# hyperplane-lab/ACL-GAN

Measured on AMD Instinct MI355X. Metric: training images/sec at 256x256 (gen+dis step), higher is better.
Workload: dtype fp32

## Files before the change

acl-gan_amd/csrc/common.h:

```cpp
#pragma once
#include <hip/hip_runtime.h>
#include <stdint.h>
#include <stddef.h>
#include <string>
#include <atomic>
#include "../../include/aclgan_hip.h"
#include "switches.h"

namespace aclgan {

void set_error(const char* fmt, ...);
int hip_fail(hipError_t e, const char* what);

extern std::atomic<long long> g_launches;
extern std::atomic<long long> g_enc_reuse_hits;

#define ACL_CHECK_LAUNCH(what)                                           \
    do {                                                                 \
        ++::aclgan::g_launches;                                          \
        hipError_t e__ = hipGetLastError();                              \
        if (e__ != hipSuccess) return ::aclgan::hip_fail(e__, what);     \
    } while (0)

#define ACL_REQUIRE(cond, ...)                                           \
    do {                                                                 \
        if (!(cond)) { ::aclgan::set_error(__VA_ARGS__); return ACLGAN_EINVAL; } \
    } while (0)

int reduce_slices_ordered(const float* part, int64_t n, int nslices, float* out, hipStream_t st);
size_t colsum_ordered_bytes(int64_t M, int C);
int colsum_ordered(const float* dy, float* db, int64_t M, int C, void* part, hipStream_t st);

static inline int cdiv(int a, int b) { return (a + b - 1) / b; }
static inline int64_t cdiv64(int64_t a, int64_t b) { return (a + b - 1) / b; }

struct ConvGeom {
    int B, Hi, Wi, Ci, Co, k, s, p, up, act;
    int Hu, Wu;
    int Hp, Wp;
    int Ho, Wo;
    int M;
    int K;
};
int make_geom(const aclgan_conv_desc* d, ConvGeom* g);

int conv_fold(const ConvGeom& g, const float* dxp, float* dx, int accumulate, hipStream_t st);
double conv_exec_flops(const ConvGeom& g, int which, bool f16);
bool conv_wgrad_fast_supported(const ConvGeom& g);
int conv_fwd(const ConvGeom& g, const float* x, const float* w, const float* bias, float* y, hipStream_t st, void* scratch = nullptr, float* stats = nullptr,
             float* keepV = nullptr);
size_t conv_fwd_keep_bytes(const ConvGeom& g);
int conv_fwd_stats_chunk(const ConvGeom& g);
size_t conv_fwd_scratch_bytes(const ConvGeom& g);
size_t conv_up5_scratch_bytes(const ConvGeom& g);
int conv_up5_fwd(const ConvGeom& g, const float* x, const float* w, const float* bias, float* y, void* scratch, hipStream_t st, float* keepV = nullptr);
int conv_fwd_naive(const ConvGeom& g, const float* x, const float* w, const float* bias, float* y, hipStream_t st);
size_t conv_dgrad_scratch_bytes(const ConvGeom& g);
int conv_dgrad(const ConvGeom& g, const float* dy, const float* w, float* dx, void* scratch, int accumulate, hipStream_t st);
int conv_wgrad(const ConvGeom& g, const float* x, const float* dy, float* dw, float* db, hipStream_t st, void* scratch = nullptr, const float* haveV = nullptr);
size_t conv_wgrad_scratch_bytes(const ConvGeom& g);
int conv_up5_dgrad(const ConvGeom& g, const float* dy, const float* w, float* dx, int accumulate, void* scratch, hipStream_t st);
int conv_up5_wgrad(const ConvGeom& g, const float* x, const float* dy, float* dw, float* db, void* scratch, hipStream_t st, const float* haveV = nullptr);

int conv_fwd_fast(const ConvGeom& g, const float* x, const float* w, const float* bias, float* y, hipStream_t st, void* scratch = nullptr, float* stats = nullptr,
                  float* keepV = nullptr);
size_t conv_fwd_fast_scratch_bytes(const ConvGeom& g);
int conv_dgrad_fast(const ConvGeom& g, const float* dy, const float* w, float* dxp, float* dx, int accumulate, bool* direct, hipStream_t st);
int conv_wgrad_fast(const ConvGeom& g, const float* x, const float* dy, float* dw, float* db, hipStream_t st, void* scratch = nullptr, const float* haveV = nullptr);
size_t conv_wgrad_fast_scratch_bytes(const ConvGeom& g);

struct WinoUCache { void* user; float* (*lookup)(void* user, const float* w, int variant, size_t bytes, bool* fresh); };
void set_wino_ucache(const WinoUCache* c);
const WinoUCache* wino_ucache();
size_t conv_wino_u_bytes(const ConvGeom& g);
int conv_wino_u_variant(const ConvGeom& g, int dgrad, bool keepV);
int conv_up5_wino_u_variant(const ConvGeom& g, int dgrad, bool keepV);
int conv_wino_prefill(const ConvGeom& g, int uv, const float* w0, int64_t w_stride, float* U0, int64_t u_stride, int count, hipStream_t st);
int wino_fused_filter_batch(const float* w0, int64_t w_stride, float* Uf0, int64_t u_stride, int count, int Co, int Ci, int flip, hipStream_t st);

bool conv_wino_ok(const ConvGeom& g);
size_t conv_wino_scratch_bytes(const ConvGeom& g);
int conv_fwd_wino(const ConvGeom& g, const float* x, const float* w, const float* bias, float* y, void* scratch, hipStream_t st, float* stats = nullptr,
                  float* keepV = nullptr);
size_t conv_wino_keep_bytes(const ConvGeom& g);
size_t conv_up5_wino_keep_bytes(const ConvGeom& g);
int conv_dgrad_wino_interior(const ConvGeom& g, const float* dy, const float* w, float* dx, int accumulate, void* scratch, hipStream_t st);
size_t conv_wgrad_wino_scratch_bytes(const ConvGeom& g);
bool conv_up5_wino_ok(const ConvGeom& g);
size_t conv_up5_wino_fwd_scratch_bytes(const ConvGeom& g);
size_t conv_up5_wino_dgrad_scratch_bytes(const ConvGeom& g);
size_t conv_up5_wino_wgrad_scratch_bytes(const ConvGeom& g);
int conv_up5_wino_fwd_phases(const ConvGeom& g, const float* x, const float* wp, const float* bias, float* y, void* scratch, hipStream_t st, float* keepV = nullptr,
                             const float* wkey = nullptr);
int conv_up5_wino_dgrad_phases(const ConvGeom& g, const float* dy, const float* wp, float* dx, int accumulate, void* scratch, hipStream_t st,
                               const float* wkey = nullptr);
bool wino_u_cached(const float* wkey, int variant);
int conv_up5_wino_wgrad_phases(const ConvGeom& g, const float* x, const float* dy, float* dwp, float* db, void* scratch, hipStream_t st, const float* haveV = nullptr);
size_t conv_up5_dgrad_scratch_bytes(const ConvGeom& g);
int conv_wgrad_wino(const ConvGeom& g, const float* x, const float* dy, float* dw, float* db, void* scratch, hipStream_t st, const float* haveV = nullptr);

bool conv16_eligible(const ConvGeom& g, int which);
size_t conv_fwd16_scratch_bytes(const ConvGeom& g);
size_t conv_dgrad16_scratch_bytes(const ConvGeom& g);
size_t conv_wgrad16_scratch_bytes(const ConvGeom& g);
int conv_fwd16(const ConvGeom& g, int dtype, const float* x, const float* w, const void* w16, const float* bias, float* y, void* scratch, hipStream_t st,
               const void* x16 = nullptr, int y_storage = 0);
int conv_dgrad16(const ConvGeom& g, int dtype, const float* dy, const float* w, const void* w16t, float* dx, int accumulate, void* scratch, hipStream_t st);
int conv_wgrad16(const ConvGeom& g, int dtype, const float* x, const float* dy, float* dw, float* db, void* scratch, hipStream_t st, int x_storage = 0,
                 int dy_storage = 0);

bool conv16s_ok(const ConvGeom& g, int which);
int conv_fwd16s_stats_chunk(const ConvGeom& g);
int wino_fused_force(int on);
bool wino_fused_ok(int B, int H, int W, int Cin_, int Cout_, int act = ACLGAN_ACT_NONE, int gph = 1, int kph = 1);
int wino_fused_filter(const float* w, float* Uf, int Co, int Ci, int flip, hipStream_t st, int nph = 1);
int wino_fused_launch(int B, int H, int W, int Cin_, int Cout_, const float* in, const float* Uf, const float* bias, float* out, int act, int accumulate,
                      int reflect, float2* stats, hipStream_t st);
int wino_fused_up5_fwd(int B, int Hi, int Wi, int Cin_, int Cout_, const float* x, const float* Uf, const float* bias, float* y, int Hf, int Wf, int act,
                       hipStream_t st);
bool wino_wgrad_fused_ok(const ConvGeom& g);
size_t wino_wgrad_fused_scratch_bytes(const ConvGeom& g);
int wino_wgrad_fused(const ConvGeom& g, const float* x, const float* dy, float* dw, float* db, void* scratch, hipStream_t st);
int wino_fused_up5_dgrad(int B, int Hi, int Wi, int Cin_, int Cout_, const float* dy, const float* Uf, float* dx, int Hf, int Wf, int accumulate, hipStream_t st);
bool wino_fused_s2k4_ok(int B, int Hi, int Wi, int Ci, int Co, int act, int dgrad);
size_t wino_fused_s2k4_u_bytes(int Ci, int Co);
int wino_fused_filter_s2k4(const float* w, float* Uf, int Co, int Ci, int dgrad, hipStream_t st);
int wino_fused_s2k4_fwd(int B, int Hi, int Wi, int Ci, int Co, const float* x, const float* Uf, const float* bias, float* y, int act, float2* stats, hipStream_t st);
int wino_fused_s2k4_dgrad(int B, int Hi, int Wi, int Ci, int Co, const float* dy, const float* Uf, float* dx, int accumulate, hipStream_t st);
bool conv_s2k4_wino_ok(const ConvGeom& g, int which);
size_t conv_s2k4_wino_scratch_bytes(const ConvGeom& g);
int conv_fwd_s2k4_wino(const ConvGeom& g, const float* x, const float* w, const float* bias, float* y, void* scratch, hipStream_t st, float* stats = nullptr);
int conv_dgrad_s2k4_wino_interior(const ConvGeom& g, const float* dy, const float* w, float* dx, int accumulate, void* scratch, hipStream_t st);
bool gemm_x3_shape_ok(int T, int K, int N);
int gemm_slices_x3(const void* A3, size_t a_plane, const void* B3, size_t b_plane, float* C, int T, int K, int N, int nslices, int a_mod, hipStream_t st);
int split3_planes(const float* x, void* out, int64_t n, int64_t plane_elems, hipStream_t st);
int conv_fwd16s(const ConvGeom& g, int dtype, const void* x16, const void* w16, const float* bias, void* y, int yst, hipStream_t st, float* stats = nullptr);
size_t conv_dgrad16s_scratch_bytes(const ConvGeom& g);
bool conv_wgrad16s_ok(const ConvGeom& g);
size_t conv_wgrad16s_scratch_bytes(const ConvGeom& g);
int conv_wgrad16s(const ConvGeom& g, int dtype, const void* x16, const void* dy16, float* dw, float* db, void* scratch, hipStream_t st);
int conv_dgrad16s(const ConvGeom& g, int dtype, const void* dy16, const void* w16t, void* dx, int dxst, int accumulate, void* scratch, hipStream_t st);
int cast_flat16(const float* src, void* dst, int64_t n, int dtype, hipStream_t st);
int transpose_flat16(const float* base, void* base_t, const int64_t* offs, const int* co, const int* taps, const int* ci, int n, int dtype, hipStream_t st);

int conv_fwd_small(const ConvGeom& g, const float* x, const float* w, const float* bias, float* y, hipStream_t st);
int conv_wgrad_small(const ConvGeom& g, const float* x, const float* dy, float* dw, float* db, hipStream_t st, void* scratch = nullptr);
size_t conv_wgrad_small_scratch_bytes(const ConvGeom& g);
int conv_dgrad_small(const ConvGeom& g, const float* dy, const float* w, float* dxp, hipStream_t st);
bool conv_s2k4_thin_dgrad_ok(const ConvGeom& g);

size_t norm_scratch_bytes(int B, int HW, int C);
struct NormST { int x = 0, y = 0, res = 0, dy = 0, dx = 0, dres = 0; };
int norm_fwd(int kind, int act, int B, int HW, int C, const void* x, const float* w, const float* b, int w_stride,
             const void* residual, void* y, float* mean, float* rstd, void* scratch, hipStream_t st, const float* stats = nullptr,
             int stats_chunk = 0, const NormST* sto = nullptr, float* ss_out = nullptr);
int norm_bwd(int kind, int act, int B, int HW, int C, const void* x, const void* y, const void* dy,
             const float* w, int w_stride, const float* mean, const float* rstd, void* dx, float* dw, float* db,
             void* dres, int dres_accumulate, void* scratch, hipStream_t st, const NormST* sto = nullptr, float* sbc_out = nullptr,
             const float* ss = nullptr);
int norm_bwd_ln_params(const float* sbc, int B, int C, float* dgamma, float* dbeta, hipStream_t st);

int act_bwd_inplace(int act, const void* y, void* dy, int64_t n, hipStream_t st, int yst = 0, int gst = 0);
int cast_storage(const void* src, int src_st, void* dst, int dst_st, int64_t n, hipStream_t st);
int positive_mask(const void* y, int yst, unsigned char* dst, int64_t n, hipStream_t st);
int positive_mask_diff(const float* a, int ca, const float* b, int cb, unsigned char* dst, int64_t npix, hipStream_t st);
int avgpool3s2_fwd(int B, int H, int W, int C, const float* x, float* y, hipStream_t st);
int avgpool3s2_bwd(int B, int H, int W, int C, const float* dy, float* dx, int accumulate, hipStream_t st);
size_t diffaugment_scratch_bytes(int N, int H, int W, int C);
int diffaugment_fwd(int N, int H, int W, int C, int policy, const float* x, const float* params, float* y, void* scratch, hipStream_t st);
int diffaugment_bwd(int N, int H, int W, int C, int policy, const float* dy, const float* params, float* dx, int accumulate, void* scratch, hipStream_t st);
int adam_flat(float* p, const float* g, float* m, float* v, int64_t n, const aclgan_adam* o, int step, hipStream_t st);
int adam_flat_ema(float* p, const float* g, float* m, float* v, float* ema, int64_t n, const aclgan_adam* o, int step, float decay, int mode, hipStream_t st);
int nchw_to_nhwc(const float* src, float* dst, int B, int C, int H, int W, hipStream_t st);
int nhwc_to_nchw(const float* src, float* dst, int B, int C, int H, int W, hipStream_t st);
int fill_zero(float* p, int64_t n, hipStream_t st);

int linear_fwd(int B, int I, int O, const float* x, const float* w, const float* bias, int act, float* y, hipStream_t st);
bool mlp3_fwd_ok(int S, int M);
int mlp3_fwd(int B, int S, int M, int O, const float* s, const float* W0, const float* b0, const float* W1, const float* b1, const float* W2,
             const float* b2, float* m0, float* m1, float* ap, hipStream_t st);
int linear_bwd(int B, int I, int O, const float* x, const float* y, float* dy, const float* w, int act,
               float* dx, float* dw, float* db, hipStream_t st);
int linear_bwd_params(int B, int I, int O, const float* x, const float* dy, float* dw, float* db, hipStream_t st);
int gap_fwd(int B, int HW, int C, const void* x, float* y, hipStream_t st, int xst = 0);
int gap_bwd(int B, int HW, int C, const float* dy, void* dx, int accumulate, hipStream_t st, int xst = 0);

int focus_blend_fwd(int B, int HW, const float* dec4, const float* bg, float* out, const float* pair_first, float* pair, hipStream_t st);
int focus_blend_bwd(int B, int HW, const float* dec4, const float* bg, const float* d_out, const float* d_pair,
                    float* d_dec4, float* d_bg, int bg_accumulate, hipStream_t st);
int plain_pair_fwd(int B, int HW, const float* dec3, float* out, const float* pair_first, float* pair, hipStream_t st);
int plain_pair_bwd(int B, int HW, const float* d_out, const float* d_pair, float* d_dec3, hipStream_t st);
int focus_translation_nchw(const float* fg, int64_t fg_bstride, const float* bg, int64_t bg_bstride, const float* focus, int64_t focus_bstride,
                           float* out, int B, int HW, hipStream_t st);
int lsgan_loss(const float* o, int n, float target, float weight, float* loss_slot, float* d_o, float gscale, hipStream_t st, const float* lscale = nullptr);
struct LsganTerm { const float* o; float* d_o; float* slot; int n; float target, weight, gscale; };
const int LSGAN_MAX_TERMS = 12;
int lsgan_loss_batch(const LsganTerm* terms, int nterms, hipStream_t st, const float* lscale = nullptr);
const int L1_PART_FLOATS = 1024;
int l1_loss(const float* a, int a_stride, const float* b, int64_t npix, float* loss_slot, float* d_a, float gscale, int d_accumulate, hipStream_t st,
            const float* lscale = nullptr, float* part = nullptr);
int focus_sums_blocks(int64_t npix);
int focus_sums(const float* dec4, int64_t npix, float eps, float upper, float* part, hipStream_t st);
int focus_loss_finish(const float* dec4, int64_t npix, const float* part, float delta, float upper, float lower, float eps,
                      float scale, float* size_slot, float* digit_slot, float* d_dec4, hipStream_t st, const float* lscale = nullptr,
                      const float* totals = nullptr, int64_t npix_total = 0);
int focus_totals(const float* part, int64_t npix, int nmask, float* totals, hipStream_t st);
int adam_flat_scaled(float* p, const float* g, float* m, float* v, int64_t n, const aclgan_adam* o, int step, float* state, int group, hipStream_t st);
int adam_flat_scaled_ema(float* p, const float* g, float* m, float* v, float* ema, int64_t n, const aclgan_adam* o, int step, float decay, int mode,
                         float* state, int group, hipStream_t st);


const int SN_MAX_LAYERS = 16;
struct SnLayerPtrs { const float* w; float* u; float* v; float* wn; float* uf; float* vf; float* G; int co, k; };
size_t sn_scratch_bytes(int n, const int* co, const int* k);
int sn_power_iteration(int n, const SnLayerPtrs* L, float* sigma, void* scratch, hipStream_t st);
struct SnFoldPtrs { const float* w; const float* G; const float* u; const float* v; float* grad; int co, k; };
size_t sn_fold_scratch_bytes(int n, const int* co, const int* k);
int sn_fold(int n, const SnFoldPtrs* L, const float* sigma, void* scratch, hipStream_t st);

}
```

acl-gan_amd/csrc/conv_fast.hip:

```cpp
#include "conv_fast_common.h"
#include <cstring>

namespace aclgan {
namespace {


constexpr int BK = 16;
constexpr int WG_MAX_CHUNK = 1024 + 16;
constexpr int LDK = BK + 4;

template <int T, bool KC>
__device__ __forceinline__ void read_frags(const float* __restrict__ tile, int ld, int base, int lane, float (&f)[T][8]) {
    const int l31 = lane & 31, kh = lane >> 5;
    if (KC) {
#pragma unroll
        for (int t = 0; t < T; ++t) {
            const f32x4* p = reinterpret_cast<const f32x4*>(tile + (base + t * 32 + l31) * LDK + kh * 8);
            const f32x4 a = p[0], b = p[1];
            f[t][0] = a.x; f[t][1] = a.y; f[t][2] = a.z; f[t][3] = a.w;
            f[t][4] = b.x; f[t][5] = b.y; f[t][6] = b.z; f[t][7] = b.w;
        }
    } else {
#pragma unroll
        for (int ks = 0; ks < 8; ++ks)
#pragma unroll
            for (int t = 0; t < T; ++t) f[t][ks] = tile[(kh * 8 + ks) * ld + base + t * 32 + l31];
    }
}

template <int TM, int TN>
__device__ __forceinline__ void mfma_step(const float (&fa)[TM][8], const float (&fb)[TN][8], int ks, f32x16 (&acc)[TM][TN]) {
#pragma unroll
    for (int i = 0; i < TM; ++i)
#pragma unroll
        for (int j = 0; j < TN; ++j) acc[i][j] = __builtin_amdgcn_mfma_f32_32x32x2f32(fa[i][ks], fb[j][ks], acc[i][j], 0, 0, 0);
}

#define ACL_GEMM_MAINLOOP(TM_, TN_, AKC_, BKC_, KBEG_, NK_, AS_, BS_, ASTR_, BSTR_, LDA_, LDB_, AM_, BN_) \
    do {                                                                                                 \
        const int nk__ = (NK_), kb__ = (KBEG_);                                                          \
        fetch(kb__);                                                                                     \
        stage(0, true);                                                                                  \
        fetch(kb__ + min(1, nk__ - 1));                                                                  \
        __syncthreads();                                                                                 \
        for (int kt = 0; kt < nk__; ++kt) {                                                              \
            const int cur = kt & 1;                                                                      \
            float fa[TM_][8], fb[TN_][8];                                                                \
            read_frags<TM_, AKC_>((AS_) + cur * (ASTR_), (LDA_), (AM_), lane, fa);                       \
            read_frags<TN_, BKC_>((BS_) + cur * (BSTR_), (LDB_), (BN_), lane, fb);                       \
            if (!(AKC_) && !(BKC_)) __builtin_amdgcn_sched_barrier(0);    \
            mfma_step<TM_, TN_>(fa, fb, 0, acc);                                                         \
            stage(cur ^ 1, kt + 1 < nk__);                                                               \
            fetch(kb__ + min(kt + 2, nk__ - 1));                                                         \
            __builtin_amdgcn_sched_barrier(0x6);    \
            mfma_step<TM_, TN_>(fa, fb, 1, acc);                                                         \
            mfma_step<TM_, TN_>(fa, fb, 2, acc);                                                         \
            mfma_step<TM_, TN_>(fa, fb, 3, acc);                                                         \
            mfma_step<TM_, TN_>(fa, fb, 4, acc);                                                         \
            mfma_step<TM_, TN_>(fa, fb, 5, acc);                                                         \
            mfma_step<TM_, TN_>(fa, fb, 6, acc);                                                         \
            mfma_step<TM_, TN_>(fa, fb, 7, acc);                                                         \
            __syncthreads();                                                                             \
        }                                                                                                \
    } while (0)



template <int WM, int WN, int TM, int TN, int OCC = 1>
__global__ void __launch_bounds__(WM * WN * 64, OCC) conv_fwd_fast_kernel(FwdFP pk) {
    constexpr int BM = WM * TM * 32, BN = WN * TN * 32, NT = WM * WN * 64;
    constexpr int RP = NT / 4;
    FwdFP p = pk;
    if (pk.fsl) {
        const long long f = blockIdx.y;
        p.x += (pk.fsx_mod ? f % pk.fsx_mod : f) * pk.fs_x; p.w += f * pk.fs_w; p.y += f * pk.fs_y;
    }
    constexpr int A_IT = BM / RP, B_IT = (BN + RP - 1) / RP;
    __shared__ __attribute__((aligned(16))) float smem[2 * (BM + BN) * LDK];
    __shared__ int ro[BM];
    float* As = smem;
    float* Bs = smem + 2 * BM * LDK;

    const int tid = threadIdx.x, lane = tid & 63, wave = tid >> 6;
    const int wm = wave / WN, wn = wave % WN;
    const int tile = xcd_map(blockIdx.x, p.nwg);
    const int m0 = (tile / p.tiles_n) * BM, n0 = (tile % p.tiles_n) * BN;
    const int q = tid & 3, r0 = tid >> 2;
    const int phase = p.phases ? (int)blockIdx.z : 0;
    const float* wbase = p.w + (size_t)phase * p.Co * p.K;

    for (int r = tid; r < BM; r += NT) {
        int b, oy, ox, o = -1;
        if (fwd_row(p, m0 + r, b, oy, ox)) {
            if (p.phases) o = (b * p.Hf + 2 * (oy + 1) + (phase >> 1)) * p.Wf + 2 * (ox + 1) + (phase & 1);
            else o = (b * p.Ho + oy) * p.Wo + ox;
        }
        ro[r] = o;
    }
    int ay[A_IT], ax[A_IT], ab[A_IT];
#pragma unroll
    for (int i = 0; i < A_IT; ++i) {
        int b = 0, oy = 0, ox = 0;
        if (!fwd_row(p, m0 + r0 + i * RP, b, oy, ox)) { b = 0; oy = 0; ox = 0; }
        ay[i] = oy * p.s - p.p; ax[i] = ox * p.s - p.p; ab[i] = b * p.Hi * p.Wi;
    }
    int wo[B_IT];
#pragma unroll
    for (int i = 0; i < B_IT; ++i) wo[i] = min(n0 + r0 + i * RP, p.Co - 1) * p.K + q * 4;

    const int cpt = p.Ci >> 4;
    int aoff[A_IT];
    f32x4 ra[A_IT], rb[B_IT];
    int f_tap = -1;

    auto fetch = [&](int kt) __attribute__((always_inline)) {
        const int tap = kt / cpt, cc = kt - tap * cpt;
        if (tap != f_tap) {
            f_tap = tap;
            const int ky = tap / p.k, kx = tap - ky * p.k;
#pragma unroll
            for (int i = 0; i < A_IT; ++i) {
                const int iy = refl(ay[i] + ky, p.Hu) >> p.up;
                const int ix = refl(ax[i] + kx, p.Wu) >> p.up;
                aoff[i] = (ab[i] + iy * p.Wi + ix) * p.Ci + q * 4;
            }
        }
#pragma unroll
        for (int i = 0; i < A_IT; ++i) ra[i] = *reinterpret_cast<const f32x4*>(p.x + (size_t)aoff[i] + cc * 16);
#pragma unroll
        for (int i = 0; i < B_IT; ++i)
            if (BN % RP == 0 || r0 + i * RP < BN) rb[i] = *reinterpret_cast<const f32x4*>(wbase + (size_t)wo[i] + kt * 16);
    };
    auto stage = [&](int buf, bool real) __attribute__((always_inline)) {
        float* a = As + buf * BM * LDK;
        float* b = Bs + buf * BN * LDK;
#pragma unroll
        for (int i = 0; i < A_IT; ++i) *reinterpret_cast<f32x4*>(a + (r0 + i * RP) * LDK + q * 4) = ra[i];
#pragma unroll
        for (int i = 0; i < B_IT; ++i)
            if (BN % RP == 0 || r0 + i * RP < BN) *reinterpret_cast<f32x4*>(b + (r0 + i * RP) * LDK + q * 4) = rb[i];
    };

    f32x16 acc[TM][TN];
#pragma unroll
    for (int i = 0; i < TM; ++i)
#pragma unroll
        for (int j = 0; j < TN; ++j)
#pragma unroll
            for (int r = 0; r < 16; ++r) acc[i][j][r] = 0.f;

    const int nk_all = p.K / BK;
    const int kbeg = p.phases ? 0 : blockIdx.z * p.nkz, nk = p.phases ? nk_all : min(p.nkz, nk_all - kbeg);
    if (nk <= 0) return;
    const bool split = !p.phases && gridDim.z > 1;
    ACL_GEMM_MAINLOOP(TM, TN, true, true, kbeg, nk, As, Bs, BM * LDK, BN * LDK, LDK, LDK, wm * TM * 32, wn * TN * 32);

    const int l31 = lane & 31, lh = lane >> 5;
#pragma unroll
    for (int j = 0; j < TN; ++j) {
        const int n = n0 + wn * TN * 32 + j * 32 + l31;
        if (n >= p.Co) continue;
        const float bv = p.bias ? p.bias[n] : 0.f;
#pragma unroll
        for (int i = 0; i < TM; ++i) {
#pragma unroll
            for (int r = 0; r < 16; ++r) {
                const int rl = wm * TM * 32 + i * 32 + (r & 3) + 8 * (r >> 2) + 4 * lh;
                const int o = ro[rl];
                if (o >= 0) {
                    if (split && p.part) p.part[((size_t)blockIdx.z * p.rows + m0 + rl) * p.Co + n] = acc[i][j][r];
                    else if (split) atomicAdd(p.y + (size_t)o * p.Co + n, acc[i][j][r] + ((p.ring > 0 && blockIdx.z == 0) ? bv : 0.f));
                    else p.y[(size_t)o * p.Co + n] = act_apply(acc[i][j][r] + bv, p.act);
                }
            }
        }
    }
}


template <int WM, int WN, int TM, int TN>
int launch_fwd_fast(const ConvGeom& g, FwdFP p, hipStream_t st) {
    constexpr int BM = WM * TM * 32, BN = WN * TN * 32;
    p.tiles_n = cdiv(g.Co, BN);
    int rows = p.M;
    if (p.ring > 0) rows = p.B * (p.Ho * p.Wo - std::max(0, p.Ho - 2 * p.ring) * std::max(0, p.Wo - 2 * p.ring));
    p.nwg = cdiv(rows, BM) * p.tiles_n;
    if (p.phases) {
        hipLaunchKernelGGL((conv_fwd_fast_kernel<WM, WN, TM, TN>), dim3(p.nwg, 1, 4), dim3(WM * WN * 64), 0, st, p);
        ACL_CHECK_LAUNCH("conv_fwd_fast_kernel(phases)");
        return ACLGAN_OK;
    }
    int splits = 1;
    fwd_split_plan(rows, g.Co, g.K, BK, &splits, &p.nkz);
    p.rows = rows;
    if (splits > 1 && p.part != nullptr) {
        hipLaunchKernelGGL((conv_fwd_fast_kernel<WM, WN, TM, TN>), dim3(p.nwg, 1, splits), dim3(WM * WN * 64), 0, st, p);
        ACL_CHECK_LAUNCH("conv_fwd_fast_kernel(split)");
        hipLaunchKernelGGL(fwd_split_finish_kernel, dim3((int)std::min<int64_t>(cdiv64((int64_t)rows * std::max(1, g.Co / 4), 256), 4096)), dim3(256), 0, st, p, splits);
        ACL_CHECK_LAUNCH("fwd_split_finish_kernel");
        return ACLGAN_OK;
    }
    p.part = nullptr;
    const int nk = g.K / BK;
    if (p.ring > 0 && (p.act != ACLGAN_ACT_NONE || g.Co % 4 != 0)) splits = 1, p.nkz = nk;
    if (sw(SW_DETERMINISTIC)) splits = 1, p.nkz = nk;
    if (splits > 1 && p.ring > 0) {
        hipLaunchKernelGGL(ring_zero_kernel, dim3(cdiv(rows * (g.Co / 4), 256)), dim3(256), 0, st, p, rows);
        ACL_CHECK_LAUNCH("ring_zero_kernel");
    } else if (splits > 1) {
        hipError_t e = hipMemsetAsync(p.y, 0, (size_t)g.M * g.Co * sizeof(float), st);
        if (e != hipSuccess) return hip_fail(e, "memset y");
    }
    hipLaunchKernelGGL((conv_fwd_fast_kernel<WM, WN, TM, TN>), dim3(p.nwg, 1, splits), dim3(WM * WN * 64), 0, st, p);
    ACL_CHECK_LAUNCH("conv_fwd_fast_kernel");
    if (splits > 1 && p.ring == 0) {
        const int64_t n = (int64_t)g.M * g.Co;
        hipLaunchKernelGGL(bias_act_kernel, dim3((int)std::min<int64_t>(cdiv64(n, 256), 4096)), dim3(256), 0, st, p.y, p.bias, g.Co, p.act, n);
        ACL_CHECK_LAUNCH("bias_act_kernel");
    }
    return ACLGAN_OK;
}


template <int WM, int WN, int TM, int TN>
__global__ void __launch_bounds__(WM * WN * 64) conv_dgrad_fast_kernel(DgFP p) {
    constexpr int BM = WM * TM * 32, BN = WN * TN * 32, NT = WM * WN * 64;
    constexpr int RP = NT / 4;
    constexpr int A_IT = BM / RP;
    constexpr int LDB = BN + 4, NVB = BN / 4;
    constexpr int B_IT = (BK * NVB + NT - 1) / NT;
    __shared__ __attribute__((aligned(16))) float smem[2 * (BM * LDK + BK * LDB)];
    __shared__ int ri_o[BM];
    __shared__ unsigned long long tap_mask;
    __shared__ int tap_list[64];
    float* As = smem;
    float* Bs = smem + 2 * BM * LDK;

    const int tid = threadIdx.x, lane = tid & 63, wave = tid >> 6;
    const int wm = wave / WN, wn = wave % WN;
    const int tile = xcd_map(blockIdx.x, p.nwg);
    const int m0 = (tile / p.tiles_n) * BM;
    const int n0 = (tile % p.tiles_n) * BN;
    const int cls = blockIdx.z / p.ksplit, slice = blockIdx.z - cls * p.ksplit;
    const int cy = cls / p.s, cx = cls % p.s;
    const int Tx = (p.k - cx + p.s - 1) / p.s, Ty = (p.k - cy + p.s - 1) / p.s;
    const int q = tid & 3, r0 = tid >> 2;

    int ylo, yhi, xlo, xhi;
    dg_box(p, cy, cx, ylo, yhi, xlo, xhi);
    const bool compact = p.mode == 2 && Ty * Tx <= 64;
    if (tid == 0) tap_mask = 0ull;
    __syncthreads();
    for (int r = tid; r < BM; r += NT) {
        int oo = -1, b, y2, x2;
        if (dg_row(p, m0 + r, ylo, yhi, xlo, xhi, b, y2, x2)) {
            const int py = y2 * p.s + cy, px = x2 * p.s + cx;
            if (compact && py < p.Hp && px < p.Wp) {
                unsigned long long mk = 0ull;
                for (int t = 0; t < Ty * Tx; ++t) {
                    const int ty = t / Tx, tx = t - ty * Tx;
                    const int oy = y2 - ty, ox = x2 - tx;
                    bool ok = (unsigned)oy < (unsigned)p.Ho && (unsigned)ox < (unsigned)p.Wo;
                    if (p.band > 0) ok = ok && (oy < 2 || oy >= p.Ho - 2 || ox < 2 || ox >= p.Wo - 2);
                    if (ok) mk |= 1ull << t;
                }
                if (mk) atomicOr(&tap_mask, mk);
            }
            if (py < p.Hp && px < p.Wp) {
                if (p.mode == 0 || p.ringpad) oo = (b * p.Hp + py) * p.Wp + px;
                else oo = (b * p.Hd + (refl(py - p.pad, p.Hi) >> p.upshift)) * p.Wd + (refl(px - p.pad, p.Wi) >> p.upshift);
            }
        }
        ri_o[r] = oo;
    }
    int ntap = Ty * Tx;
    if (compact) {
        __syncthreads();
        if (tid == 0) {
            int n = 0;
            for (int t = 0; t < Ty * Tx; ++t)
                if ((tap_mask >> t) & 1ull) tap_list[n++] = t;
            tap_list[63] = n;
        }
        __syncthreads();
        ntap = tap_list[63];
        if (ntap == 0) return;
    }
    int ay[A_IT], ax[A_IT], ab[A_IT];
#pragma unroll
    for (int i = 0; i < A_IT; ++i) {
        int b = 0, y2 = 0, x2 = 0;
        if (!dg_row(p, m0 + r0 + i * RP, ylo, yhi, xlo, xhi, b, y2, x2)) { b = 0; y2 = 0; x2 = 0; }
        ay[i] = y2; ax[i] = x2; ab[i] = b;
    }
    int bo[B_IT];
#pragma unroll
    for (int i = 0; i < B_IT; ++i) {
        const int idx = tid + i * NT;
        const int krow = idx / NVB, nc = idx - krow * NVB;
        const int n = n0 + nc * 4;
        bo[i] = krow * p.k * p.k * p.Ci + (n < p.Ci ? n : 0);
    }
    const int cpt = p.Co >> 4;
    int aoff[A_IT];
    f32x4 ra[A_IT], rb[B_IT];
    float za[A_IT];
    int f_tap = -1, tapoff = 0;

    auto fetch = [&](int kt) __attribute__((always_inline)) {
        const int tq = kt / cpt, cc = kt - tq * cpt;
        if (tq != f_tap) {
            f_tap = tq;
            const int t = compact ? tap_list[tq] : tq;
            const int ty = t / Tx, tx = t - ty * Tx;
            tapoff = ((cy + p.s * ty) * p.k + (cx + p.s * tx)) * p.Ci;
#pragma unroll
            for (int i = 0; i < A_IT; ++i) {
                const int oy = ay[i] - ty, ox = ax[i] - tx;
                const bool ok = (unsigned)oy < (unsigned)p.Ho && (unsigned)ox < (unsigned)p.Wo;
                bool okk = ok;
                if (p.band > 0) okk = ok && (oy < 2 || oy >= p.Ho - 2 || ox < 2 || ox >= p.Wo - 2);
                const int dpix = p.dyv ? (ab[i] * p.Hf + 2 * (oy + 1) + p.py) * p.Wf + 2 * (ox + 1) + p.px
                                       : (ab[i] * p.Ho + oy) * p.Wo + ox;
                aoff[i] = okk ? dpix * p.Co + q * 4 : -1;
            }
        }
#pragma unroll
        for (int i = 0; i < A_IT; ++i) {
            ra[i] = *reinterpret_cast<const f32x4*>(p.dy + (size_t)(aoff[i] < 0 ? 0 : aoff[i]) + cc * 16);
            za[i] = aoff[i] < 0 ? 0.f : 1.f;
        }
#pragma unroll
        for (int i = 0; i < B_IT; ++i)
            if ((BK * NVB) % NT == 0 || tid + i * NT < BK * NVB)
                rb[i] = *reinterpret_cast<const f32x4*>(p.w + (size_t)bo[i] + tapoff + (size_t)cc * 16 * p.k * p.k * p.Ci);
    };
    auto stage = [&](int buf, bool real) __attribute__((always_inline)) {
        float* a = As + buf * BM * LDK;
        float* b = Bs + buf * BK * LDB;
#pragma unroll
        for (int i = 0; i < A_IT; ++i) *reinterpret_cast<f32x4*>(a + (r0 + i * RP) * LDK + q * 4) = ra[i] * za[i];
#pragma unroll
        for (int i = 0; i < B_IT; ++i) {
            const int idx = tid + i * NT;
            if ((BK * NVB) % NT == 0 || idx < BK * NVB) {
                const int krow = idx / NVB, nc = idx - krow * NVB;
                *reinterpret_cast<f32x4*>(b + krow * LDB + nc * 4) = rb[i];
            }
        }
    };

    f32x16 acc[TM][TN];
#pragma unroll
    for (int i = 0; i < TM; ++i)
#pragma unroll
        for (int j = 0; j < TN; ++j)
#pragma unroll
            for (int r = 0; r < 16; ++r) acc[i][j][r] = 0.f;

    const int nk_all = ntap * cpt;
    const int nkz = (nk_all + p.ksplit - 1) / p.ksplit;
    const int kbeg = slice * nkz, nk = min(nkz, nk_all - kbeg);
    if (nk <= 0) return;
    ACL_GEMM_MAINLOOP(TM, TN, true, false, kbeg, nk, As, Bs, BM * LDK, BK * LDB, LDK, LDB, wm * TM * 32, wn * TN * 32);

    const int l31 = lane & 31, lh = lane >> 5;
#pragma unroll
    for (int j = 0; j < TN; ++j) {
        const int n = n0 + wn * TN * 32 + j * 32 + l31;
        if (n >= p.Ci) continue;
#pragma unroll
        for (int i = 0; i < TM; ++i) {
#pragma unroll
            for (int r = 0; r < 16; ++r) {
                const int of = ri_o[wm * TM * 32 + i * 32 + (r & 3) + 8 * (r >> 2) + 4 * lh];
                if (of >= 0) {
                    float* o = p.dxp + (size_t)of * p.Ci + n;
                    if (p.ksplit > 1 || (p.mode == 2 && !p.ringpad)) atomicAdd(o, acc[i][j][r]);
                    else if (p.accumulate) *o += acc[i][j][r];
                    else *o = acc[i][j][r];
                }
            }
        }
    }
}

template <int WM, int WN, int TM, int TN>
int launch_dgrad_fast(const ConvGeom& g, DgFP p, hipStream_t st) {
    constexpr int BM = WM * TM * 32, BN = WN * TN * 32;
    int mmax = 0;
    for (int cy = 0; cy < g.s; ++cy)
        for (int cx = 0; cx < g.s; ++cx) {
            const int ylo = g.p > cy ? (g.p - cy + g.s - 1) / g.s : 0, xlo = g.p > cx ? (g.p - cx + g.s - 1) / g.s : 0;
            const int yhi = std::min(p.Hc - 1, (g.p + g.Hi - 1 - cy) / g.s), xhi = std::min(p.Wc - 1, (g.p + g.Wi - 1 - cx) / g.s);
            int inner = (yhi - ylo + 1) * (xhi - xlo + 1);
            if (p.band > 0) inner = std::max(0, p.Hc - 2 * p.band) * std::max(0, p.Wc - 2 * p.band);
            const int rows = p.mode == 0 ? p.Hc * p.Wc : (p.mode == 1 ? inner : p.Hc * p.Wc - inner);
            mmax = std::max(mmax, g.B * rows);
        }
    if (mmax <= 0) return ACLGAN_OK;
    p.Mc = mmax;
    p.tiles_n = cdiv(g.Ci, BN);
    p.nwg = cdiv(p.Mc, BM) * p.tiles_n;
    const int nk_min = ((g.k + g.s - 1) / g.s) * ((g.k + g.s - 1) / g.s) * (g.Co / 16);
    const int nblk = p.nwg * g.s * g.s;
    p.ksplit = 1;
    const int nk_plan = (p.mode == 2 && p.band == 0) ? std::max(g.Co / 16, nk_min / ((g.k + g.s - 1) / g.s)) : nk_min;
    if (nblk < 128 && nk_plan >= 32 && !sw(SW_DETERMINISTIC) && !p.ringpad)
        p.ksplit = max(1, min(nk_plan / 8, 512 / nblk));
    if (p.ksplit > 1 && p.mode == 0) {
        hipError_t e = hipMemsetAsync(p.dxp, 0, conv_dgrad_scratch_bytes(g), st);
        if (e != hipSuccess) return hip_fail(e, "memset dxp");
    }
    if (p.ksplit > 1 && p.mode == 1 && !p.accumulate) {
        hipError_t e = hipMemsetAsync(p.dxp, 0, (size_t)g.B * g.Hi * g.Wi * g.Ci * sizeof(float), st);
        if (e != hipSuccess) return hip_fail(e, "memset dx");
    }
    hipLaunchKernelGGL((conv_dgrad_fast_kernel<WM, WN, TM, TN>), dim3(p.nwg, 1, g.s * g.s * p.ksplit), dim3(WM * WN * 64), 0, st, p);
    ACL_CHECK_LAUNCH("conv_dgrad_fast_kernel");
    return ACLGAN_OK;
}

template <int WM, int WN, int TM, int TN>
int launch_dgrad_halo(const ConvGeom& g, DgFP p, hipStream_t st) {
    if (p.band == 0 && !p.ringpad && g.k == 3 && g.s == 1 && g.Ci % 128 == 0 && WM == 2 && WN == 2 && TM == 2 && TN == 2)
        return launch_dgrad_fast<2, 2, 1, 2>(g, p, st);
    return launch_dgrad_fast<WM, WN, TM, TN>(g, p, st);
}

template <int WM, int WN, int TM, int TN>
int dgrad_fast_all(const ConvGeom& g, DgFP p, float* dxp, float* dx, int accumulate, bool* direct, hipStream_t st) {
    if (g.up == 0 && dx != nullptr && (!sw(SW_DETERMINISTIC) || g.p == 0 || (dxp && conv_wino_ok(g)))) {
        *direct = true;
        p.dxp = dx; p.accumulate = accumulate;
        p.mode = 1;
        int rc = (dxp && conv_wino_ok(g)) ? conv_dgrad_wino_interior(g, p.dy, p.w, dx, accumulate, dxp, st)
             : (dxp && conv_s2k4_wino_ok(g, 1)) ? conv_dgrad_s2k4_wino_interior(g, p.dy, p.w, dx, accumulate, dxp, st)
                                      : launch_dgrad_fast<WM, WN, TM, TN>(g, p, st);
        if (rc) return rc;
        if (g.p > 0 && sw(SW_DETERMINISTIC)) {
            hipError_t e = hipMemsetAsync(dxp, 0, (size_t)g.B * g.Hp * g.Wp * g.Ci * sizeof(float), st);
            if (e != hipSuccess) return hip_fail(e, "memset padded grid");
            p.mode = 2; p.ringpad = 1; p.dxp = dxp; p.accumulate = 0;
            rc = launch_dgrad_fast<WM, WN, TM, TN>(g, p, st);
            if (rc) return rc;
            return conv_fold(g, dxp, dx, 1, st);
        }
        if (g.p > 0) { p.mode = 2; rc = launch_dgrad_halo<WM, WN, TM, TN>(g, p, st); }
        return rc;
    }
    *direct = false;
    p.dxp = dxp; p.mode = 0; p.accumulate = 0;
    return launch_dgrad_fast<WM, WN, TM, TN>(g, p, st);
}


template <int WM, int WN, int TM, int TN, bool ST>
__global__ void __launch_bounds__(WM * WN * 64) conv_wgrad_fast_kernel(WgFP p) {
    constexpr int BM = WM * TM * 32, BN = WN * TN * 32, NT = WM * WN * 64;
    constexpr int LDA = BM + 4, LDB = BN + 4, MVA = BM / 4, NVB = BN / 4;
    constexpr int A_IT = (BK * MVA + NT - 1) / NT, B_IT = (BK * NVB + NT - 1) / NT;
    __shared__ __attribute__((aligned(16))) float smem[2 * BK * (LDA + LDB)];
    float* As = smem;
    float* Bs = smem + 2 * BK * LDA;

    const int tid = threadIdx.x, lane = tid & 63, wave = tid >> 6;
    const int wm = wave / WN, wn = wave % WN;
    const int tile = xcd_map(blockIdx.x, p.nwg);
    const int m0 = (tile / p.tiles_n) * BM, n0 = (tile % p.tiles_n) * BN;
    const int pbeg = blockIdx.z * p.chunk;
    const int pend = min(p.P, pbeg + p.chunk);
    if (pbeg >= pend) return;
    const int phase = p.phases ? (int)blockIdx.y : 0;
    float* dwbase = p.dw + (size_t)phase * p.Co * p.Kn + (size_t)blockIdx.z * p.dw_zs;
    const int py = phase >> 1, px = phase & 1;

    __shared__ int4 pinfo[WG_MAX_CHUNK];
    const int st_tap = n0 / p.Ci, st_ky = st_tap / p.k, st_kx = st_tap - st_ky * p.k;
    for (int i = tid; i < pend - pbeg + BK; i += NT) {
        int b, oy, ox;
        wg_coord(p, min(pbeg + i, pend - 1), b, oy, ox);
        const int dyp = p.phases ? (b * p.Hf + 2 * (oy + 1) + py) * p.Wf + 2 * (ox + 1) + px : (b * p.Ho + oy) * p.Wo + ox;
        if (ST) {
            const int iy = refl(oy * p.s - p.p + st_ky, p.Hu) >> p.up, ix = refl(ox * p.s - p.p + st_kx, p.Wu) >> p.up;
            pinfo[i] = make_int4(b * p.Hi * p.Wi + iy * p.Wi + ix, 0, 0, dyp);
        } else {
            pinfo[i] = make_int4(oy * p.s - p.p, ox * p.s - p.p, b * p.Hi * p.Wi, dyp);
        }
    }
    __syncthreads();

    int a_m[A_IT], a_kr[A_IT];
#pragma unroll
    for (int i = 0; i < A_IT; ++i) {
        const int idx = tid + i * NT;
        a_kr[i] = idx / MVA;
        const int m = m0 + (idx - a_kr[i] * MVA) * 4;
        a_m[i] = m < p.Co ? m : 0;
    }
    int b_kr[B_IT], b_ci[B_IT], b_ky[B_IT], b_kx[B_IT];
#pragma unroll
    for (int i = 0; i < B_IT; ++i) {
        const int idx = tid + i * NT;
        b_kr[i] = idx / NVB;
        int n = n0 + (idx - b_kr[i] * NVB) * 4;
        if (n >= p.Kn) n = 0;
        const int tap = n / p.Ci;
        b_ci[i] = n - tap * p.Ci; b_ky[i] = tap / p.k; b_kx[i] = tap - b_ky[i] * p.k;
    }
    f32x4 ra[A_IT], rb[B_IT];
    float za[A_IT];
    const bool do_bias = p.db != nullptr && (tile % p.tiles_n) == 0;
    f32x4 bsum[A_IT];
#pragma unroll
    for (int i = 0; i < A_IT; ++i) bsum[i] = (f32x4){0.f, 0.f, 0.f, 0.f};

    auto fetch = [&](int kt) __attribute__((always_inline)) {
        const int pb = kt * BK;
#pragma unroll
        for (int i = 0; i < A_IT; ++i) {
            if ((BK * MVA) % NT != 0 && tid + i * NT >= BK * MVA) continue;
            const int pi = pb + a_kr[i];
            ra[i] = *reinterpret_cast<const f32x4*>(p.dy + (size_t)pinfo[pi].w * p.Co + a_m[i]);
            za[i] = pbeg + pi < pend ? 1.f : 0.f;
        }
#pragma unroll
        for (int i = 0; i < B_IT; ++i) {
            if ((BK * NVB) % NT != 0 && tid + i * NT >= BK * NVB) continue;
            if (ST) {
                rb[i] = *reinterpret_cast<const f32x4*>(p.x + (size_t)pinfo[pb + b_kr[i]].x * p.Ci + b_ci[i]);
            } else {
                const int4 pi = pinfo[pb + b_kr[i]];
                const int iy = refl(pi.x + b_ky[i], p.Hu) >> p.up;
                const int ix = refl(pi.y + b_kx[i], p.Wu) >> p.up;
                rb[i] = *reinterpret_cast<const f32x4*>(p.x + (size_t)(pi.z + iy * p.Wi + ix) * p.Ci + b_ci[i]);
            }
        }
    };
    auto stage = [&](int buf, bool real) __attribute__((always_inline)) {
        float* a = As + buf * BK * LDA;
        float* b = Bs + buf * BK * LDB;
#pragma unroll
        for (int i = 0; i < A_IT; ++i) {
            const int idx = tid + i * NT;
            if ((BK * MVA) % NT == 0 || idx < BK * MVA) {
                const f32x4 v = ra[i] * za[i];
                *reinterpret_cast<f32x4*>(a + a_kr[i] * LDA + (idx - a_kr[i] * MVA) * 4) = v;
                bsum[i] += v * (real ? 1.f : 0.f);
            }
        }
#pragma unroll
        for (int i = 0; i < B_IT; ++i) {
            const int idx = tid + i * NT;
            if ((BK * NVB) % NT == 0 || idx < BK * NVB) *reinterpret_cast<f32x4*>(b + b_kr[i] * LDB + (idx - b_kr[i] * NVB) * 4) = rb[i];
        }
    };

    f32x16 acc[TM][TN];
#pragma unroll
    for (int i = 0; i < TM; ++i)
#pragma unroll
        for (int j = 0; j < TN; ++j)
#pragma unroll
            for (int r = 0; r < 16; ++r) acc[i][j][r] = 0.f;

    ACL_GEMM_MAINLOOP(TM, TN, false, false, 0, (pend - pbeg + BK - 1) / BK, As, Bs, BK * LDA, BK * LDB, LDA, LDB, wm * TM * 32, wn * TN * 32);

    if (do_bias) {
        float* red = smem;
#pragma unroll
        for (int i = 0; i < A_IT; ++i) {
            const int idx = tid + i * NT;
            if ((BK * MVA) % NT == 0 || idx < BK * MVA) *reinterpret_cast<f32x4*>(red + a_kr[i] * BM + (idx - a_kr[i] * MVA) * 4) = bsum[i];
        }
        __syncthreads();
        if (tid < BM && m0 + tid < p.Co) {
            float t = 0.f;
#pragma unroll
            for (int r = 0; r < BK; ++r) t += red[r * BM + tid];
            atomicAdd(p.db + (size_t)blockIdx.z * p.db_zs + m0 + tid, t);
        }
    }
    const int l31 = lane & 31, lh = lane >> 5;
#pragma unroll
    for (int j = 0; j < TN; ++j) {
        const int n = n0 + wn * TN * 32 + j * 32 + l31;
        if (n >= p.Kn) continue;
#pragma unroll
        for (int i = 0; i < TM; ++i) {
#pragma unroll
            for (int r = 0; r < 16; ++r) {
                const int m = m0 + wm * TM * 32 + i * 32 + (r & 3) + 8 * (r >> 2) + 4 * lh;
                if (m < p.Co) {
                    atomicAdd(dwbase + (size_t)m * p.Kn + n, acc[i][j][r]);
                }
            }
        }
    }
}

constexpr int WGKC_TARGET = 768;

template <int WM, int WN, int TM, int TN>
__global__ void __launch_bounds__(WM * WN * 64) conv_wgrad_kc_kernel(WgFP pk, WgPartX xp) {
    constexpr int BM = WM * TM * 32, BN = WN * TN * 32, NT = WM * WN * 64;
    WgFP p = pk;
    if (pk.fsl) {
        const long long f = blockIdx.y;
        p.x += (pk.fsx_mod ? f % pk.fsx_mod : f) * pk.fs_x; p.dy += f * pk.fs_dy;
    }
    static_assert(BM % 64 == 0 && BN % 64 == 0 && BM + BN <= NT, "one staging unit (4 channels x 4 pixels) per thread, wave-uniform roles");
    constexpr int CH = 1024;
    __shared__ __attribute__((aligned(16))) float smem[2 * (BM + BN) * LDK];
    __shared__ int2 pinfo[CH + BK];
    float* As = smem;
    float* Bs = smem + 2 * BM * LDK;

    const int tid = threadIdx.x, lane = tid & 63, wave = tid >> 6;
    const int wm = wave / WN, wn = wave % WN;
    const int tile = xcd_map(blockIdx.x, p.nwg);
    const int m0 = (tile / p.tiles_n) * BM, n0 = (tile % p.tiles_n) * BN;
    const int pbeg = blockIdx.z * p.chunk;
    const int pend = min(p.P, pbeg + p.chunk);
    const int phase = (p.phases || p.fsl) ? (int)blockIdx.y : 0;
    float* dwbase = p.dw + (size_t)phase * p.Co * p.Kn;
    const int py = phase >> 1, px = phase & 1;
    const int st_tap = n0 / p.Ci, st_ky = st_tap / p.k, st_kx = st_tap - st_ky * p.k;

    const bool isA = tid < BM, isB = !isA && tid < BM + BN;
    const int u = isA ? tid : tid - BM;
    const int ncg = (isA ? BM : BN) >> 2;
    const int cg = u % ncg, pg = u / ncg;
    const float* src = isA ? p.dy : p.x;
    const int cstride = isA ? p.Co : p.Ci;
    const int chan = isA ? m0 + 4 * cg : (n0 - st_tap * p.Ci) + 4 * cg;
    float* mytile = isA ? As : Bs;
    const int tstride = (isA ? BM : BN) * LDK;
    f32x4 rr[4];
    float zm[4];
    const bool do_bias = p.db != nullptr && (tile % p.tiles_n) == 0;
    f32x4 bsum = {0.f, 0.f, 0.f, 0.f};

    f32x16 acc[TM][TN];
#pragma unroll
    for (int i = 0; i < TM; ++i)
#pragma unroll
        for (int j = 0; j < TN; ++j)
#pragma unroll
            for (int r = 0; r < 16; ++r) acc[i][j][r] = 0.f;

    for (int cb = pbeg; cb < pend; cb += CH) {
        const int ce = min(pend, cb + CH);
        for (int i = tid; i < ce - cb + BK; i += NT) {
            int b, oy, ox;
            wg_coord(p, min(cb + i, ce - 1), b, oy, ox);
            const int dyp = p.phases ? (b * p.Hf + 2 * (oy + 1) + py) * p.Wf + 2 * (ox + 1) + px : (b * p.Ho + oy) * p.Wo + ox;
            const int iy = refl(oy * p.s - p.p + st_ky, p.Hu) >> p.up, ix = refl(ox * p.s - p.p + st_kx, p.Wu) >> p.up;
            pinfo[i] = make_int2(b * p.Hi * p.Wi + iy * p.Wi + ix, dyp);
        }
        __syncthreads();

        auto fetch = [&](int kt) __attribute__((always_inline)) {
            const int pb = kt * BK + 4 * pg;
            if (isA || isB) {
#pragma unroll
                for (int j = 0; j < 4; ++j) {
                    const int2 pi = pinfo[pb + j];
                    rr[j] = *reinterpret_cast<const f32x4*>(src + (size_t)(isA ? pi.y : pi.x) * cstride + chan);
                    zm[j] = cb + pb + j < ce ? 1.f : 0.f;
                }
            }
        };
        auto stage = [&](int buf, bool real) __attribute__((always_inline)) {
            if (isA || isB) {
                float* t = mytile + buf * tstride;
                f32x4 v[4];
#pragma unroll
                for (int j = 0; j < 4; ++j) v[j] = rr[j] * zm[j];
                if (isA) {
                    const float on = real ? 1.f : 0.f;
#pragma unroll
                    for (int j = 0; j < 4; ++j) bsum += v[j] * on;
                }
#pragma unroll
                for (int c = 0; c < 4; ++c) {
                    const f32x4 k4 = {v[0][c], v[1][c], v[2][c], v[3][c]};
                    *reinterpret_cast<f32x4*>(t + (c * ncg + cg) * LDK + 4 * pg) = k4;
                }
            }
        };
        ACL_GEMM_MAINLOOP(TM, TN, true, true, 0, (ce - cb + BK - 1) / BK, As, Bs, BM * LDK, BN * LDK, LDK, LDK, wm * TM * 32, wn * TN * 32);
    }

    const bool partial = xp.part != nullptr;
    if (do_bias) {
        float* red = smem;
        if (isA) *reinterpret_cast<f32x4*>(red + pg * BM + 4 * cg) = bsum;
        __syncthreads();
        if (tid < BM) {
            const float t = red[tid] + red[BM + tid] + red[2 * BM + tid] + red[3 * BM + tid];
            if (partial) xp.part_b[((size_t)blockIdx.z * xp.ny + phase) * p.Co + m0 + tid] = t;
            else p.db[m0 + tid] += t;
        }
    }
    const int l31 = lane & 31, lh = lane >> 5;
    constexpr int MQ = BM / 4, NQ = BN / 4;
    if (partial) {
        float* pt = xp.part + (((size_t)blockIdx.z * xp.ny + phase) * p.nwg + tile) * (BM * BN);
#pragma unroll
        for (int j = 0; j < TN; ++j)
#pragma unroll
            for (int i = 0; i < TM; ++i)
#pragma unroll
                for (int r = 0; r < 16; ++r) {
                    const int rw = wm * TM * 32 + i * 32 + (r & 3) + 8 * (r >> 2) + 4 * lh;
                    pt[rw * BN + wn * TN * 32 + j * 32 + l31] = acc[i][j][r];
                }
        return;
    }
#pragma unroll
    for (int j = 0; j < TN; ++j) {
        const int cr = wn * TN * 32 + j * 32 + l31;
        const int n = n0 + 4 * (cr % NQ) + cr / NQ;
#pragma unroll
        for (int i = 0; i < TM; ++i) {
#pragma unroll
            for (int r = 0; r < 16; ++r) {
                const int rw = wm * TM * 32 + i * 32 + (r & 3) + 8 * (r >> 2) + 4 * lh;
                const int m = m0 + 4 * (rw % MQ) + rw / MQ;
                dwbase[(size_t)m * p.Kn + n] += acc[i][j][r];
            }
        }
    }
}

bool wgrad_kc_ok(const ConvGeom& g) {
    return !sw(SW_NOWGKC) && g.Co % 64 == 0 && g.Ci % 64 == 0;
}

template <int WM, int WN, int TM, int TN>
int launch_wgrad_kc(const ConvGeom& g, WgFP p, void* part, hipStream_t st) {
    constexpr int BM = WM * TM * 32, BN = WN * TN * 32;
    const int ny = p.fsl ? p.fsl : (p.phases ? 4 : 1);
    const WgPlan q = wgrad_plan(g.Co, p.Ci, p.Kn, p.P, ny, BK, WGKC_TARGET);
    if (q.BM != BM || q.BN != BN) { set_error("wgrad_kc: tile plan mismatch"); return ACLGAN_EINVAL; }
    p.tiles_n = q.tiles_n; p.nwg = q.nwg; p.chunk = q.chunk;
    WgPartX xp;
    xp.ny = ny; xp.part = nullptr; xp.part_b = nullptr;
    const bool use_part = q.splits > 1 || ny > 1;
    if (use_part) {
        if (!part) { set_error("wgrad_kc: %d slices need the scratch buffer", q.splits); return ACLGAN_EINVAL; }
        xp.part = (float*)part;
        xp.part_b = xp.part + (size_t)q.splits * ny * q.nwg * BM * BN;
    }
    hipLaunchKernelGGL((conv_wgrad_kc_kernel<WM, WN, TM, TN>), dim3(p.nwg, ny, q.splits), dim3(WM * WN * 64), 0, st, p, xp);
    ACL_CHECK_LAUNCH("conv_wgrad_kc_kernel");
    if (use_part) {
        const int64_t n = (int64_t)ny * g.Co * (p.Kn / 4);
        hipLaunchKernelGGL(wgrad_finish_kernel, dim3((int)std::min<int64_t>(cdiv64(n, 256), 4096)), dim3(256), 0, st, p, xp, BM, BN, q.splits);
        ACL_CHECK_LAUNCH("wgrad_finish_kernel");
    }
    return ACLGAN_OK;
}
int launch_wgrad_kc_any(const ConvGeom& g, const WgFP& p, void* part, hipStream_t st) {
    if (g.Co % 128 == 0 && p.Ci % 128 == 0) return launch_wgrad_kc<2, 2, 2, 2>(g, p, part, st);
    if (g.Co % 128 == 0) return launch_wgrad_kc<2, 2, 2, 1>(g, p, part, st);
    if (p.Ci % 128 == 0) return launch_wgrad_kc<2, 2, 1, 2>(g, p, part, st);
    return launch_wgrad_kc<2, 2, 1, 1>(g, p, part, st);
}

template <int WM, int WN, int TM, int TN>
int launch_wgrad_fast(const ConvGeom& g, WgFP p, hipStream_t st, void* det_part = nullptr) {
    constexpr int BM = WM * TM * 32, BN = WN * TN * 32;
    p.tiles_n = cdiv(p.Kn, BN);
    p.nwg = cdiv(g.Co, BM) * p.tiles_n;
    const int target = 1536;
    const int ny = p.phases ? 4 : 1;
    int splits = max(1, target / (p.nwg * ny));
    splits = max(1, min(splits, cdiv(p.P, 256)));
    splits = max(splits, cdiv(p.P, 1024));
    p.chunk = cdiv(cdiv(p.P, splits), 16) * 16;
    splits = cdiv(p.P, p.chunk);
    float* dw_out = p.dw; float* db_out = p.db;
    const int64_t ndw = (int64_t)ny * g.Co * p.Kn;
    if (det_part != nullptr && splits > 1) {
        hipError_t e = hipMemsetAsync(det_part, 0, (size_t)splits * (ndw + g.Co) * sizeof(float), st);
        if (e != hipSuccess) return hip_fail(e, "memset wgrad slices");
        p.dw = (float*)det_part; p.dw_zs = ndw;
        if (p.db) { p.db = (float*)det_part + (size_t)splits * ndw; p.db_zs = g.Co; }
    }
    if (p.Ci % BN == 0) hipLaunchKernelGGL((conv_wgrad_fast_kernel<WM, WN, TM, TN, true>), dim3(p.nwg, ny, splits), dim3(WM * WN * 64), 0, st, p);
    else hipLaunchKernelGGL((conv_wgrad_fast_kernel<WM, WN, TM, TN, false>), dim3(p.nwg, ny, splits), dim3(WM * WN * 64), 0, st, p);
    ACL_CHECK_LAUNCH("conv_wgrad_fast_kernel");
    if (p.dw_zs) {
        int rc = reduce_slices_ordered(p.dw, ndw, splits, dw_out, st);
        if (rc) return rc;
        if (db_out) { rc = reduce_slices_ordered(p.db, g.Co, splits, db_out, st); if (rc) return rc; }
    }
    return ACLGAN_OK;
}
size_t wgrad_fast_det_bytes(const ConvGeom& g, int Kn, int P, int ny) {
    const int nwg = cdiv(g.Co, 128) * cdiv(Kn, 128);
    int splits = std::max(1, 1536 / (nwg * ny));
    splits = std::max(1, std::min(splits, cdiv(P, 256)));
    splits = std::max(splits, cdiv(P, 1024)) + 1;
    return (size_t)splits * ((size_t)ny * g.Co * Kn + g.Co) * sizeof(float) + 256;
}


template <int WM, int WN, int TM, int TN>
int up5_fwd_t(const ConvGeom& g, const float* x, const float* w, const float* bias, float* y, float* wp, hipStream_t st, float* keepV) {
    const int64_t nm = (int64_t)4 * g.Co * 9 * (g.Ci / 4);
    if (!(conv_up5_wino_ok(g) && wino_u_cached(w, conv_up5_wino_u_variant(g, 0, keepV != nullptr)))) {
        hipLaunchKernelGGL(up5_merge_kernel, dim3((int)std::min<int64_t>(cdiv64(nm, 256), 2048)), dim3(256), 0, st, w, wp, g.Co, g.Ci);
        ACL_CHECK_LAUNCH("up5_merge_kernel");
    }
    FwdFP p;
    p.fsl = 0; p.fsx_mod = 0; p.fs_x = p.fs_w = p.fs_y = 0; p.w16 = nullptr; p.x16 = nullptr;
    p.x = x; p.w = wp; p.bias = bias; p.y = y;
    p.Hi = g.Hi; p.Wi = g.Wi; p.Ci = g.Ci; p.Ho = g.Hi - 2; p.Wo = g.Wi - 2; p.Co = g.Co; p.k = 3; p.s = 1; p.p = 0;
    p.up = 0; p.Hu = g.Hi; p.Wu = g.Wi; p.M = g.B * p.Ho * p.Wo; p.K = 9 * g.Ci; p.act = g.act; p.tiles_n = 0; p.nwg = 0; p.nkz = 0;
    p.B = g.B; p.ring = 0; p.phases = 1; p.Hf = g.Ho; p.Wf = g.Wo; p.part = nullptr; p.rows = 0;
    ConvGeom gp = g;
    gp.M = p.M; gp.K = p.K;
    char* wino_scr = (char*)wp + up5_merged_bytes(g) + ((fwd_partial_bytes(g, 2, BK) + 255) & ~(size_t)255);
    if (keepV && !conv_up5_wino_ok(g)) { set_error("conv_fwd: this layer does not keep a Winograd input transform"); return ACLGAN_EINVAL; }
    int rc = conv_up5_wino_ok(g) ? conv_up5_wino_fwd_phases(g, x, wp, bias, y, wino_scr, st, keepV, w) : launch_fwd_fast<WM, WN, TM, TN>(gp, p, st);
    if (rc) return rc;
    p.w = w;
    p.Hi = g.Hi; p.Wi = g.Wi; p.Ho = g.Ho; p.Wo = g.Wo; p.k = 5; p.s = 1; p.p = 2; p.up = 1; p.Hu = g.Hu; p.Wu = g.Wu;
    p.M = g.M; p.K = g.K; p.ring = 2; p.phases = 0;
    p.part = (float*)((char*)wp + up5_merged_bytes(g));
    return launch_fwd_fast<WM, WN, TM, TN>(g, p, st);
}

template <int WM, int WN, int TM, int TN>
int up5_wgrad_t(const ConvGeom& g, const float* x, const float* dy, float* dw, float* db, float* dwp, hipStream_t st, const float* haveV) {
    const size_t nb = (size_t)4 * g.Co * 9 * g.Ci * sizeof(float);
    hipError_t e = hipMemsetAsync(dwp, 0, nb, st);
    if (e != hipSuccess) return hip_fail(e, "memset dwp");
    const bool kc = wgrad_kc_ok(g);
    void* part = (char*)dwp + up5_dwp_bytes(g);
    WgFP p;
    p.fsl = 0; p.fsx_mod = 0; p.fs_x = p.fs_dy = 0;
    p.x = x; p.dy = dy; p.dw = dwp; p.db = db;
    p.Hi = g.Hi; p.Wi = g.Wi; p.Ci = g.Ci; p.Ho = g.Hi - 2; p.Wo = g.Wi - 2; p.Co = g.Co; p.k = 3; p.s = 1; p.p = 0;
    p.up = 0; p.Hu = g.Hi; p.Wu = g.Wi; p.P = g.B * p.Ho * p.Wo; p.Kn = 9 * g.Ci; p.chunk = 0; p.tiles_n = 0; p.nwg = 0;
    p.B = g.B; p.ring = 0; p.phases = 1; p.Hf = g.Ho; p.Wf = g.Wo;
    int rc;
    if (kc && conv_up5_wino_wgrad_scratch_bytes(g)) {
        void* wino_scr = (char*)dwp + ((wgrad_part_scratch(g, BK, WGKC_TARGET) + 255) & ~(size_t)255);
        rc = conv_up5_wino_wgrad_phases(g, x, dy, dwp, db, wino_scr, st, haveV);
    } else rc = kc ? launch_wgrad_kc_any(g, p, part, st) : launch_wgrad_fast<WM, WN, TM, TN>(g, p, st);
    if (rc) return rc;
    const int64_t ns = (int64_t)g.Co * 25 * (g.Ci / 4);
    hipLaunchKernelGGL(up5_scatter_kernel, dim3((int)std::min<int64_t>(cdiv64(ns, 256), 2048)), dim3(256), 0, st, dwp, dw, g.Co, g.Ci);
    ACL_CHECK_LAUNCH("up5_scatter_kernel");
    p.dw = dw;
    p.Hi = g.Hi; p.Wi = g.Wi; p.Ho = g.Ho; p.Wo = g.Wo; p.k = 5; p.s = 1; p.p = 2; p.up = 1; p.Hu = g.Hu; p.Wu = g.Wu;
    p.ring = 2; p.phases = 0; p.Kn = g.K;
    p.P = g.B * (g.Ho * g.Wo - (g.Ho - 4) * (g.Wo - 4));
    return kc ? launch_wgrad_kc_any(g, p, part, st) : launch_wgrad_fast<WM, WN, TM, TN>(g, p, st);
}

template <int WM, int WN, int TM, int TN>
int up5_dgrad_t(const ConvGeom& g, const float* dy, const float* w, float* dx, int accumulate, float* wp, hipStream_t st) {
    const int64_t nm = (int64_t)4 * g.Co * 9 * (g.Ci / 4);
    if (!(conv_up5_wino_ok(g) && wino_u_cached(w, conv_up5_wino_u_variant(g, 1, false)))) {
        hipLaunchKernelGGL(up5_merge_kernel, dim3((int)std::min<int64_t>(cdiv64(nm, 256), 2048)), dim3(256), 0, st, w, wp, g.Co, g.Ci);
        ACL_CHECK_LAUNCH("up5_merge_kernel");
    }
    ConvGeom gv = g;
    gv.k = 3; gv.s = 1; gv.p = 0; gv.up = 0; gv.Hu = g.Hi; gv.Wu = g.Wi; gv.Hp = g.Hi; gv.Wp = g.Wi;
    gv.Ho = g.Hi - 2; gv.Wo = g.Wi - 2; gv.M = g.B * gv.Ho * gv.Wo; gv.K = 9 * g.Ci;
    DgFP p;
    p.dy = dy; p.dxp = dx;
    p.Ho = gv.Ho; p.Wo = gv.Wo; p.Co = g.Co; p.Ci = g.Ci; p.k = 3; p.s = 1; p.Hp = g.Hi; p.Wp = g.Wi;
    p.Hc = g.Hi; p.Wc = g.Wi; p.Mc = 0; p.tiles_n = 0; p.nwg = 0; p.ksplit = 1;
    p.mode = 1; p.pad = 0; p.B = g.B; p.Hi = g.Hi; p.Wi = g.Wi;
    p.dyv = 1; p.Hf = g.Ho; p.Wf = g.Wo; p.band = 0; p.upshift = 0; p.Hd = g.Hi; p.Wd = g.Wi;
    if (conv_up5_wino_ok(g)) {
        const int rc = conv_up5_wino_dgrad_phases(g, dy, wp, dx, accumulate, (char*)wp + up5_merged_bytes(g), st, w);
        if (rc) return rc;
    } else for (int ph = 0; ph < 4; ++ph) {
        p.w = wp + (size_t)ph * g.Co * 9 * g.Ci;
        p.py = ph >> 1; p.px = ph & 1;
        p.accumulate = (ph > 0 || accumulate) ? 1 : 0;
        const int rc = launch_dgrad_fast<WM, WN, TM, TN>(gv, p, st);
        if (rc) return rc;
    }
    p.w = w;
    p.Ho = g.Ho; p.Wo = g.Wo; p.k = 5; p.s = 1; p.Hp = g.Hp; p.Wp = g.Wp; p.Hc = g.Hp; p.Wc = g.Wp;
    p.mode = 2; p.accumulate = 1; p.pad = 2; p.Hi = g.Hu; p.Wi = g.Wu;
    p.dyv = 0; p.band = 6; p.upshift = 1; p.Hd = g.Hi; p.Wd = g.Wi;
    if (sw(SW_DETERMINISTIC)) {
        float* dxp = (float*)((char*)wp + up5_merged_bytes(g));
        hipError_t e = hipMemsetAsync(dxp, 0, (size_t)g.B * g.Hp * g.Wp * g.Ci * sizeof(float), st);
        if (e != hipSuccess) return hip_fail(e, "memset padded grid");
        p.ringpad = 1; p.dxp = dxp; p.accumulate = 0;
        const int rc = launch_dgrad_fast<WM, WN, TM, TN>(g, p, st);
        if (rc) return rc;
        return conv_fold(g, dxp, dx, 1, st);
    }
    return launch_dgrad_fast<WM, WN, TM, TN>(g, p, st);
}


}

size_t conv_up5_scratch_bytes(const ConvGeom& g) {
    return up5_eligible(g) ? (size_t)4 * g.Co * 9 * g.Ci * sizeof(float) : 0;
}
size_t conv_up5_dgrad_scratch_bytes(const ConvGeom& g) {
    if (sw(SW_NOFAST) || !up5_eligible(g)) return 0;
    const size_t padded = sw(SW_DETERMINISTIC) ? (size_t)g.B * g.Hp * g.Wp * g.Ci * sizeof(float) : 0;
    return up5_merged_bytes(g) + std::max(conv_up5_wino_dgrad_scratch_bytes(g), padded);
}
size_t conv_wgrad_fast_scratch_bytes(const ConvGeom& g) {
    if (sw(SW_NOFAST)) return 0;
    if (wgrad_kc_ok(g) && conv_wino_ok(g)) return conv_wgrad_wino_scratch_bytes(g);
    if (wgrad_kc_ok(g)) return ((wgrad_part_scratch(g, BK, WGKC_TARGET) + 255) & ~(size_t)255) + (up5_eligible(g) ? conv_up5_wino_wgrad_scratch_bytes(g) : 0);
    if (sw(SW_DETERMINISTIC)) return wgrad_fast_det_bytes(g, g.K, g.M, 1);
    return conv_up5_scratch_bytes(g);
}
size_t conv_fwd_fast_scratch_bytes(const ConvGeom& g) {
    if (sw(SW_NOFAST)) return 0;
    if (conv_wino_ok(g)) return conv_wino_scratch_bytes(g);
    if (up5_eligible(g)) return up5_merged_bytes(g) + ((fwd_partial_bytes(g, 2, BK) + 255) & ~(size_t)255) + conv_up5_wino_fwd_scratch_bytes(g);
    return std::max(fwd_partial_bytes(g, 0, BK), conv_s2k4_wino_scratch_bytes(g));
}

int conv_up5_fwd(const ConvGeom& g, const float* x, const float* w, const float* bias, float* y, void* scratch, hipStream_t st, float* keepV) {
    if (sw(SW_NOFAST) || !up5_eligible(g) || !scratch) return ACLGAN_EUNSUPPORTED;
    if (g.Co > 64) return up5_fwd_t<2, 2, 2, 2>(g, x, w, bias, y, (float*)scratch, st, keepV);
    if (g.Co > 32) return up5_fwd_t<4, 1, 2, 2>(g, x, w, bias, y, (float*)scratch, st, keepV);
    return up5_fwd_t<4, 1, 2, 1>(g, x, w, bias, y, (float*)scratch, st, keepV);
}

int conv_up5_dgrad(const ConvGeom& g, const float* dy, const float* w, float* dx, int accumulate, void* scratch, hipStream_t st) {
    if (sw(SW_NOFAST) || !up5_eligible(g) || !scratch) return ACLGAN_EUNSUPPORTED;
    if (sw(SW_NOUP5DGRAD)) return ACLGAN_EUNSUPPORTED;
    if (g.Ci > 64) return up5_dgrad_t<2, 2, 2, 2>(g, dy, w, dx, accumulate, (float*)scratch, st);
    if (g.Ci > 32) return up5_dgrad_t<4, 1, 2, 2>(g, dy, w, dx, accumulate, (float*)scratch, st);
    return up5_dgrad_t<4, 1, 2, 1>(g, dy, w, dx, accumulate, (float*)scratch, st);
}

int conv_up5_wgrad(const ConvGeom& g, const float* x, const float* dy, float* dw, float* db, void* scratch, hipStream_t st, const float* haveV) {
    if (sw(SW_NOFAST) || !up5_eligible(g) || !scratch || !dw) return ACLGAN_EUNSUPPORTED;
    if (sw(SW_DETERMINISTIC) && !wgrad_kc_ok(g)) return ACLGAN_EUNSUPPORTED;
    if (g.Co > 64) return up5_wgrad_t<2, 2, 2, 2>(g, x, dy, dw, db, (float*)scratch, st, haveV);
    if (g.Co > 32) return up5_wgrad_t<2, 2, 1, 2>(g, x, dy, dw, db, (float*)scratch, st, haveV);
    return up5_wgrad_t<1, 4, 1, 2>(g, x, dy, dw, db, (float*)scratch, st, haveV);
}

int gemm_slices_f32(const float* A, const float* Bm, float* Cm, int T, int K, int N, int nslices, int a_mod, hipStream_t st) {
    if (K % 16 != 0 || T <= 0 || N <= 0) { set_error("gemm_slices_f32: bad shape"); return ACLGAN_EINVAL; }
    FwdFP p;
    p.part = nullptr; p.rows = 0; p.w16 = nullptr; p.x16 = nullptr;
    p.x = A; p.w = Bm; p.bias = nullptr; p.y = Cm;
    p.Hi = T; p.Wi = 1; p.Ci = K; p.Ho = T; p.Wo = 1; p.Co = N; p.k = 1; p.s = 1; p.p = 0;
    p.up = 0; p.Hu = T; p.Wu = 1; p.M = T; p.K = K; p.act = ACLGAN_ACT_NONE; p.tiles_n = 0; p.nwg = 0; p.nkz = K / BK;
    p.B = 1; p.ring = 0; p.phases = 0; p.Hf = 0; p.Wf = 0;
    p.fsl = nslices; p.fsx_mod = a_mod; p.fs_x = (long long)T * K; p.fs_w = (long long)N * K; p.fs_y = (long long)T * N;
    if (N > 64) {
        p.tiles_n = cdiv(N, 128); p.nwg = cdiv(T, 64) * p.tiles_n;
        hipLaunchKernelGGL((conv_fwd_fast_kernel<2, 2, 1, 2, 4>), dim3(p.nwg, nslices, 1), dim3(256), 0, st, p);
    } else if (N > 32) {
        p.tiles_n = cdiv(N, 64); p.nwg = cdiv(T, 256) * p.tiles_n;
        hipLaunchKernelGGL((conv_fwd_fast_kernel<4, 1, 2, 2>), dim3(p.nwg, nslices, 1), dim3(256), 0, st, p);
    } else {
        p.tiles_n = cdiv(N, 32); p.nwg = cdiv(T, 256) * p.tiles_n;
        hipLaunchKernelGGL((conv_fwd_fast_kernel<4, 1, 2, 1>), dim3(p.nwg, nslices, 1), dim3(256), 0, st, p);
    }
    ACL_CHECK_LAUNCH("conv_fwd_fast_kernel(gemm slices)");
    return ACLGAN_OK;
}

int conv_fwd_stats_chunk(const ConvGeom& g) {
    if (sw(SW_NOSTATFUSE) || sw(SW_NOFAST) || g.Ci % 16 != 0 || g.act != ACLGAN_ACT_NONE) return 0;
    if (conv_wino_ok(g)) return 16;
    return (g.Ho % 4 == 0 && g.Wo % 4 == 0 && conv_s2k4_wino_ok(g, 0)) ? 16 : 0;
}
size_t conv_fwd_keep_bytes(const ConvGeom& g) {
    if (sw(SW_NOKEEPV) || sw(SW_NOFAST) || !wgrad_kc_ok(g)) return 0;
    if (up5_eligible(g)) return conv_up5_wino_wgrad_scratch_bytes(g) ? conv_up5_wino_keep_bytes(g) : 0;
    if (g.Ci % 16 != 0 || !conv_wino_ok(g) || !conv_wgrad_wino_scratch_bytes(g)) return 0;
    return conv_wino_keep_bytes(g);
}
int conv_fwd_fast(const ConvGeom& g, const float* x, const float* w, const float* bias, float* y, hipStream_t st, void* scratch, float* stats, float* keepV) {
    if (sw(SW_NOFAST) || g.Ci % 16 != 0) return ACLGAN_EUNSUPPORTED;
    if (scratch && conv_wino_ok(g)) return conv_fwd_wino(g, x, w, bias, y, scratch, st, stats, keepV);
    if (scratch && !keepV && conv_s2k4_wino_ok(g, 0) && (!stats || (g.Ho % 4 == 0 && g.Wo % 4 == 0)))
        return conv_fwd_s2k4_wino(g, x, w, bias, y, scratch, st, stats);
    if (stats || keepV) return ACLGAN_EUNSUPPORTED;
    FwdFP p;
    p.fsl = 0; p.fsx_mod = 0; p.fs_x = p.fs_w = p.fs_y = 0; p.w16 = nullptr; p.x16 = nullptr;
    p.part = (float*)scratch; p.rows = 0;
    p.x = x; p.w = w; p.bias = bias; p.y = y;
    p.Hi = g.Hi; p.Wi = g.Wi; p.Ci = g.Ci; p.Ho = g.Ho; p.Wo = g.Wo; p.Co = g.Co; p.k = g.k; p.s = g.s; p.p = g.p;
    p.up = g.up; p.Hu = g.Hu; p.Wu = g.Wu; p.M = g.M; p.K = g.K; p.act = g.act; p.tiles_n = 0; p.nwg = 0; p.nkz = 0;
    p.B = g.B; p.ring = 0; p.phases = 0; p.Hf = 0; p.Wf = 0;
    if (g.Co > 64) return launch_fwd_fast<2, 2, 2, 2>(g, p, st);
    if (g.Co > 32) return launch_fwd_fast<4, 1, 2, 2>(g, p, st);
    return launch_fwd_fast<4, 1, 2, 1>(g, p, st);
}

int conv_dgrad_fast(const ConvGeom& g, const float* dy, const float* w, float* dxp, float* dx, int accumulate, bool* direct, hipStream_t st) {
    *direct = false;
    if (sw(SW_NOFAST) || g.Co % 16 != 0 || g.Ci % 4 != 0) return ACLGAN_EUNSUPPORTED;
    if (sw(SW_NODIRECT)) dx = nullptr;
    if (sw(SW_DETERMINISTIC) && !dxp) { set_error("conv_dgrad: deterministic mode needs the scratch buffer"); return ACLGAN_EINVAL; }
    DgFP p;
    p.dy = dy; p.w = w; p.dxp = dxp;
    p.Ho = g.Ho; p.Wo = g.Wo; p.Co = g.Co; p.Ci = g.Ci; p.k = g.k; p.s = g.s; p.Hp = g.Hp; p.Wp = g.Wp;
    p.Hc = cdiv(g.Hp, g.s); p.Wc = cdiv(g.Wp, g.s); p.Mc = 0; p.tiles_n = 0; p.nwg = 0; p.ksplit = 1;
    p.mode = 0; p.accumulate = 0; p.pad = g.p; p.B = g.B; p.Hi = g.Hu; p.Wi = g.Wu;
    p.dyv = 0; p.py = 0; p.px = 0; p.Hf = 0; p.Wf = 0; p.band = 0; p.upshift = 0; p.Hd = g.Hu; p.Wd = g.Wu;
    if (g.Ci > 64) return dgrad_fast_all<2, 2, 2, 2>(g, p, dxp, dx, accumulate, direct, st);
    if (g.Ci > 32) return dgrad_fast_all<4, 1, 2, 2>(g, p, dxp, dx, accumulate, direct, st);
    return dgrad_fast_all<4, 1, 2, 1>(g, p, dxp, dx, accumulate, direct, st);
}

size_t gemm_at_b_slices_scratch(int T, int M, int N, int nslices) {
    return wgrad_partial_bytes(wgrad_plan(M, N, N, T, nslices, BK, WGKC_TARGET), M, nslices) + 256;
}
int gemm_at_b_slices_f32(const float* A, const float* Bm, float* Cm, int T, int M, int N, int nslices, int b_mod, void* part, hipStream_t st) {
    if (M % 64 != 0 || N % 64 != 0 || T <= 0) { set_error("gemm_at_b_slices_f32: bad shape"); return ACLGAN_EINVAL; }
    WgFP p;
    p.x = Bm; p.dy = A; p.dw = Cm; p.db = nullptr;
    p.Hi = T; p.Wi = 1; p.Ci = N; p.Ho = T; p.Wo = 1; p.Co = M; p.k = 1; p.s = 1; p.p = 0;
    p.up = 0; p.Hu = T; p.Wu = 1; p.P = T; p.Kn = N; p.chunk = 0; p.tiles_n = 0; p.nwg = 0;
    p.B = 1; p.ring = 0; p.phases = 0; p.Hf = 0; p.Wf = 0;
    p.fsl = nslices; p.fsx_mod = b_mod; p.fs_x = (long long)T * N; p.fs_dy = (long long)T * M;
    p.dw_overwrite = 1;
    ConvGeom g;
    memset(&g, 0, sizeof g);
    g.Co = M; g.Ci = N;
    return launch_wgrad_kc_any(g, p, part, st);
}

bool conv_wgrad_fast_supported(const ConvGeom& g) { return !sw(SW_NOFAST) && g.Co % 4 == 0 && g.Ci % 4 == 0; }
int conv_wgrad_fast(const ConvGeom& g, const float* x, const float* dy, float* dw, float* db, hipStream_t st, void* scratch, const float* haveV) {
    if (sw(SW_NOFAST) || g.Co % 4 != 0 || g.Ci % 4 != 0) return ACLGAN_EUNSUPPORTED;
    WgFP p;
    p.fsl = 0; p.fsx_mod = 0; p.fs_x = p.fs_dy = 0;
    p.x = x; p.dy = dy; p.dw = dw; p.db = db;
    p.Hi = g.Hi; p.Wi = g.Wi; p.Ci = g.Ci; p.Ho = g.Ho; p.Wo = g.Wo; p.Co = g.Co; p.k = g.k; p.s = g.s; p.p = g.p;
    p.up = g.up; p.Hu = g.Hu; p.Wu = g.Wu; p.P = g.M; p.Kn = g.K; p.chunk = 0; p.tiles_n = 0; p.nwg = 0;
    p.B = g.B; p.ring = 0; p.phases = 0; p.Hf = 0; p.Wf = 0;
    if (scratch && conv_wino_ok(g) && wgrad_kc_ok(g)) return conv_wgrad_wino(g, x, dy, dw, db, scratch, st, haveV);
    if (wgrad_kc_ok(g) && (scratch || wgrad_part_scratch(g, BK, WGKC_TARGET) == 0)) return launch_wgrad_kc_any(g, p, scratch, st);
    void* det = nullptr;
    if (sw(SW_DETERMINISTIC)) {
        if (!scratch) { set_error("conv_wgrad: deterministic mode needs the scratch buffer (aclgan_conv2d_wgrad_ws)"); return ACLGAN_EINVAL; }
        det = scratch;
    }
    if (g.Co > 64) return launch_wgrad_fast<2, 2, 2, 2>(g, p, st, det);
    if (g.Co > 32) return launch_wgrad_fast<2, 2, 1, 2>(g, p, st, det);
    return launch_wgrad_fast<1, 4, 1, 2>(g, p, st, det);
}

namespace {
double fused_flops(int B, int OH, int OW, int Cin_, int Cout_, int gph, int kph) {
    const int TY = cdiv(OH, 4), TX = cdiv(OW, 4);
    const double wgs = (double)B * cdiv(TY, 4) * cdiv(TX, 8) * (Cout_ / 64) * gph;
    return wgs * 2.0 * 36.0 * 32.0 * 64.0 * (double)Cin_ * kph;
}
double pipe_flops(int B, int OH, int OW, int Cin_, int Cout_, int slices) { return 2.0 * 36.0 * slices * (double)B * cdiv(OH, 4) * cdiv(OW, 4) * Cin_ * Cout_; }
}
double conv_exec_flops(const ConvGeom& g, int which, bool f16) {
    const double direct = 2.0 * (double)g.M * g.Co * g.K;
    const double ringpix = (double)g.Ho * g.Wo - (double)std::max(0, g.Ho - 4) * std::max(0, g.Wo - 4);
    if (up5_eligible(g) && !sw(SW_NOFAST)) {
        const double ring_fwd = 2.0 * g.B * ringpix * g.Co * g.K;
        const double band = (double)g.Hp * g.Wp - (double)std::max(0, g.Hp - 12) * std::max(0, g.Wp - 12);
        const double ring_dg = 2.0 * g.B * band * g.Ci * g.Co * 9.0;
        if (!f16 && conv_up5_wino_ok(g)) {
            if (which == 0) return (wino_fused_ok(g.B, g.Hi - 2, g.Wi - 2, g.Ci, g.Co, g.act, 4, 1) ? fused_flops(g.B, g.Hi - 2, g.Wi - 2, g.Ci, g.Co, 4, 1)
                                                                                                     : pipe_flops(g.B, g.Hi - 2, g.Wi - 2, g.Ci, g.Co, 4)) + ring_fwd;
            if (which == 1) return (wino_fused_ok(g.B, g.Hi, g.Wi, g.Co, g.Ci, ACLGAN_ACT_NONE, 1, 4) ? fused_flops(g.B, g.Hi, g.Wi, g.Co, g.Ci, 1, 4)
                                                                                                       : pipe_flops(g.B, g.Hi, g.Wi, g.Co, g.Ci, 4)) + ring_dg;
            return (conv_up5_wino_wgrad_scratch_bytes(g) ? pipe_flops(g.B, g.Hi - 2, g.Wi - 2, g.Ci, g.Co, 4) : 4.0 * 2.0 * g.B * (g.Hi - 2.0) * (g.Wi - 2.0) * g.Co * 9.0 * g.Ci) + ring_fwd;
        }
        const double phases = 4.0 * 2.0 * g.B * (g.Hi - 2.0) * (g.Wi - 2.0) * g.Co * 9.0 * g.Ci;
        return phases + (which == 1 ? ring_dg : ring_fwd);
    }
    if (!f16 && !sw(SW_NOFAST) && g.Ci % 16 == 0 && conv_wino_ok(g)) {
        const double halo = 2.0 * g.B * ((double)g.Hp * g.Wp - (double)g.Hi * g.Wi) * g.Ci * g.Co * 3.0;
        if (which == 0) return wino_fused_ok(g.B, g.Hi, g.Wi, g.Ci, g.Co, g.act) && !conv_fwd_keep_bytes(g) ? fused_flops(g.B, g.Hi, g.Wi, g.Ci, g.Co, 1, 1)
                                                                                                              : pipe_flops(g.B, g.Hi, g.Wi, g.Ci, g.Co, 1);
        if (which == 1) return (wino_fused_ok(g.B, g.Hi, g.Wi, g.Co, g.Ci, ACLGAN_ACT_NONE) ? fused_flops(g.B, g.Hi, g.Wi, g.Co, g.Ci, 1, 1) : pipe_flops(g.B, g.Hi, g.Wi, g.Co, g.Ci, 1)) + halo;
        if (wgrad_kc_ok(g) && conv_wgrad_wino_scratch_bytes(g)) return pipe_flops(g.B, g.Hi, g.Wi, g.Ci, g.Co, 1);
        return direct;
    }
    const bool s2k4_dg_direct = !sw(SW_NODIRECT);
    if (!f16 && !sw(SW_NOFAST) && which < 2 && conv_s2k4_wino_ok(g, which) && (which == 0 || s2k4_dg_direct)) {
        if (which == 0) return fused_flops(g.B, g.Ho, g.Wo, g.Ci, g.Co, 1, 4);
        const double halo = 2.0 * g.B * ((double)g.Hp * g.Wp - (double)g.Hi * g.Wi) * g.Ci * g.Co * 2.0;
        return fused_flops(g.B, g.Ho, g.Wo, g.Co, g.Ci, 4, 1) + halo;
    }
    if (which == 1 && !f16 && conv_s2k4_thin_dgrad_ok(g)) return 0.0;
    if (which == 1 && g.Ci < 32) return direct * 32.0 / g.Ci;
    if (which == 2 && g.k == 7 && (g.Ci < 16 || g.Co < 16)) return direct * 1.09 * (g.Ci == 3 ? 4.0 / 3.0 : 1.0);
    return direct;
}

}
```

acl-gan_amd/csrc/conv_wino.hip:

```cpp
#include "common.h"
#include "st16.h"
#include <atomic>
#include <cstdlib>
#include <algorithm>

namespace aclgan {

int gemm_slices_f32(const float* A, const float* Bm, float* Cm, int T, int K, int N, int nslices, int a_mod, hipStream_t st);
size_t gemm_at_b_slices_scratch(int T, int M, int N, int nslices);
int gemm_at_b_slices_f32(const float* A, const float* Bm, float* Cm, int T, int M, int N, int nslices, int b_mod, void* part, hipStream_t st);

static thread_local const WinoUCache* g_ucache = nullptr;
void set_wino_ucache(const WinoUCache* c) { g_ucache = c; }
const WinoUCache* wino_ucache() { return g_ucache; }
bool wino_u_cached(const float* wkey, int variant) {
    if (!g_ucache || !wkey) return false;
    bool fresh = true;
    float* u = g_ucache->lookup(g_ucache->user, wkey, variant, 0, &fresh);
    return u != nullptr && !fresh;
}

namespace {

float* cached_u(float* scratch_u, const float* key, int variant, size_t bytes, bool* fresh) {
    *fresh = true;
    if (!g_ucache || !key) return scratch_u;
    float* u = g_ucache->lookup(g_ucache->user, key, variant, bytes, fresh);
    if (!u) { *fresh = true; return scratch_u; }
    return u;
}
enum { U_PIPE = 0, U_FRAG = 1, U_X3 = 2 };
inline int uvar(int variant, int layout) { return variant | (layout << 4); }

__device__ __forceinline__ int reflw(int v, int n) {
    v = v < 0 ? -v : v;
    return v >= n ? 2 * (n - 1) - v : v;
}
__device__ __forceinline__ float actw(float v, int act) {
    if (act == ACLGAN_ACT_RELU) return v > 0.f ? v : 0.f;
    if (act == ACLGAN_ACT_LRELU) return v > 0.f ? v : 0.2f * v;
    if (act == ACLGAN_ACT_TANH) return tanhf(v);
    return v;
}

template <int NV> struct VecOf { typedef float T __attribute__((ext_vector_type(NV))); };
template <> struct VecOf<1> { typedef float T; };
template <int NV> __device__ __forceinline__ typename VecOf<NV>::T actv(typename VecOf<NV>::T v, int act) {
    if (act == ACLGAN_ACT_NONE) return v;
#pragma unroll
    for (int e = 0; e < NV; ++e) v[e] = actw(v[e], act);
    return v;
}
template <> __device__ __forceinline__ float actv<1>(float v, int act) { return actw(v, act); }

template <typename F>
__device__ __forceinline__ void bt6(const F (&d)[6], F (&t)[6]) {
    t[0] = 4.f * d[0] - 5.f * d[2] + d[4];
    t[1] = -4.f * d[1] - 4.f * d[2] + d[3] + d[4];
    t[2] = 4.f * d[1] - 4.f * d[2] - d[3] + d[4];
    t[3] = -2.f * d[1] - d[2] + 2.f * d[3] + d[4];
    t[4] = 2.f * d[1] - d[2] - 2.f * d[3] + d[4];
    t[5] = 4.f * d[1] - 5.f * d[3] + d[5];
}
template <typename F>
__device__ __forceinline__ void g6(const F (&g)[3], F (&u)[6]) {
    u[0] = 0.25f * g[0];
    u[1] = -(g[0] + g[1] + g[2]) * (1.f / 6.f);
    u[2] = -(g[0] - g[1] + g[2]) * (1.f / 6.f);
    u[3] = g[0] * (1.f / 24.f) + g[1] * (1.f / 12.f) + g[2] * (1.f / 6.f);
    u[4] = g[0] * (1.f / 24.f) - g[1] * (1.f / 12.f) + g[2] * (1.f / 6.f);
    u[5] = g[2];
}
template <typename F>
__device__ __forceinline__ void at4(const F (&m)[6], F (&y)[4]) {
    y[0] = m[0] + m[1] + m[2] + m[3] + m[4];
    y[1] = m[1] - m[2] + 2.f * (m[3] - m[4]);
    y[2] = m[1] + m[2] + 4.f * (m[3] + m[4]);
    y[3] = m[1] - m[2] + 8.f * (m[3] - m[4]) + m[5];
}

__global__ void __launch_bounds__(256) wino_filter_kernel(const float* __restrict__ w, float* __restrict__ U, int Co, int Ci, int flip, int64_t planes,
                                                          int64_t wstr, int64_t ustr, int64_t ustr16) {
    const int R = flip ? Ci : Co, K = flip ? Co : Ci;
    const int64_t n = (int64_t)R * K;
    w += (size_t)blockIdx.y * wstr;
    unsigned short* U16 = reinterpret_cast<unsigned short*>(U) + (size_t)blockIdx.y * ustr16;
    U += (size_t)blockIdx.y * ustr;
    for (int64_t i = (int64_t)blockIdx.x * 256 + threadIdx.x; i < n; i += (int64_t)gridDim.x * 256) {
        const int kk = (int)(i % K), row = (int)(i / K);
        const int co = flip ? kk : row, ci = flip ? row : kk;
        float t[6][3];
#pragma unroll
        for (int kx = 0; kx < 3; ++kx) {
            float c[3];
#pragma unroll
            for (int ky = 0; ky < 3; ++ky) {
                const int sy = flip ? 2 - ky : ky, sx = flip ? 2 - kx : kx;
                c[ky] = w[((size_t)(co * 3 + sy) * 3 + sx) * Ci + ci];
            }
            float o[6];
            g6(c, o);
#pragma unroll
            for (int a = 0; a < 6; ++a) t[a][kx] = o[a];
        }
#pragma unroll
        for (int a = 0; a < 6; ++a) {
            float o[6];
            g6(t[a], o);
#pragma unroll
            for (int j = 0; j < 6; ++j) {
                const size_t at = ((size_t)(a * 6 + j) * R + row) * K + kk;
                if (planes) {
                    unsigned short h, m, l;
                    split3(o[j], h, m, l);
                    U16[at] = h; U16[at + planes] = m; U16[at + 2 * planes] = l;
                } else {
                    U[at] = o[j];
                }
            }
        }
    }
}

struct WView { int H, W, sy, sx, oy0, ox0, HS, WS; };
struct WViews { WView v[4]; int nph; };
__host__ __device__ __forceinline__ size_t vaddr(const WView& v, int b, int iy, int ix, int C) {
    return ((size_t)(b * v.HS + v.oy0 + v.sy * iy) * v.WS + v.ox0 + v.sx * ix) * C;
}
WView ident_view(int H, int W) { WView v = {H, W, 1, 1, 0, 0, H, W}; return v; }
WView phase_view(int Hv, int Wv, int py, int px, int Hf, int Wf) { WView v = {Hv, Wv, 2, 2, 2 + py, 2 + px, Hf, Wf}; return v; }

template <int NV>
__global__ void __launch_bounds__(256) wino_input_kernel(const float* __restrict__ x, float* __restrict__ V, int B, WViews vs, int C, int TY, int TX, int off,
                                                         int reflect, int64_t planes) {
    typedef typename VecOf<NV>::T F;
    const WView v = vs.v[blockIdx.y];
    const int Cv = C / NV;
    const int64_t T = (int64_t)B * TY * TX, n = T * Cv;
    float* Vp = V + (size_t)blockIdx.y * 36 * T * C;
    unsigned short* Vq = reinterpret_cast<unsigned short*>(V) + (size_t)blockIdx.y * 36 * T * C;
    for (int64_t i = (int64_t)blockIdx.x * 256 + threadIdx.x; i < n; i += (int64_t)gridDim.x * 256) {
        const int c = (int)(i % Cv) * NV;
        const int64_t t = i / Cv;
        const int tx = (int)(t % TX), ty = (int)((t / TX) % TY), b = (int)(t / ((int64_t)TX * TY));
        F tmp[6][6];
#pragma unroll
        for (int j = 0; j < 6; ++j) {
            F d[6];
            const int ixr = 4 * tx + off + j;
            const bool xin = (unsigned)ixr < (unsigned)v.W;
            const int ix = reflect ? reflw(ixr, v.W) : (xin ? ixr : 0);
#pragma unroll
            for (int r = 0; r < 6; ++r) {
                const int iyr = 4 * ty + off + r;
                const bool yin = (unsigned)iyr < (unsigned)v.H;
                const int iy = reflect ? reflw(iyr, v.H) : (yin ? iyr : 0);
                const F val = *reinterpret_cast<const F*>(x + vaddr(v, b, iy, ix, C) + c);
                d[r] = (reflect || (xin && yin)) ? val : (F)(0.f);
            }
            F o[6];
            bt6(d, o);
#pragma unroll
            for (int r = 0; r < 6; ++r) tmp[r][j] = o[r];
        }
#pragma unroll
        for (int r = 0; r < 6; ++r) {
            F o[6];
            bt6(tmp[r], o);
#pragma unroll
            for (int j = 0; j < 6; ++j) {
                const size_t at = ((size_t)(r * 6 + j) * T + t) * C + c;
                if (planes) {
                    if constexpr (NV == 1) {
                        unsigned short h, m, l;
                        split3(o[j], h, m, l);
                        Vq[at] = h; Vq[at + planes] = m; Vq[at + 2 * planes] = l;
                    } else {
                        typedef unsigned int U __attribute__((ext_vector_type(NV / 2)));
                        U ph, pm, pl;
#pragma unroll
                        for (int e = 0; e < NV; e += 2) {
                            unsigned short h0, m0, l0, h1, m1, l1;
                            split3(o[j][e], h0, m0, l0); split3(o[j][e + 1], h1, m1, l1);
                            const unsigned int wh = h0 | ((unsigned int)h1 << 16), wm = m0 | ((unsigned int)m1 << 16), wl = l0 | ((unsigned int)l1 << 16);
                            if constexpr (NV == 2) { ph = wh; pm = wm; pl = wl; }
                            else { ph[e / 2] = wh; pm[e / 2] = wm; pl[e / 2] = wl; }
                        }
                        *reinterpret_cast<U*>(Vq + at) = ph; *reinterpret_cast<U*>(Vq + at + planes) = pm; *reinterpret_cast<U*>(Vq + at + 2 * planes) = pl;
                    }
                } else {
                    *reinterpret_cast<F*>(Vp + at) = o[j];
                }
            }
        }
    }
}

template <int NV, int SUM>
__global__ void __launch_bounds__(256) wino_output_kernel(const float* __restrict__ M, const float* __restrict__ bias, float* __restrict__ y, int B, WViews vs,
                                                          int C, int TY, int TX, int act, int accumulate, float2* __restrict__ stats) {
    constexpr int sum = SUM;
    typedef typename VecOf<NV>::T F;
    const int Cv = C / NV;
    const int64_t T = (int64_t)B * TY * TX, n = T * Cv;
    for (int64_t i = (int64_t)blockIdx.x * 256 + threadIdx.x; i < n; i += (int64_t)gridDim.x * 256) {
        const int c = (int)(i % Cv) * NV;
        const int64_t t = i / Cv;
        const int tx = (int)(t % TX), ty = (int)((t / TX) % TY), b = (int)(t / ((int64_t)TX * TY));
        const F bv = bias ? *reinterpret_cast<const F*>(bias + c) : (F)(0.f);
        F tot[SUM ? 4 : 1][4];
#pragma unroll
        for (int r = 0; r < (SUM ? 4 : 1); ++r)
#pragma unroll
            for (int j = 0; j < 4; ++j) tot[r][j] = (F)(0.f);
        F st_sh = (F)(0.f), st_s = (F)(0.f), st_q = (F)(0.f);
        const unsigned int toff = (unsigned int)t * (unsigned int)C + (unsigned int)c;
        for (int ph = 0; ph < vs.nph; ++ph) {
            const float* Mp = M + (size_t)ph * 36 * T * C;
            F tmp[4][6];
#pragma unroll
            for (int j = 0; j < 6; ++j) {
                F m[6];
#pragma unroll
                for (int r = 0; r < 6; ++r) m[r] = *reinterpret_cast<const F*>(Mp + (size_t)(r * 6 + j) * T * C + toff);
                F o[4];
                at4(m, o);
#pragma unroll
                for (int r = 0; r < 4; ++r) tmp[r][j] = o[r];
            }
#pragma unroll
            for (int r = 0; r < 4; ++r) {
                F o[4];
                at4(tmp[r], o);
#pragma unroll
                for (int j = 0; j < 4; ++j) {
                    if (sum) tot[SUM ? r : 0][j] += o[j];
                    else {
                        const WView v = vs.v[ph];
                        const int oy = 4 * ty + r, ox = 4 * tx + j;
                        if (oy < v.H && ox < v.W) {
                            F* dst = reinterpret_cast<F*>(y + vaddr(v, b, oy, ox, C) + c);
                            const F val = actv<NV>(o[j] + bv, act);
                            *dst = accumulate ? *dst + val : val;
                            if (stats) {
                                if (r == 0 && j == 0) st_sh = val;
                                const F dv = val - st_sh;
                                st_s += dv; st_q += dv * dv;
                            }
                        }
                    }
                }
            }
        }
        if (stats) {
            const F mean = st_sh + st_s * (1.f / 16.f), m2 = st_q - st_s * st_s * (1.f / 16.f);
            float2* o = stats + (size_t)t * C + c;
            if constexpr (NV == 1) o[0] = make_float2(mean, m2);
            else {
#pragma unroll
                for (int e = 0; e < NV; ++e) o[e] = make_float2(mean[e], m2[e]);
            }
        }
        if (sum) {
            const WView v = vs.v[0];
#pragma unroll
            for (int r = 0; r < 4; ++r)
#pragma unroll
                for (int j = 0; j < 4; ++j) {
                    const int oy = 4 * ty + r, ox = 4 * tx + j;
                    if (oy < v.H && ox < v.W) {
                        F* dst = reinterpret_cast<F*>(y + vaddr(v, b, oy, ox, C) + c);
                        const F val = actv<NV>(tot[SUM ? r : 0][j] + bv, act);
                        *dst = accumulate ? *dst + val : val;
                    }
                }
        }
    }
}

template <typename F>
__device__ __forceinline__ void a6(const F (&y)[4], F (&m)[6]) {
    m[0] = y[0];
    m[1] = y[0] + y[1] + y[2] + y[3];
    m[2] = y[0] - y[1] + y[2] - y[3];
    m[3] = y[0] + 2.f * y[1] + 4.f * y[2] + 8.f * y[3];
    m[4] = y[0] - 2.f * y[1] + 4.f * y[2] - 8.f * y[3];
    m[5] = y[3];
}
__device__ __forceinline__ void gt3(const float (&u)[6], float (&g)[3]) {
    g[0] = 0.25f * u[0] - (u[1] + u[2]) * (1.f / 6.f) + (u[3] + u[4]) * (1.f / 24.f);
    g[1] = (u[2] - u[1]) * (1.f / 6.f) + (u[3] - u[4]) * (1.f / 12.f);
    g[2] = -(u[1] + u[2]) * (1.f / 6.f) + (u[3] + u[4]) * (1.f / 6.f) + u[5];
}

template <int NV>
__global__ void __launch_bounds__(256) wino_outgrad_kernel(const float* __restrict__ dy, float* __restrict__ dM, float* __restrict__ bpart, int B, WViews vs,
                                                           int C, int TY, int TX) {
    typedef typename VecOf<NV>::T F;
    const WView v = vs.v[blockIdx.y];
    const int Cv = C / NV;
    const int64_t T = (int64_t)B * TY * TX;
    float* dMp = dM + (size_t)blockIdx.y * 36 * T * C;
    const int64_t gid = (int64_t)blockIdx.x * 256 + threadIdx.x, nth = (int64_t)gridDim.x * 256;
    const int c = (int)(gid % Cv) * NV;
    F bs = (F)(0.f);
    for (int64_t t = gid / Cv; t < T; t += nth / Cv) {
        const int tx = (int)(t % TX), ty = (int)((t / TX) % TY), b = (int)(t / ((int64_t)TX * TY));
        F tmp[6][4];
#pragma unroll
        for (int j = 0; j < 4; ++j) {
            F q[4];
            const int ox = 4 * tx + j;
#pragma unroll
            for (int r = 0; r < 4; ++r) {
                const int oy = 4 * ty + r;
                const bool in = oy < v.H && ox < v.W;
                q[r] = in ? *reinterpret_cast<const F*>(dy + vaddr(v, b, in ? oy : 0, in ? ox : 0, C) + c) : (F)(0.f);
                bs += q[r];
            }
            F o[6];
            a6(q, o);
#pragma unroll
            for (int r = 0; r < 6; ++r) tmp[r][j] = o[r];
        }
#pragma unroll
        for (int r = 0; r < 6; ++r) {
            F o[6];
            a6(tmp[r], o);
#pragma unroll
            for (int j = 0; j < 6; ++j) *reinterpret_cast<F*>(dMp + ((size_t)(r * 6 + j) * T + t) * C + c) = o[j];
        }
    }
    if (bpart) *reinterpret_cast<F*>(bpart + ((size_t)blockIdx.y * (nth / Cv) + gid / Cv) * C + c) = bs;
}
__global__ void __launch_bounds__(256) wino_bias_finish_kernel(const float* __restrict__ bpart, int rows, int C, float* __restrict__ db,
                                                               float* __restrict__ level2) {
    __shared__ float red[16][17];
    const int cl = threadIdx.x & 15, rg = threadIdx.x >> 4;
    const int c = blockIdx.x * 16 + cl;
    const int per_slice = (rows + gridDim.y - 1) / gridDim.y;
    const int r0 = blockIdx.y * per_slice, r1 = min(rows, r0 + per_slice);
    const int per = (max(r1 - r0, 0) + 15) >> 4;
    float s0 = 0.f, s1 = 0.f, s2 = 0.f, s3 = 0.f;
    if (c < C) {
        const int jb = r0 + rg * per, je = min(r1, jb + per);
        int j = jb;
        for (; j + 3 < je; j += 4) {
            s0 += bpart[(size_t)j * C + c]; s1 += bpart[(size_t)(j + 1) * C + c];
            s2 += bpart[(size_t)(j + 2) * C + c]; s3 += bpart[(size_t)(j + 3) * C + c];
        }
        for (; j < je; ++j) s0 += bpart[(size_t)j * C + c];
    }
    red[rg][cl] = (s0 + s1) + (s2 + s3);
    __syncthreads();
    if (threadIdx.x < 16 && c < C) {
        float t = 0.f;
#pragma unroll
        for (int g = 0; g < 16; ++g) t += red[g][threadIdx.x];
        if (level2) level2[(size_t)blockIdx.y * C + c] = t;
        else db[c] += t;
    }
}
__global__ void __launch_bounds__(256) wino_filtergrad_kernel(const float* __restrict__ dU, float* __restrict__ dw, int Co, int Ci) {
    const int64_t n = (int64_t)Co * Ci;
    dU += (size_t)blockIdx.y * 36 * n;
    dw += (size_t)blockIdx.y * 9 * n;
    for (int64_t i = (int64_t)blockIdx.x * 256 + threadIdx.x; i < n; i += (int64_t)gridDim.x * 256) {
        const int ci = (int)(i % Ci), co = (int)(i / Ci);
        float t[3][6];
#pragma unroll
        for (int j = 0; j < 6; ++j) {
            float u[6];
#pragma unroll
            for (int r = 0; r < 6; ++r) u[r] = dU[((size_t)(r * 6 + j) * Co + co) * Ci + ci];
            float o[3];
            gt3(u, o);
#pragma unroll
            for (int r = 0; r < 3; ++r) t[r][j] = o[r];
        }
#pragma unroll
        for (int r = 0; r < 3; ++r) {
            float o[3];
            gt3(t[r], o);
#pragma unroll
            for (int j = 0; j < 3; ++j) dw[((size_t)(co * 3 + r) * 3 + j) * Ci + ci] += o[j];
        }
    }
}

size_t align256(size_t b) { return (b + 255) & ~(size_t)255; }
int grid_for(int64_t n, int cap) { return (int)std::min<int64_t>(cdiv64(n, 256), cap); }
const int WINO_BIAS_BLOCKS = 1024;
const size_t WINO_BPART_BYTES = (size_t)WINO_BIAS_BLOCKS * 256 * 4 * sizeof(float);
const size_t WINO_L2_BYTES = (size_t)64 * 1024 * sizeof(float);

int launch_wino_input(const float* x, float* V, int B, const WViews& vs, int nph, int C, int TY, int TX, int off, int reflect, hipStream_t st, int64_t planes = 0) {
    const int nv = planes ? sw(SW_WINO_VEC3) : sw(SW_WINO_VEC);
    const dim3 grid(grid_for((int64_t)B * TY * TX * (C / nv), 16384), nph);
    if (nv == 4) hipLaunchKernelGGL(wino_input_kernel<4>, grid, dim3(256), 0, st, x, V, B, vs, C, TY, TX, off, reflect, planes);
    else if (nv == 2) hipLaunchKernelGGL(wino_input_kernel<2>, grid, dim3(256), 0, st, x, V, B, vs, C, TY, TX, off, reflect, planes);
    else hipLaunchKernelGGL(wino_input_kernel<1>, grid, dim3(256), 0, st, x, V, B, vs, C, TY, TX, off, reflect, planes);
    ACL_CHECK_LAUNCH("wino_input_kernel");
    return ACLGAN_OK;
}
int launch_wino_output(const float* M, const float* bias, float* y, int B, const WViews& vs, int C, int TY, int TX, int act, int accumulate, int sum,
                       hipStream_t st, float2* stats = nullptr) {
    const int nv = sw(SW_WINO_VEC);
    ACL_REQUIRE((int64_t)B * TY * TX * C < (1ll << 30), "wino_output: plane beyond 2^30 elements");
    const dim3 grid(grid_for((int64_t)B * TY * TX * (C / nv), 16384));
#define ACL_WO(NV_)                                                                                                                                     \
    do {                                                                                                                                                \
        if (sum) hipLaunchKernelGGL((wino_output_kernel<NV_, 1>), grid, dim3(256), 0, st, M, bias, y, B, vs, C, TY, TX, act, accumulate, stats);           \
        else hipLaunchKernelGGL((wino_output_kernel<NV_, 0>), grid, dim3(256), 0, st, M, bias, y, B, vs, C, TY, TX, act, accumulate, stats);             \
    } while (0)
    if (nv == 4) ACL_WO(4);
    else if (nv == 2) ACL_WO(2);
    else ACL_WO(1);
#undef ACL_WO
    ACL_CHECK_LAUNCH("wino_output_kernel");
    return ACLGAN_OK;
}
int launch_wino_outgrad(const float* dy, float* dM, float* bpart, int B, const WViews& vs, int nph, int C, int TY, int TX, hipStream_t st, int* rows) {
    const int nv = sw(SW_WINO_VEC), Cv = C / nv;
    const int mult = std::max(1, Cv / 256);
    int blocks = (int)std::max<int64_t>(1, std::min<int64_t>(WINO_BIAS_BLOCKS, cdiv64((int64_t)B * TY * TX * Cv, 256)));
    blocks = cdiv(blocks, mult) * mult;
    *rows = blocks * 256 / Cv;
    const dim3 grid(blocks, nph);
    if (nv == 4) hipLaunchKernelGGL(wino_outgrad_kernel<4>, grid, dim3(256), 0, st, dy, dM, bpart, B, vs, C, TY, TX);
    else if (nv == 2) hipLaunchKernelGGL(wino_outgrad_kernel<2>, grid, dim3(256), 0, st, dy, dM, bpart, B, vs, C, TY, TX);
    else hipLaunchKernelGGL(wino_outgrad_kernel<1>, grid, dim3(256), 0, st, dy, dM, bpart, B, vs, C, TY, TX);
    ACL_CHECK_LAUNCH("wino_outgrad_kernel");
    return ACLGAN_OK;
}
const int WINO_BIAS_SLICES = 64;
int launch_wino_bias_finish(const float* bpart, int rows, int C, float* db, float* level2, hipStream_t st) {
    if (rows >= 1024) {
        hipLaunchKernelGGL(wino_bias_finish_kernel, dim3(cdiv(C, 16), WINO_BIAS_SLICES), dim3(256), 0, st, bpart, rows, C, (float*)nullptr, level2);
        ACL_CHECK_LAUNCH("wino_bias_finish_kernel(level 1)");
        hipLaunchKernelGGL(wino_bias_finish_kernel, dim3(cdiv(C, 16), 1), dim3(256), 0, st, level2, WINO_BIAS_SLICES, C, db, (float*)nullptr);
    } else {
        hipLaunchKernelGGL(wino_bias_finish_kernel, dim3(cdiv(C, 16), 1), dim3(256), 0, st, bpart, rows, C, db, (float*)nullptr);
    }
    ACL_CHECK_LAUNCH("wino_bias_finish_kernel");
    return ACLGAN_OK;
}
bool wino_bias_ok(int C) { const int Cv = C / sw(SW_WINO_VEC); return C % sw(SW_WINO_VEC) == 0 && (256 % Cv == 0 || Cv % 256 == 0); }

WViews one_view(const WView& v) { WViews w; w.v[0] = v; w.v[1] = v; w.v[2] = v; w.v[3] = v; w.nph = 1; return w; }

float* take(char*& cur, size_t bytes) { float* p = (float*)cur; cur += align256(bytes); return p; }

}

bool conv_wino_ok(const ConvGeom& g) {
    return !sw(SW_NOWINO) && g.k == 3 && g.s == 1 && g.p == 1 && g.up == 0 && g.Ho % 4 == 0 && g.Wo % 4 == 0 && g.Ci % 16 == 0 && g.Co % 16 == 0 &&
           (int64_t)g.Ci * g.Co >= 64 * 64;
}
size_t conv_wino_u_bytes(const ConvGeom& g) {
    if (conv_wino_ok(g)) return align256((size_t)36 * g.Co * g.Ci * 6);
    if (conv_up5_wino_ok(g)) return align256((size_t)144 * g.Co * g.Ci * 6);
    if (conv_s2k4_wino_ok(g, 0) || conv_s2k4_wino_ok(g, 1)) return align256(wino_fused_s2k4_u_bytes(g.Ci, g.Co));
    return 0;
}
size_t conv_wino_scratch_bytes(const ConvGeom& g) {
    if (!conv_wino_ok(g)) return 0;
    const int64_t T = (int64_t)g.B * (g.Ho / 4) * (g.Wo / 4);
    const int cmax = std::max(g.Ci, g.Co);
    return align256((size_t)36 * g.Co * g.Ci * 6) + align256((size_t)36 * T * cmax * 6) + align256((size_t)36 * T * cmax * sizeof(float)) + 256;
}
namespace {
int wino_run(int B, int H, int W, int Cin_, int Cout_, const float* in, const float* w, int w_co, int w_ci, int flip, const float* bias, float* out,
             int act, int accumulate, int reflect, void* scratch, hipStream_t st, float2* stats = nullptr, float* keepV = nullptr) {
    const int TY = H / 4, TX = W / 4;
    const int64_t T = (int64_t)B * TY * TX;
    char* cur = (char*)scratch;
    if (!keepV && wino_fused_ok(B, H, W, Cin_, Cout_, act)) {
        bool fresh_f = true;
        float* Uf = cached_u((float*)scratch, w, uvar(flip ? 1 : 0, U_FRAG), (size_t)36 * Cout_ * Cin_ * 4, &fresh_f);
        if (fresh_f) { const int rcf = wino_fused_filter(w, Uf, w_co, w_ci, flip, st); if (rcf) return rcf; }
        return wino_fused_launch(B, H, W, Cin_, Cout_, in, Uf, bias, out, act, accumulate, reflect, stats, st);
    }
    const bool x3 = !keepV && sw(SW_WINO_X3) && gemm_x3_shape_ok((int)T, Cin_, Cout_);
    const size_t eb = x3 ? 6 : 4;
    float* U = take(cur, (size_t)36 * Cout_ * Cin_ * 6);
    float* V = take(cur, (size_t)36 * T * Cin_ * eb);
    float* M = take(cur, (size_t)36 * T * Cout_ * 4);
    if (keepV) V = keepV;
    const WViews vw = one_view(ident_view(H, W));
    const int64_t uplanes = x3 ? (int64_t)36 * Cout_ * Cin_ : 0, vplanes = x3 ? (int64_t)36 * T * Cin_ : 0;
    bool fresh = true;
    U = cached_u(U, w, uvar(flip ? 1 : 0, x3 ? U_X3 : U_PIPE), (size_t)36 * Cout_ * Cin_ * eb, &fresh);
    if (fresh) {
        hipLaunchKernelGGL(wino_filter_kernel, dim3(grid_for((int64_t)w_co * w_ci, 4096), 1), dim3(256), 0, st, w, U, w_co, w_ci, flip, uplanes,
                           (int64_t)0, (int64_t)0, (int64_t)0);
        ACL_CHECK_LAUNCH("wino_filter_kernel");
    }
    int rc = launch_wino_input(in, V, B, vw, 1, Cin_, TY, TX, -1, reflect, st, vplanes);
    if (rc) return rc;
    rc = x3 ? gemm_slices_x3(V, (size_t)vplanes * 2, U, (size_t)uplanes * 2, M, (int)T, Cin_, Cout_, 36, 0, st) : gemm_slices_f32(V, U, M, (int)T, Cin_, Cout_, 36, 0, st);
    if (rc) return rc;
    return launch_wino_output(M, bias, out, B, vw, Cout_, TY, TX, act, accumulate, 0, st, stats);
}
}
int conv_wino_u_variant(const ConvGeom& g, int dgrad, bool keepV) {
    if (!conv_wino_ok(g)) return -1;
    const int Cin_ = dgrad ? g.Co : g.Ci, Cout_ = dgrad ? g.Ci : g.Co, act = dgrad ? ACLGAN_ACT_NONE : g.act;
    const int64_t T = (int64_t)g.B * (g.Hi / 4) * (g.Wi / 4);
    if (dgrad) keepV = false;
    if (!keepV && wino_fused_ok(g.B, g.Hi, g.Wi, Cin_, Cout_, act)) return uvar(dgrad, U_FRAG);
    const bool x3 = !keepV && sw(SW_WINO_X3) && gemm_x3_shape_ok((int)T, Cin_, Cout_);
    return uvar(dgrad, x3 ? U_X3 : U_PIPE);
}
int conv_wino_prefill(const ConvGeom& g, int uv, const float* w0, int64_t w_stride, float* U0, int64_t u_stride, int count, hipStream_t st) {
    if (!conv_wino_ok(g) || uv < 0 || count < 1) return ACLGAN_EUNSUPPORTED;
    const int flip = uv & 1, layout = uv >> 4;
    if (layout == U_FRAG) return wino_fused_filter_batch(w0, w_stride, U0, u_stride, count, g.Co, g.Ci, flip, st);
    const int64_t planes = layout == U_X3 ? (int64_t)36 * g.Co * g.Ci : 0;
    hipLaunchKernelGGL(wino_filter_kernel, dim3(grid_for((int64_t)g.Co * g.Ci, 4096), count), dim3(256), 0, st, w0, U0, g.Co, g.Ci, flip, planes,
                       w_stride, u_stride, u_stride * 2);
    ACL_CHECK_LAUNCH("wino_filter_kernel(batch)");
    return ACLGAN_OK;
}
size_t conv_wino_keep_bytes(const ConvGeom& g) {
    if (!conv_wino_ok(g) || g.Co % 64 != 0 || g.Ci % 64 != 0) return 0;
    if (sw(SW_WINO_X3) && gemm_x3_shape_ok(1, g.Ci, g.Co)) return 0;
    if (wino_fused_ok(g.B, g.Hi, g.Wi, g.Ci, g.Co, g.act)) return 0;
    if (wino_wgrad_fused_ok(g)) return 0;
    return align256((size_t)36 * g.B * (g.Ho / 4) * (g.Wo / 4) * g.Ci * sizeof(float));
}
int conv_fwd_wino(const ConvGeom& g, const float* x, const float* w, const float* bias, float* y, void* scratch, hipStream_t st, float* stats, float* keepV) {
    if (!conv_wino_ok(g) || !scratch) return ACLGAN_EUNSUPPORTED;
    return wino_run(g.B, g.Hi, g.Wi, g.Ci, g.Co, x, w, g.Co, g.Ci, 0, bias, y, g.act, 0, 1, scratch, st, (float2*)stats, keepV);
}
int conv_dgrad_wino_interior(const ConvGeom& g, const float* dy, const float* w, float* dx, int accumulate, void* scratch, hipStream_t st) {
    if (!conv_wino_ok(g) || !scratch) return ACLGAN_EUNSUPPORTED;
    return wino_run(g.B, g.Hi, g.Wi, g.Co, g.Ci, dy, w, g.Co, g.Ci, 1, nullptr, dx, ACLGAN_ACT_NONE, accumulate, 0, scratch, st);
}

size_t conv_wgrad_wino_scratch_bytes(const ConvGeom& g) {
    if (!conv_wino_ok(g) || g.Co % 64 != 0 || g.Ci % 64 != 0) return 0;
    const int64_t T = (int64_t)g.B * (g.Ho / 4) * (g.Wo / 4);
    const size_t pipe = align256((size_t)36 * T * g.Ci * 4) + align256((size_t)36 * T * g.Co * 4) + align256((size_t)36 * g.Co * g.Ci * 4) +
                        align256(WINO_BPART_BYTES + WINO_L2_BYTES) + gemm_at_b_slices_scratch((int)T, g.Co, g.Ci, 36) + 256;
    return std::max(pipe, wino_wgrad_fused_scratch_bytes(g));
}
int conv_wgrad_wino(const ConvGeom& g, const float* x, const float* dy, float* dw, float* db, void* scratch, hipStream_t st, const float* haveV) {
    if (!conv_wino_ok(g) || g.Co % 64 != 0 || g.Ci % 64 != 0 || !scratch || !dw) return ACLGAN_EUNSUPPORTED;
    if (wino_wgrad_fused_ok(g)) return wino_wgrad_fused(g, x, dy, dw, db, scratch, st);
    if (!wino_bias_ok(g.Co)) return ACLGAN_EUNSUPPORTED;
    const int TY = g.Ho / 4, TX = g.Wo / 4;
    const int64_t T = (int64_t)g.B * TY * TX;
    char* cur = (char*)scratch;
    float* V = take(cur, (size_t)36 * T * g.Ci * 4);
    float* dM = take(cur, (size_t)36 * T * g.Co * 4);
    float* dU = take(cur, (size_t)36 * g.Co * g.Ci * 4);
    float* bpart = take(cur, WINO_BPART_BYTES + WINO_L2_BYTES);
    void* part = cur;
    const WViews vw = one_view(ident_view(g.Hi, g.Wi));
    int rc0 = ACLGAN_OK;
    if (haveV) V = const_cast<float*>(haveV);
    else rc0 = launch_wino_input(x, V, g.B, vw, 1, g.Ci, TY, TX, -1, 1, st);
    if (rc0) return rc0;
    int brows = 0;
    rc0 = launch_wino_outgrad(dy, dM, db ? bpart : (float*)nullptr, g.B, vw, 1, g.Co, TY, TX, st, &brows);
    if (rc0) return rc0;
    if (db) {
        const int rcb = launch_wino_bias_finish(bpart, brows, g.Co, db, bpart + WINO_BPART_BYTES / sizeof(float), st);
        if (rcb) return rcb;
    }
    const int rc = gemm_at_b_slices_f32(dM, V, dU, (int)T, g.Co, g.Ci, 36, 0, part, st);
    if (rc) return rc;
    hipLaunchKernelGGL(wino_filtergrad_kernel, dim3(grid_for((int64_t)g.Co * g.Ci, 4096), 1), dim3(256), 0, st, dU, dw, g.Co, g.Ci);
    ACL_CHECK_LAUNCH("wino_filtergrad_kernel");
    return ACLGAN_OK;
}

bool conv_up5_wino_ok(const ConvGeom& g) {
    return !sw(SW_NOWINO) && !sw(SW_NOWINOUP5) && g.up == 1 && g.k == 5 && g.p == 2 && g.s == 1 && g.Hi >= 6 && g.Wi >= 6 && g.Ci % 16 == 0 &&
           g.Co % 16 == 0 && (int64_t)g.Ci * g.Co >= 64 * 64;
}
namespace {
struct Up5Geo { int Hv, Wv, TY, TX, TYd, TXd; int64_t T, Td; WViews ph; };
Up5Geo up5_geo(const ConvGeom& g) {
    Up5Geo q;
    q.Hv = g.Hi - 2; q.Wv = g.Wi - 2;
    q.TY = cdiv(q.Hv, 4); q.TX = cdiv(q.Wv, 4); q.T = (int64_t)g.B * q.TY * q.TX;
    q.TYd = cdiv(g.Hi, 4); q.TXd = cdiv(g.Wi, 4); q.Td = (int64_t)g.B * q.TYd * q.TXd;
    for (int p = 0; p < 4; ++p) q.ph.v[p] = phase_view(q.Hv, q.Wv, p >> 1, p & 1, g.Ho, g.Wo);
    q.ph.nph = 4;
    return q;
}
}
int conv_up5_wino_u_variant(const ConvGeom& g, int dgrad, bool keepV) {
    if (!conv_up5_wino_ok(g)) return -1;
    const Up5Geo q = up5_geo(g);
    if (!dgrad) {
        if (!keepV && wino_fused_ok(g.B, g.Hi - 2, g.Wi - 2, g.Ci, g.Co, g.act, 4, 1)) return uvar(2, U_FRAG);
        return uvar(2, (!keepV && sw(SW_WINO_X3) && gemm_x3_shape_ok((int)q.T, g.Ci, g.Co)) ? U_X3 : U_PIPE);
    }
    if (wino_fused_ok(g.B, g.Hi, g.Wi, g.Co, g.Ci, ACLGAN_ACT_NONE, 1, 4)) return uvar(3, U_FRAG);
    return uvar(3, (sw(SW_WINO_X3) && gemm_x3_shape_ok((int)q.Td, g.Co, g.Ci)) ? U_X3 : U_PIPE);
}
size_t conv_up5_wino_fwd_scratch_bytes(const ConvGeom& g) {
    if (!conv_up5_wino_ok(g)) return 0;
    const Up5Geo q = up5_geo(g);
    return align256((size_t)144 * g.Co * g.Ci * 6) + align256((size_t)36 * q.T * g.Ci * 6) + align256((size_t)144 * q.T * g.Co * 4) + 256;
}
size_t conv_up5_wino_keep_bytes(const ConvGeom& g) {
    if (!conv_up5_wino_ok(g) || g.Co % 64 != 0 || g.Ci % 64 != 0) return 0;
    if (sw(SW_WINO_X3) && gemm_x3_shape_ok(1, g.Ci, g.Co)) return 0;
    if (wino_fused_ok(g.B, g.Hi - 2, g.Wi - 2, g.Ci, g.Co, g.act, 4, 1)) return 0;
    return align256((size_t)36 * up5_geo(g).T * g.Ci * sizeof(float));
}
int conv_up5_wino_fwd_phases(const ConvGeom& g, const float* x, const float* wp, const float* bias, float* y, void* scratch, hipStream_t st, float* keepV,
                             const float* wkey) {
    if (!conv_up5_wino_ok(g) || !scratch) return ACLGAN_EUNSUPPORTED;
    const Up5Geo q = up5_geo(g);
    char* cur = (char*)scratch;
    if (!keepV && wino_fused_ok(g.B, g.Hi - 2, g.Wi - 2, g.Ci, g.Co, g.act, 4, 1)) {
        bool fresh_f = true;
        float* Uf = cached_u((float*)scratch, wkey, uvar(2, U_FRAG), (size_t)144 * g.Co * g.Ci * 4, &fresh_f);
        if (fresh_f) { const int rcf = wino_fused_filter(wp, Uf, g.Co, g.Ci, 0, st, 4); if (rcf) return rcf; }
        return wino_fused_up5_fwd(g.B, g.Hi, g.Wi, g.Ci, g.Co, x, Uf, bias, y, g.Ho, g.Wo, g.act, st);
    }
    const bool x3 = !keepV && sw(SW_WINO_X3) && gemm_x3_shape_ok((int)q.T, g.Ci, g.Co);
    const size_t eb = x3 ? 6 : 4;
    float* U = take(cur, (size_t)144 * g.Co * g.Ci * 6);
    float* V = take(cur, (size_t)36 * q.T * g.Ci * 6);
    float* M = take(cur, (size_t)144 * q.T * g.Co * 4);
    if (keepV) V = keepV;
    const int64_t uplanes = x3 ? (int64_t)144 * g.Co * g.Ci : 0, vplanes = x3 ? (int64_t)36 * q.T * g.Ci : 0;
    bool fresh = true;
    U = cached_u(U, wkey, uvar(2, x3 ? U_X3 : U_PIPE), (size_t)144 * g.Co * g.Ci * eb, &fresh);
    if (fresh) {
        hipLaunchKernelGGL(wino_filter_kernel, dim3(grid_for((int64_t)g.Co * g.Ci, 4096), 4), dim3(256), 0, st, wp, U, g.Co, g.Ci, 0, uplanes,
                           (int64_t)g.Co * 9 * g.Ci, (int64_t)36 * g.Co * g.Ci, (int64_t)36 * g.Co * g.Ci);
        ACL_CHECK_LAUNCH("wino_filter_kernel(up5)");
    }
    int rc = launch_wino_input(x, V, g.B, one_view(ident_view(g.Hi, g.Wi)), 1, g.Ci, q.TY, q.TX, 0, 0, st, vplanes);
    if (rc) return rc;
    rc = x3 ? gemm_slices_x3(V, (size_t)vplanes * 2, U, (size_t)uplanes * 2, M, (int)q.T, g.Ci, g.Co, 144, 36, st) : gemm_slices_f32(V, U, M, (int)q.T, g.Ci, g.Co, 144, 36, st);
    if (rc) return rc;
    return launch_wino_output(M, bias, y, g.B, q.ph, g.Co, q.TY, q.TX, g.act, 0, 0, st);
}
size_t conv_up5_wino_dgrad_scratch_bytes(const ConvGeom& g) {
    if (!conv_up5_wino_ok(g)) return 0;
    const Up5Geo q = up5_geo(g);
    return align256((size_t)144 * g.Co * g.Ci * 6) + align256((size_t)144 * q.Td * g.Co * 6) + align256((size_t)144 * q.Td * g.Ci * 4) + 256;
}
int conv_up5_wino_dgrad_phases(const ConvGeom& g, const float* dy, const float* wp, float* dx, int accumulate, void* scratch, hipStream_t st, const float* wkey) {
    if (!conv_up5_wino_ok(g) || !scratch) return ACLGAN_EUNSUPPORTED;
    const Up5Geo q = up5_geo(g);
    char* cur = (char*)scratch;
    if (wino_fused_ok(g.B, g.Hi, g.Wi, g.Co, g.Ci, ACLGAN_ACT_NONE, 1, 4)) {
        bool fresh_f = true;
        float* Uf = cached_u((float*)scratch, wkey, uvar(3, U_FRAG), (size_t)144 * g.Co * g.Ci * 4, &fresh_f);
        if (fresh_f) { const int rcf = wino_fused_filter(wp, Uf, g.Co, g.Ci, 1, st, 4); if (rcf) return rcf; }
        return wino_fused_up5_dgrad(g.B, g.Hi, g.Wi, g.Ci, g.Co, dy, Uf, dx, g.Ho, g.Wo, accumulate, st);
    }
    const bool x3 = sw(SW_WINO_X3) && gemm_x3_shape_ok((int)q.Td, g.Co, g.Ci);
    const size_t eb = x3 ? 6 : 4;
    float* U = take(cur, (size_t)144 * g.Co * g.Ci * 6);
    float* V = take(cur, (size_t)144 * q.Td * g.Co * 6);
    float* M = take(cur, (size_t)144 * q.Td * g.Ci * 4);
    const int64_t uplanes = x3 ? (int64_t)144 * g.Co * g.Ci : 0, vplanes = x3 ? (int64_t)144 * q.Td * g.Co : 0;
    bool fresh = true;
    U = cached_u(U, wkey, uvar(3, x3 ? U_X3 : U_PIPE), (size_t)144 * g.Co * g.Ci * eb, &fresh);
    if (fresh) {
        hipLaunchKernelGGL(wino_filter_kernel, dim3(grid_for((int64_t)g.Co * g.Ci, 4096), 4), dim3(256), 0, st, wp, U, g.Co, g.Ci, 1, uplanes,
                           (int64_t)g.Co * 9 * g.Ci, (int64_t)36 * g.Co * g.Ci, (int64_t)36 * g.Co * g.Ci);
        ACL_CHECK_LAUNCH("wino_filter_kernel(up5 dgrad)");
    }
    int rc = launch_wino_input(dy, V, g.B, q.ph, 4, g.Co, q.TYd, q.TXd, -2, 0, st, vplanes);
    if (rc) return rc;
    rc = x3 ? gemm_slices_x3(V, (size_t)vplanes * 2, U, (size_t)uplanes * 2, M, (int)q.Td, g.Co, g.Ci, 144, 0, st) : gemm_slices_f32(V, U, M, (int)q.Td, g.Co, g.Ci, 144, 0, st);
    if (rc) return rc;
    WViews dst = one_view(ident_view(g.Hi, g.Wi));
    dst.nph = 4;
    return launch_wino_output(M, nullptr, dx, g.B, dst, g.Ci, q.TYd, q.TXd, ACLGAN_ACT_NONE, accumulate, 1, st);
}
size_t conv_up5_wino_wgrad_scratch_bytes(const ConvGeom& g) {
    if (!conv_up5_wino_ok(g) || g.Co % 64 != 0 || g.Ci % 64 != 0) return 0;
    const Up5Geo q = up5_geo(g);
    return align256((size_t)36 * q.T * g.Ci * 4) + align256((size_t)144 * q.T * g.Co * 4) + align256((size_t)144 * g.Co * g.Ci * 4) +
           align256(4 * WINO_BPART_BYTES + WINO_L2_BYTES) + gemm_at_b_slices_scratch((int)q.T, g.Co, g.Ci, 144) + 256;
}
int conv_up5_wino_wgrad_phases(const ConvGeom& g, const float* x, const float* dy, float* dwp, float* db, void* scratch, hipStream_t st, const float* haveV) {
    if (!conv_up5_wino_ok(g) || g.Co % 64 != 0 || g.Ci % 64 != 0 || !scratch || !wino_bias_ok(g.Co)) return ACLGAN_EUNSUPPORTED;
    const Up5Geo q = up5_geo(g);
    char* cur = (char*)scratch;
    float* V = take(cur, (size_t)36 * q.T * g.Ci * 4);
    float* dM = take(cur, (size_t)144 * q.T * g.Co * 4);
    float* dU = take(cur, (size_t)144 * g.Co * g.Ci * 4);
    float* bpart = take(cur, 4 * WINO_BPART_BYTES + WINO_L2_BYTES);
    void* part = cur;
    int rc0 = ACLGAN_OK;
    if (haveV) V = const_cast<float*>(haveV);
    else rc0 = launch_wino_input(x, V, g.B, one_view(ident_view(g.Hi, g.Wi)), 1, g.Ci, q.TY, q.TX, 0, 0, st);
    if (rc0) return rc0;
    int brows = 0;
    rc0 = launch_wino_outgrad(dy, dM, db ? bpart : (float*)nullptr, g.B, q.ph, 4, g.Co, q.TY, q.TX, st, &brows);
    if (rc0) return rc0;
    if (db) {
        const int rcb = launch_wino_bias_finish(bpart, 4 * brows, g.Co, db, bpart + 4 * WINO_BPART_BYTES / sizeof(float), st);
        if (rcb) return rcb;
    }
    const int rc = gemm_at_b_slices_f32(dM, V, dU, (int)q.T, g.Co, g.Ci, 144, 36, part, st);
    if (rc) return rc;
    hipLaunchKernelGGL(wino_filtergrad_kernel, dim3(grid_for((int64_t)g.Co * g.Ci, 4096), 4), dim3(256), 0, st, dU, dwp, g.Co, g.Ci);
    ACL_CHECK_LAUNCH("wino_filtergrad_kernel(up5)");
    return ACLGAN_OK;
}

bool conv_s2k4_wino_ok(const ConvGeom& g, int which) {
    if (!sw(SW_WINO_S2K4) || sw(SW_NOWINO) || g.k != 4 || g.s != 2 || g.p != 1 || g.up != 0) return false;
    if (which == 1 && sw(SW_DETERMINISTIC)) return false;
    return wino_fused_s2k4_ok(g.B, g.Hi, g.Wi, g.Ci, g.Co, which ? ACLGAN_ACT_NONE : g.act, which);
}
size_t conv_s2k4_wino_scratch_bytes(const ConvGeom& g) {
    return (conv_s2k4_wino_ok(g, 0) || conv_s2k4_wino_ok(g, 1)) ? align256(wino_fused_s2k4_u_bytes(g.Ci, g.Co)) + 256 : 0;
}
int conv_fwd_s2k4_wino(const ConvGeom& g, const float* x, const float* w, const float* bias, float* y, void* scratch, hipStream_t st, float* stats) {
    if (!conv_s2k4_wino_ok(g, 0) || !scratch) return ACLGAN_EUNSUPPORTED;
    bool fresh = true;
    float* Uf = cached_u((float*)scratch, w, uvar(0, U_FRAG), wino_fused_s2k4_u_bytes(g.Ci, g.Co), &fresh);
    if (fresh) { const int rcf = wino_fused_filter_s2k4(w, Uf, g.Co, g.Ci, 0, st); if (rcf) return rcf; }
    return wino_fused_s2k4_fwd(g.B, g.Hi, g.Wi, g.Ci, g.Co, x, Uf, bias, y, g.act, (float2*)stats, st);
}
int conv_dgrad_s2k4_wino_interior(const ConvGeom& g, const float* dy, const float* w, float* dx, int accumulate, void* scratch, hipStream_t st) {
    if (!conv_s2k4_wino_ok(g, 1) || !scratch) return ACLGAN_EUNSUPPORTED;
    bool fresh = true;
    float* Uf = cached_u((float*)scratch, w, uvar(1, U_FRAG), wino_fused_s2k4_u_bytes(g.Ci, g.Co), &fresh);
    if (fresh) { const int rcf = wino_fused_filter_s2k4(w, Uf, g.Co, g.Ci, 1, st); if (rcf) return rcf; }
    return wino_fused_s2k4_dgrad(g.B, g.Hi, g.Wi, g.Ci, g.Co, dy, Uf, dx, accumulate, st);
}

}
```

acl-gan_amd/csrc/conv_wino_fused.hip:

```cpp
#include "common.h"
#include <cstdlib>
#include <algorithm>
#include <cmath>
#include <type_traits>

namespace aclgan {

const WinoUCache* wino_ucache();

namespace {

typedef float f32x2 __attribute__((ext_vector_type(2)));
typedef float f32x4 __attribute__((ext_vector_type(4)));
typedef float f32x16 __attribute__((ext_vector_type(16)));
typedef unsigned int u32x4 __attribute__((ext_vector_type(4)));

constexpr int TBX = 8, TBY = 4;
constexpr int PR = 4 * TBY + 2, PC = 4 * TBX + 2, NPIX = PR * PC;
constexpr int RS = 42;
constexpr int QS = PR * RS;
constexpr int NBC = 64;
constexpr unsigned int OOBV = 0x7ffffff0u;
constexpr int M_BYTES = 36 * 32 * 32 * 4;

struct WfP {
    const float* x; const float* Uf; const float* bias; float* y; float2* stats;
    int B, Cin, Cout;
    int IH, IW, ivs, ivy0, ivx0, IHS, IWS, off, reflect;
    int nkph;
    int kph_xoff[4];
    int uphase;
    int OH, OW, ovs, OHS, OWS, ovy0[4], ovx0[4];
    int TY, TX, NBY, NBX, act, accumulate, ncb, ntb, xcdmap;
    long long xbytes, ubytes;
};


__device__ __forceinline__ int reflf(int v, int n) {
    v = v < 0 ? -v : v;
    return v >= n ? 2 * (n - 1) - v : v;
}
__device__ __forceinline__ float actf(float v, int act) {
    if (act == ACLGAN_ACT_RELU) return v > 0.f ? v : 0.f;
    if (act == ACLGAN_ACT_LRELU) return v > 0.f ? v : 0.2f * v;
    if (act == ACLGAN_ACT_TANH) return tanhf(v);
    return v;
}

__device__ __forceinline__ void at4f(const float (&m)[6], float (&y)[4]) {
    y[0] = m[0] + m[1] + m[2] + m[3] + m[4];
    y[1] = m[1] - m[2] + 2.f * (m[3] - m[4]);
    y[2] = m[1] + m[2] + 4.f * (m[3] + m[4]);
    y[3] = m[1] - m[2] + 8.f * (m[3] - m[4]) + m[5];
}
__device__ __forceinline__ void g6f(const float (&g)[3], float (&u)[6]) {
    u[0] = 0.25f * g[0];
    u[1] = -(g[0] + g[1] + g[2]) * (1.f / 6.f);
    u[2] = -(g[0] - g[1] + g[2]) * (1.f / 6.f);
    u[3] = g[0] * (1.f / 24.f) + g[1] * (1.f / 12.f) + g[2] * (1.f / 6.f);
    u[4] = g[0] * (1.f / 24.f) - g[1] * (1.f / 12.f) + g[2] * (1.f / 6.f);
    u[5] = g[2];
}

__device__ __forceinline__ int s2k4_tap(int mode, int par, int t) {
    if (mode == 1) return par == 0 ? (t == 0 ? -1 : (t == 1 ? 1 : 3)) : (t == 0 ? 0 : (t == 1 ? 2 : -1));
    return par == 0 ? (t == 0 ? 3 : (t == 1 ? 1 : -1)) : (t == 0 ? -1 : (t == 1 ? 2 : 0));
}
__global__ void __launch_bounds__(256) wino_filter_frag_kernel(const float* __restrict__ w, float* __restrict__ Uf, int Co, int Ci, int flip,
                                                               int64_t wstr, int64_t ustr, int mode) {
    const int R = flip ? Ci : Co, K = flip ? Co : Ci, KQ = K >> 2;
    const int64_t n = (int64_t)R * K;
    w += (size_t)blockIdx.y * wstr;
    Uf += (size_t)blockIdx.y * ustr;
    const int py = (int)(blockIdx.y >> 1) & 1, px = (int)blockIdx.y & 1;
    for (int64_t idx = (int64_t)blockIdx.x * 256 + threadIdx.x; idx < n; idx += (int64_t)gridDim.x * 256) {
        const int row = (int)(idx % R), kk = (int)(idx / R);
        const int co = flip ? kk : row, ci = flip ? row : kk;
        float t[6][3];
#pragma unroll
        for (int kx = 0; kx < 3; ++kx) {
            float c[3];
#pragma unroll
            for (int ky = 0; ky < 3; ++ky) {
                if (mode == 0) {
                    const int sy = flip ? 2 - ky : ky, sx = flip ? 2 - kx : kx;
                    c[ky] = w[((size_t)(co * 3 + sy) * 3 + sx) * Ci + ci];
                } else {
                    const int sy = s2k4_tap(mode, py, ky), sx = s2k4_tap(mode, px, kx);
                    c[ky] = (sy >= 0 && sx >= 0) ? w[((size_t)(co * 4 + sy) * 4 + sx) * Ci + ci] : 0.f;
                }
            }
            float o[6];
            g6f(c, o);
#pragma unroll
            for (int a = 0; a < 6; ++a) t[a][kx] = o[a];
        }
        const int cb = row >> 6, j = (row >> 5) & 1, l31 = row & 31;
        const int kq = kk >> 2, h = (kk >> 1) & 1, e = kk & 1;
        float* base = Uf + ((size_t)cb * KQ + kq) * (4 * 9 * 2 * 128) + (size_t)(h * 32 + l31) * 4 + j * 2 + e;
#pragma unroll
        for (int a = 0; a < 6; ++a) {
            float o[6];
            g6f(t[a], o);
#pragma unroll
            for (int jf = 0; jf < 6; ++jf) {
                const int g = (a / 3) * 2 + jf / 3, fi = (a % 3) * 3 + jf % 3;
                base[(size_t)(g * 9 + fi) * 256] = o[jf];
            }
        }
    }
}

__device__ __forceinline__ f32x2 opaque2(float v) {
    f32x2 r = {v, v};
    asm volatile("" : "+v"(r));
    return r;
}
__device__ __forceinline__ f32x2 fma2(f32x2 a, f32x2 b, f32x2 c) { return __builtin_elementwise_fma(a, b, c); }
__device__ __forceinline__ f32x4 fma4(f32x4 a, f32x4 b, f32x4 c) { return __builtin_elementwise_fma(a, b, c); }
__device__ __forceinline__ f32x4 opaque4(float v) {
    f32x4 r = {v, v, v, v};
    asm volatile("" : "+v"(r));
    return r;
}
struct BtK { f32x2 k4, k5n, k4n, k2, k2n; };
template <int W>
__device__ __forceinline__ void bt3(const BtK& k, const f32x2 (&x)[5], f32x2& o0, f32x2& o1, f32x2& o2) {
    if (W == 0) {
        const f32x2 pp = fma2(k.k4n, x[2], x[4]), qq = fma2(k.k4, x[1], -x[3]);
        o0 = fma2(k.k4, x[0], fma2(k.k5n, x[2], x[4]));
        o1 = pp - qq;
        o2 = pp + qq;
    } else {
        const f32x2 pp = x[3] - x[1], sd = x[2] - x[0];
        o0 = fma2(k.k2, sd, pp);
        o1 = fma2(k.k2n, sd, pp);
        o2 = fma2(k.k4, x[0], fma2(k.k5n, x[2], x[4]));
    }
}

constexpr int KC = 8;
constexpr int NP = 5;
constexpr int XBUF = (KC / 2) * QS;
constexpr int UD = 17;

template <int WI, int WJ, int ABL>
__device__ __forceinline__ void wf_wave(const WfP& p, char* smem, const int lane, const int cb, const unsigned int (&go)[NP], const int (&lub)[NP],
                                        f32x16 (&acc)[9][2]) {
    const int nchp = p.Cin / KC, nch = nchp * p.nkph, KQp = p.Cin >> 2;
    const int wave = WI * 2 + WJ;
    const int l31 = lane & 31, h = lane >> 5;
    const int lanebase = (h * QS + 4 * (l31 >> 3) * RS + (l31 & 7)) * 8;
    const __amdgpu_buffer_rsrc_t rx = __builtin_amdgcn_make_buffer_rsrc(const_cast<float*>(p.x), 0, (int)p.xbytes, 0x00020000);
    const __amdgpu_buffer_rsrc_t ru = __builtin_amdgcn_make_buffer_rsrc(const_cast<float*>(p.Uf), 0, (int)p.ubytes, 0x00020000);
    const int uvo = lane * 16;
    const int ustep = 4 * 9 * 2 * 64 * 8;
    const int ubase = (cb * KQp * 4 + wave) * (9 * 2 * 64 * 8) + (int)blockIdx.y * p.uphase;
    auto xoff = [&](int chunk) __attribute__((always_inline)) {
        int c = min(chunk, nch - 1), xo = 0;
        if (c >= nchp) { c -= nchp; xo = p.kph_xoff[1]; if (c >= nchp) { c -= nchp; xo = p.kph_xoff[2]; if (c >= nchp) { c -= nchp; xo = p.kph_xoff[3]; } } }
        return __builtin_amdgcn_readfirstlane(c * (KC * 4) + xo);
    };
    auto uoff = [&](int kq) __attribute__((always_inline)) {
        int q = min(kq, 2 * nch - 1), so = ubase;
        if (q >= KQp) { q -= KQp; so += p.uphase; if (q >= KQp) { q -= KQp; so += p.uphase; if (q >= KQp) { q -= KQp; so += p.uphase; } } }
        return __builtin_amdgcn_readfirstlane(so + q * ustep);
    };
    const BtK bk = {opaque2(4.f), opaque2(-5.f), opaque2(-4.f), opaque2(2.f), opaque2(-2.f)};

    f32x4 xr[NP];
    auto xissue = [&](int xso, int i) __attribute__((always_inline)) {
        xr[i] = __builtin_bit_cast(f32x4, __builtin_amdgcn_raw_buffer_load_b128(rx, go[i], xso, 0));
    };
    auto xwrite = [&](int par, int i) __attribute__((always_inline)) {
        char* dst = smem + par * XBUF * 8 + lub[i];
        *reinterpret_cast<f32x2*>(dst) = (f32x2){xr[i].x, xr[i].y};
        *reinterpret_cast<f32x2*>(dst + QS * 8) = (f32x2){xr[i].z, xr[i].w};
    };
    auto xslot = [&](int xso, int par, int wsl) __attribute__((always_inline)) {
        if (wsl >= 12 && wsl - 12 < NP) xwrite(par, wsl - 12);
        if (wsl < NP) xissue(xso, wsl);
    };

    f32x2 u[2][9][2];
    auto uload = [&](int so, int par2, int fi) __attribute__((always_inline)) {
        const f32x4 v = __builtin_bit_cast(f32x4, __builtin_amdgcn_raw_buffer_load_b128(ru, uvo + (fi & 3) * 1024, so + (fi >> 2) * 4096, 0));
        u[par2][fi][0] = (f32x2){v.x, v.y};
        u[par2][fi][1] = (f32x2){v.z, v.w};
    };
    f32x2 d[5][5];
    auto rdcol = [&](int par, int ss, int c) __attribute__((always_inline)) {
        const int cc = WJ + c;
        const char* src = smem + par * XBUF * 8 + lanebase;
#pragma unroll
        for (int r = 0; r < 5; ++r) d[c][r] = *reinterpret_cast<const f32x2*>(src + (2 * ss * QS + (WI + r) * RS + (cc & 3) * 9 + (cc >> 2)) * 8);
    };
    auto transform = [&](f32x2 (&V)[9]) __attribute__((always_inline)) {
        f32x2 t[3][5];
#pragma unroll
        for (int c = 0; c < 5; ++c) bt3<WI>(bk, d[c], t[0][c], t[1][c], t[2][c]);
#pragma unroll
        for (int il = 0; il < 3; ++il) bt3<WJ>(bk, t[il], V[il * 3], V[il * 3 + 1], V[il * 3 + 2]);
    };
    auto mfma1 = [&](int fi, int j, float a, float b) __attribute__((always_inline)) {
        if (fi == 8) asm volatile("v_mfma_f32_32x32x2_f32 %0, %1, %2, %0" : "+v"(acc[fi][j]) : "v"(a), "v"(b));
        else acc[fi][j] = __builtin_amdgcn_mfma_f32_32x32x2f32(a, b, acc[fi][j], 0, 0, 0);
    };

    {
        f32x4 xp[NP];
#pragma unroll
        for (int i = 0; i < NP; ++i) xp[i] = __builtin_bit_cast(f32x4, __builtin_amdgcn_raw_buffer_load_b128(rx, go[i], 0, 0));
#pragma unroll
        for (int fi = 0; fi < 9; ++fi) uload(uoff(0), 0, fi);
#pragma unroll
        for (int fi = 0; fi < 8; ++fi) uload(uoff(1), 1, fi);
#pragma unroll
        for (int i = 0; i < NP; ++i) {
            *reinterpret_cast<f32x2*>(smem + lub[i]) = (f32x2){xp[i].x, xp[i].y};
            *reinterpret_cast<f32x2*>(smem + lub[i] + QS * 8) = (f32x2){xp[i].z, xp[i].w};
        }
        const int xso1 = xoff(1);
#pragma unroll
        for (int i = 0; i < NP; ++i) xissue(xso1, i);
    }
    __syncthreads();
    f32x2 Va[9], Vb[9];
#pragma unroll
    for (int c = 0; c < 5; ++c) rdcol(0, 0, c);
    transform(Va);
    if (ABL & 1) {
#pragma unroll
        for (int i = 0; i < 9; ++i) Vb[i] = Va[i];
    }

    auto substep = [&](int ch, int par, int ss, f32x2 (&Vc)[9], f32x2 (&Vn)[9]) __attribute__((always_inline)) {
        const int kq = ch * 2 + ss;
        const int npar = ss == 0 ? par : par ^ 1, ns = ss == 0 ? 1 : 0;
        const int schunk = ss == 1 ? ch + 2 : ch + 1, spar = ss == 1 ? par : par ^ 1;
        const int wbase = ss == 1 ? 0 : 9;
        const int so_nxt = uoff(kq + 1), so_nx2 = uoff(kq + 2), xso = xoff(schunk);
#pragma unroll
        for (int s = 0; s < 9; ++s) {
            mfma1(s, 0, Vc[s].x, u[ss][s][0].x);
            mfma1(s, 1, Vc[s].x, u[ss][s][1].x);
            mfma1(s, 0, Vc[s].y, u[ss][s][0].y);
            mfma1(s, 1, Vc[s].y, u[ss][s][1].y);
            if (!(ABL & 2)) uload(s == 0 ? so_nxt : so_nx2, s == 0 ? (ss ^ 1) : ss, (s + UD) % 9);
            if (s < 5 && !(ABL & 1)) rdcol(npar, ns, s);
            if (!(ABL & 4)) xslot(xso, spar, wbase + s);
            __builtin_amdgcn_sched_barrier(0);
        }
        if (!(ABL & 1)) transform(Vn);
        __builtin_amdgcn_sched_barrier(0);
        if (ss == 0 && !(ABL & 8)) __syncthreads();
    };
    for (int ch = 0; ch < ((ABL & 16) ? 0 : nch); ch += 2) {
        substep(ch, 0, 0, Va, Vb);
        substep(ch, 0, 1, Vb, Va);
        substep(ch + 1, 1, 0, Va, Vb);
        substep(ch + 1, 1, 1, Vb, Va);
    }
}

template <int ABL = 0>
__global__ void __launch_bounds__(256) __attribute__((amdgpu_waves_per_eu(1, 1))) wino_fused_kernel(WfP p) {
    constexpr int JN = KC / 4;
    constexpr int NSLOT = NPIX * JN;
    constexpr int MAIN_BYTES = 2 * XBUF * 8;
    __shared__ __attribute__((aligned(16))) char smem[MAIN_BYTES > M_BYTES ? MAIN_BYTES : M_BYTES];

    const int tid = threadIdx.x, lane = tid & 63;
    const int wave = __builtin_amdgcn_readfirstlane(tid >> 6);
    int cb, tb;
    {
        const int bid = blockIdx.x;
        if (p.xcdmap) { const int per = 8 / p.ncb, xcd = bid & 7, idx = bid >> 3; cb = xcd / per; tb = idx * per + xcd % per; }
        else { cb = bid % p.ncb; tb = bid / p.ncb; }
    }
    const int bx = tb % p.NBX, by = (tb / p.NBX) % p.NBY, b = tb / (p.NBX * p.NBY);
    const int ty0 = by * TBY, tx0 = bx * TBX;
    const int gph = blockIdx.y;
    const int ovy0 = gph == 0 ? p.ovy0[0] : (gph == 1 ? p.ovy0[1] : (gph == 2 ? p.ovy0[2] : p.ovy0[3]));
    const int ovx0 = gph == 0 ? p.ovx0[0] : (gph == 1 ? p.ovx0[1] : (gph == 2 ? p.ovx0[2] : p.ovx0[3]));

    unsigned int go[NP];
    int lub[NP];
#pragma unroll
    for (int i = 0; i < NP; ++i) {
        const int s = i * 256 + tid;
        go[i] = OOBV;
        lub[i] = 36 * 8;
        if (s < NSLOT) {
            const int pix = s / JN, j = s - pix * JN;
            const int r = pix / PC, c = pix - r * PC;
            int iy = 4 * ty0 + p.off + r, ix = 4 * tx0 + p.off + c;
            if (p.reflect == 1) { iy = reflf(iy, p.IH); ix = reflf(ix, p.IW); }
            else if (p.reflect == 2) { iy = min(max(iy, 0), p.IH - 1); ix = min(max(ix, 0), p.IW - 1); }
            if ((unsigned)iy < (unsigned)p.IH && (unsigned)ix < (unsigned)p.IW)
                go[i] = (unsigned int)((((size_t)b * p.IHS + p.ivy0 + p.ivs * iy) * p.IWS + p.ivx0 + p.ivs * ix) * p.Cin * 4 + j * 16);
            lub[i] = (2 * j * QS + r * RS + (c & 3) * 9 + (c >> 2)) * 8;
        }
    }

    f32x16 acc[9][2];
#pragma unroll
    for (int i = 0; i < 9; ++i)
#pragma unroll
        for (int j = 0; j < 2; ++j)
#pragma unroll
            for (int r = 0; r < 16; ++r) acc[i][j][r] = 0.f;

    if (ABL & 512) p.y[tid] = 0.f;
    if (wave == 0) wf_wave<0, 0, ABL>(p, smem, lane, cb, go, lub, acc);
    else if (wave == 1) wf_wave<0, 1, ABL>(p, smem, lane, cb, go, lub, acc);
    else if (wave == 2) wf_wave<1, 0, ABL>(p, smem, lane, cb, go, lub, acc);
    else wf_wave<1, 1, ABL>(p, smem, lane, cb, go, lub, acc);

    float* Ms = reinterpret_cast<float*>(smem);
    const int wi = wave >> 1, wj = wave & 1;
    const int l31 = lane & 31, h = lane >> 5;
    const int tl = tid >> 4, c4 = tid & 15;
    const int n = cb * NBC + c4 * 4;
    const f32x4 bv = p.bias ? *reinterpret_cast<const f32x4*>(p.bias + n) : (f32x4)(0.f);
    const float slope = p.act == ACLGAN_ACT_RELU ? 0.f : (p.act == ACLGAN_ACT_LRELU ? 0.2f : 1.f);
    const f32x4 k2 = opaque4(2.f), k4 = opaque4(4.f), k8 = opaque4(8.f);
#pragma unroll
    for (int P = 0; P < ((ABL & 512) ? 0 : 2); ++P) {
        __syncthreads();
#pragma unroll
        for (int fi = 0; fi < 9; ++fi) {
            const int f = (3 * wi + fi / 3) * 6 + 3 * wj + fi % 3;
#pragma unroll
            for (int j = 0; j < 2; ++j)
#pragma unroll
                for (int r8 = 0; r8 < 8; ++r8) {
                    const int tr = (r8 & 3) + 8 * (r8 >> 2) + 4 * h;
                    Ms[(f * 16 + tr) * 64 + j * 32 + l31] = acc[fi][j][8 * P + r8];
                }
        }
        __syncthreads();
        if (ABL & 256) continue;
        const int tile = 16 * P + tl;
        const int ty = ty0 + (tile >> 3), tx = tx0 + (tile & 7);
        const bool live = ty < p.TY && tx < p.TX;
        const int rows = live ? min(4, p.OH - 4 * ty) : 0, cols = live ? min(4, p.OW - 4 * tx) : 0;
        float* ybase = p.y + (((size_t)b * p.OHS + ovy0 + p.ovs * 4 * (live ? ty : 0)) * p.OWS + ovx0 + p.ovs * 4 * (live ? tx : 0)) * p.Cout + n;
        const size_t yrs = (size_t)p.ovs * p.OWS * p.Cout, ycs = (size_t)p.ovs * p.Cout;
        auto at4v = [&](const f32x4 (&m)[6], f32x4& y0, f32x4& y1, f32x4& y2, f32x4& y3) __attribute__((always_inline)) {
            const f32x4 s12 = m[1] + m[2], d12 = m[1] - m[2], s34 = m[3] + m[4], d34 = m[3] - m[4];
            y0 = m[0] + s12 + s34;
            y1 = fma4(k2, d34, d12);
            y2 = fma4(k4, s34, s12);
            y3 = fma4(k8, d34, d12) + m[5];
        };
        f32x4 tmp[4][6];
#pragma unroll
        for (int jf = 0; jf < 6; ++jf) {
            f32x4 m[6];
#pragma unroll
            for (int i = 0; i < 6; ++i) m[i] = *reinterpret_cast<const f32x4*>(Ms + ((i * 6 + jf) * 16 + tl) * 64 + c4 * 4);
            at4v(m, tmp[0][jf], tmp[1][jf], tmp[2][jf], tmp[3][jf]);
        }
        auto finish = [&](auto ACT_, auto ACC_, auto STATS_) __attribute__((always_inline)) {
            constexpr bool ACT = decltype(ACT_)::value, ACC = decltype(ACC_)::value, STATS = decltype(STATS_)::value;
            f32x4 sh = (f32x4)(0.f), s1 = (f32x4)(0.f), s2 = (f32x4)(0.f);
#pragma unroll
            for (int a = 0; a < 4; ++a) {
                f32x4 o[4], old[4];
                if (ACC) {
#pragma unroll
                    for (int bb = 0; bb < 4; ++bb) old[bb] = (a < rows && bb < cols) ? *reinterpret_cast<const f32x4*>(ybase + a * yrs + bb * ycs) : (f32x4)(0.f);
                }
                at4v(tmp[a], o[0], o[1], o[2], o[3]);
#pragma unroll
                for (int bb = 0; bb < 4; ++bb) {
                    f32x4 val = o[bb] + bv;
                    if (ACT) {
#pragma unroll
                        for (int e = 0; e < 4; ++e) val[e] = fmaxf(val[e], 0.f) + slope * fminf(val[e], 0.f);
                    }
                    if (ACC) val += old[bb];
                    if (a < rows && bb < cols && !(ABL & 128)) *reinterpret_cast<f32x4*>(ybase + a * yrs + bb * ycs) = val;
                    if (STATS) {
                        if (a == 0 && bb == 0) sh = val;
                        const f32x4 dv = val - sh;
                        s1 += dv; s2 += dv * dv;
                    }
                }
            }
            if (STATS && live) {
                const f32x4 mean = sh + s1 * (1.f / 16.f), m2 = s2 - s1 * s1 * (1.f / 16.f);
                float* so = reinterpret_cast<float*>(p.stats + (((size_t)b * p.TY + ty) * p.TX + tx) * p.Cout + n);
                *reinterpret_cast<f32x4*>(so) = (f32x4){mean[0], m2[0], mean[1], m2[1]};
                *reinterpret_cast<f32x4*>(so + 4) = (f32x4){mean[2], m2[2], mean[3], m2[3]};
            }
        };
        using T_ = std::true_type; using F_ = std::false_type;
        const bool actq = p.act != ACLGAN_ACT_NONE, accq = p.accumulate != 0, stq = p.stats != nullptr;
        if (!actq && !accq && stq) finish(F_{}, F_{}, T_{});
        else if (!actq && !accq && !stq) finish(F_{}, F_{}, F_{});
        else if (!actq && accq && !stq) finish(F_{}, T_{}, F_{});
        else if (accq) { if (stq) finish(T_{}, T_{}, T_{}); else finish(T_{}, T_{}, F_{}); }
        else { if (stq) finish(T_{}, F_{}, T_{}); else finish(T_{}, F_{}, F_{}); }
    }
}

thread_local int tl_wino_force = 0;

}

int wino_fused_force(int on) { const int old = tl_wino_force; tl_wino_force = on; return old; }

bool wino_fused_ok(int B, int H, int W, int Cin_, int Cout_, int act, int gph, int kph) {
    const int m = tl_wino_force > 0 ? 2 : (sw(SW_WINO_FUSED) & 15);
    if (m == 0) return false;
    const bool shape = act != ACLGAN_ACT_TANH && Cin_ % (2 * KC) == 0 && Cout_ % NBC == 0 && (long long)4 * 36 * Cin_ * Cout_ * 4 < 0x7fffffe0ll && H >= 4 && W >= 4 &&
                       (long long)B * (2 * H + 8) * (2 * W + 8) * std::max(Cin_, Cout_) * 4 < 0x7fffffe0ll;
    if (!shape || m == 2) return shape;
    const int TY = cdiv(H, 4), TX = cdiv(W, 4);
    const double nwg = (double)B * cdiv(TY, TBY) * cdiv(TX, TBX) * (Cout_ / NBC) * gph;
    const double t_fused = (10.0 + 83.0 * (double)Cin_ * kph / 256.0) * std::ceil(nwg / 256.0);
    const double t_pipe = 30.0 + 0.0488 * (double)B * TY * TX * gph * kph * ((double)Cin_ * Cout_ / 65536.0);
    return t_fused <= t_pipe;
}
size_t wino_fused_u_bytes(int Cin_, int Cout_) { return (size_t)36 * Cin_ * Cout_ * sizeof(float); }

int wino_fused_filter(const float* w, float* Uf, int Co, int Ci, int flip, hipStream_t st, int nph) {
    const int64_t n = (int64_t)Co * Ci;
    hipLaunchKernelGGL(wino_filter_frag_kernel, dim3((int)std::min<int64_t>(cdiv64(n, 256), 4096), nph), dim3(256), 0, st, w, Uf, Co, Ci, flip,
                       (int64_t)Co * 9 * Ci, (int64_t)36 * n, 0);
    ACL_CHECK_LAUNCH("wino_filter_frag_kernel");
    return ACLGAN_OK;
}
int wino_fused_filter_batch(const float* w0, int64_t w_stride, float* Uf0, int64_t u_stride, int count, int Co, int Ci, int flip, hipStream_t st) {
    const int64_t n = (int64_t)Co * Ci;
    hipLaunchKernelGGL(wino_filter_frag_kernel, dim3((int)std::min<int64_t>(cdiv64(n, 256), 1024), count), dim3(256), 0, st, w0, Uf0, Co, Ci, flip,
                       w_stride, u_stride, 0);
    ACL_CHECK_LAUNCH("wino_filter_frag_kernel(batch)");
    return ACLGAN_OK;
}

namespace {
int wino_fused_go(WfP& p, int ngph, hipStream_t st) {
    p.TY = cdiv(p.OH, 4); p.TX = cdiv(p.OW, 4); p.NBY = cdiv(p.TY, TBY); p.NBX = cdiv(p.TX, TBX);
    p.ncb = p.Cout / NBC; p.ntb = p.B * p.NBY * p.NBX;
    p.xcdmap = (p.ncb <= 8 && 8 % p.ncb == 0 && p.ntb % (8 / p.ncb) == 0) ? 1 : 0;
    p.xbytes = (long long)p.B * p.IHS * p.IWS * p.Cin * 4;
    p.uphase = 36 * p.Cin * p.Cout * 4;
    p.ubytes = (long long)p.uphase * p.nkph * ngph;
    const dim3 grid(p.ncb * p.ntb, ngph);
    const int abl = sw(SW_WINO_FUSED) >> 4;
#ifdef ACLGAN_FUSED_ABLATION
#define ACL_ABL(A_) else if (abl == A_) hipLaunchKernelGGL((wino_fused_kernel<A_>), grid, dim3(256), 0, st, p);
    if (abl == 0) hipLaunchKernelGGL(wino_fused_kernel<0>, grid, dim3(256), 0, st, p);
    ACL_ABL(1) ACL_ABL(2) ACL_ABL(4) ACL_ABL(8) ACL_ABL(14) ACL_ABL(15) ACL_ABL(31) ACL_ABL(128)
#undef ACL_ABL
    else
#endif
    { (void)abl; hipLaunchKernelGGL(wino_fused_kernel<0>, grid, dim3(256), 0, st, p); }
    ACL_CHECK_LAUNCH("wino_fused_kernel");
    return ACLGAN_OK;
}
}

int wino_fused_launch(int B, int H, int W, int Cin_, int Cout_, const float* in, const float* Uf, const float* bias, float* out, int act, int accumulate,
                      int reflect, float2* stats, hipStream_t st) {
    if (!wino_fused_ok(B, H, W, Cin_, Cout_, act) || H % 4 != 0 || W % 4 != 0) return ACLGAN_EUNSUPPORTED;
    WfP p;
    p.x = in; p.Uf = Uf; p.bias = bias; p.y = out; p.stats = stats;
    p.B = B; p.Cin = Cin_; p.Cout = Cout_;
    p.IH = H; p.IW = W; p.ivs = 1; p.ivy0 = 0; p.ivx0 = 0; p.IHS = H; p.IWS = W; p.off = -1; p.reflect = reflect;
    p.nkph = 1;
    for (int i = 0; i < 4; ++i) { p.kph_xoff[i] = 0; p.ovy0[i] = 0; p.ovx0[i] = 0; }
    p.OH = H; p.OW = W; p.ovs = 1; p.OHS = H; p.OWS = W;
    p.act = act; p.accumulate = accumulate;
    return wino_fused_go(p, 1, st);
}

int wino_fused_up5_fwd(int B, int Hi, int Wi, int Cin_, int Cout_, const float* x, const float* Uf, const float* bias, float* y, int Hf, int Wf, int act,
                       hipStream_t st) {
    if (!wino_fused_ok(B, Hi - 2, Wi - 2, Cin_, Cout_, act, 4, 1) || Hi < 6 || Wi < 6) return ACLGAN_EUNSUPPORTED;
    WfP p;
    p.x = x; p.Uf = Uf; p.bias = bias; p.y = y; p.stats = nullptr;
    p.B = B; p.Cin = Cin_; p.Cout = Cout_;
    p.IH = Hi; p.IW = Wi; p.ivs = 1; p.ivy0 = 0; p.ivx0 = 0; p.IHS = Hi; p.IWS = Wi; p.off = 0; p.reflect = 0;
    p.nkph = 1;
    for (int i = 0; i < 4; ++i) { p.kph_xoff[i] = 0; p.ovy0[i] = 2 + (i >> 1); p.ovx0[i] = 2 + (i & 1); }
    p.OH = Hi - 2; p.OW = Wi - 2; p.ovs = 2; p.OHS = Hf; p.OWS = Wf;
    p.act = act; p.accumulate = 0;
    return wino_fused_go(p, 4, st);
}
int wino_fused_up5_dgrad(int B, int Hi, int Wi, int Cin_, int Cout_, const float* dy, const float* Uf, float* dx, int Hf, int Wf, int accumulate, hipStream_t st) {
    if (!wino_fused_ok(B, Hi, Wi, Cout_, Cin_, ACLGAN_ACT_NONE, 1, 4) || Hi < 6 || Wi < 6) return ACLGAN_EUNSUPPORTED;
    WfP p;
    p.x = dy; p.Uf = Uf; p.bias = nullptr; p.y = dx; p.stats = nullptr;
    p.B = B; p.Cin = Cout_; p.Cout = Cin_;
    p.IH = Hi - 2; p.IW = Wi - 2; p.ivs = 2; p.ivy0 = 2; p.ivx0 = 2; p.IHS = Hf; p.IWS = Wf; p.off = -2; p.reflect = 0;
    p.nkph = 4;
    for (int i = 0; i < 4; ++i) { p.kph_xoff[i] = ((i >> 1) * Wf + (i & 1)) * Cout_ * 4; p.ovy0[i] = 0; p.ovx0[i] = 0; }
    p.OH = Hi; p.OW = Wi; p.ovs = 1; p.OHS = Hi; p.OWS = Wi;
    p.act = ACLGAN_ACT_NONE; p.accumulate = accumulate;
    return wino_fused_go(p, 1, st);
}

int wino_fused_filter_s2k4(const float* w, float* Uf, int Co, int Ci, int dgrad, hipStream_t st) {
    const int64_t n = (int64_t)Co * Ci;
    hipLaunchKernelGGL(wino_filter_frag_kernel, dim3((int)std::min<int64_t>(cdiv64(n, 256), 4096), 4), dim3(256), 0, st, w, Uf, Co, Ci, dgrad ? 1 : 0,
                       (int64_t)0, (int64_t)36 * n, dgrad ? 2 : 1);
    ACL_CHECK_LAUNCH("wino_filter_frag_kernel(s2k4)");
    return ACLGAN_OK;
}
bool wino_fused_s2k4_ok(int B, int Hi, int Wi, int Ci, int Co, int act, int dgrad) {
    const int m = tl_wino_force > 0 ? 2 : (sw(SW_WINO_FUSED) & 15);
    if (m == 0) return false;
    const int Cin_ = dgrad ? Co : Ci, Cout_ = dgrad ? Ci : Co;
    const bool shape = act != ACLGAN_ACT_TANH && Hi % 2 == 0 && Wi % 2 == 0 && Hi >= 8 && Wi >= 8 && Cin_ % (2 * KC) == 0 && Cout_ % NBC == 0 &&
                       (long long)4 * 36 * Ci * Co * 4 < 0x7fffffe0ll && (long long)B * Hi * Wi * std::max(Ci, Co) * 4 < 0x7fffffe0ll;
    if (!shape || m == 2) return shape;
    const int OH = Hi / 2, OW = Wi / 2, TY = cdiv(OH, 4), TX = cdiv(OW, 4);
    const int gph = dgrad ? 4 : 1, kph = dgrad ? 1 : 4;
    const double nwg = (double)B * cdiv(TY, TBY) * cdiv(TX, TBX) * (Cout_ / NBC) * gph;
    const double t_fused = (10.0 + 83.0 * (double)Cin_ * kph / 256.0) * std::ceil(nwg / 256.0);
    const double flop = 2.0 * B * OH * OW * 16.0 * Ci * Co;
    const double nblk = (double)cdiv(B * OH * OW, 128) * cdiv(dgrad ? Ci : Co, 128) * (dgrad ? 4 : 1);
    const double t_direct = 8.0 + flop / (nblk >= 256 ? 120e6 : 60e6 + 60e6 * nblk / 256.0);
    return t_fused <= 0.95 * t_direct;
}
size_t wino_fused_s2k4_u_bytes(int Ci, int Co) { return (size_t)144 * Ci * Co * sizeof(float); }

int wino_fused_s2k4_fwd(int B, int Hi, int Wi, int Ci, int Co, const float* x, const float* Uf, const float* bias, float* y, int act, float2* stats,
                        hipStream_t st) {
    if (!wino_fused_s2k4_ok(B, Hi, Wi, Ci, Co, act, 0)) return ACLGAN_EUNSUPPORTED;
    const int OH = Hi / 2, OW = Wi / 2;
    if (stats && (OH % 4 != 0 || OW % 4 != 0)) return ACLGAN_EUNSUPPORTED;
    WfP p;
    p.x = x; p.Uf = Uf; p.bias = bias; p.y = y; p.stats = stats;
    p.B = B; p.Cin = Ci; p.Cout = Co;
    p.IH = OH; p.IW = OW; p.ivs = 2; p.ivy0 = 0; p.ivx0 = 0; p.IHS = Hi; p.IWS = Wi; p.off = -1; p.reflect = 2;
    p.nkph = 4;
    for (int i = 0; i < 4; ++i) { p.kph_xoff[i] = ((i >> 1) * Wi + (i & 1)) * Ci * 4; p.ovy0[i] = 0; p.ovx0[i] = 0; }
    p.OH = OH; p.OW = OW; p.ovs = 1; p.OHS = OH; p.OWS = OW;
    p.act = act; p.accumulate = 0;
    return wino_fused_go(p, 1, st);
}
int wino_fused_s2k4_dgrad(int B, int Hi, int Wi, int Ci, int Co, const float* dy, const float* Uf, float* dx, int accumulate, hipStream_t st) {
    if (!wino_fused_s2k4_ok(B, Hi, Wi, Ci, Co, ACLGAN_ACT_NONE, 1)) return ACLGAN_EUNSUPPORTED;
    const int OH = Hi / 2, OW = Wi / 2;
    WfP p;
    p.x = dy; p.Uf = Uf; p.bias = nullptr; p.y = dx; p.stats = nullptr;
    p.B = B; p.Cin = Co; p.Cout = Ci;
    p.IH = OH; p.IW = OW; p.ivs = 1; p.ivy0 = 0; p.ivx0 = 0; p.IHS = OH; p.IWS = OW; p.off = -1; p.reflect = 0;
    p.nkph = 1;
    for (int i = 0; i < 4; ++i) { p.kph_xoff[i] = 0; p.ovy0[i] = i >> 1; p.ovx0[i] = i & 1; }
    p.OH = OH; p.OW = OW; p.ovs = 2; p.OHS = Hi; p.OWS = Wi;
    p.act = ACLGAN_ACT_NONE; p.accumulate = accumulate;
    return wino_fused_go(p, 4, st);
}

}
```

acl-gan_amd/csrc/switches.h:

```cpp
#pragma once
#include <atomic>

namespace aclgan {

enum SwitchId {
    SW_LANES, SW_U_BATCH, SW_NORM_MASK, SW_MLP_FUSED, SW_FAULT_AT, SW_ENC_REUSE,
    SW_GLDS_TILE, SW_WINO_X3, SW_WINO_FUSED, SW_WINO_WGRAD_FUSED, SW_WINO_S2K4, SW_DGRAD16S_DIRECT, SW_FWD16_PATCH,
    SW_DETERMINISTIC,
    SW_NOFAST, SW_NOUP5, SW_SPLIT_NWG,
    SW_NOWGKC, SW_NOUP5DGRAD,
    SW_NOSTATFUSE, SW_NOKEEPV, SW_NODIRECT,
    SW_NOWGRAD16S, SW_WGRAD16S_MINPIX, SW_NOGLDS16,
    SW_NOSMALL, SW_NOTHIN,
    SW_NOWINO, SW_NOWINOUP5, SW_WINO_VEC, SW_WINO_VEC3,
    SW_ROCTX, SW_NOUCACHE, SW_ACT16, SW_CO16, SW_SIDE_STREAM, SW_KEEPV_BUDGET_GB,
    SW_COUNT
};

const long long SW_BIAS = 1ll << 32;
extern std::atomic<long long> g_switches[SW_COUNT];
int sw_latch(SwitchId id);
inline int sw(SwitchId id) {
    const long long e = g_switches[id].load(std::memory_order_relaxed);
    return e ? (int)(e - SW_BIAS) : sw_latch(id);
}
double sw_real(SwitchId id);
int sw_set(SwitchId id, int v);

long long tuning_epoch();

}
```

acl-gan_amd/csrc/switches.hip:

```cpp
#include <string.h>
#include "common.h"

#include <climits>
#include <cmath>
#include <cstdlib>

namespace aclgan {

namespace {

enum Rule {
    R_INT,
    R_BOOL,
    R_NOT,
    R_CLAMP,
    R_RANGE,
    R_LOW4,
    R_ONEOF,
};
enum { SETTABLE = 1,
       EMPTY_UNSET = 2 };

struct Switch {
    const char* key;
    const char* env;
    int dflt;
    Rule rule;
    int lo, hi;
    int flags;
    double (*parse)(const char*);
};

double parse_real(const char* s) { return atof(s); }
const int VEC_124 = (1 << 1) | (1 << 2) | (1 << 4);

const Switch kSwitches[SW_COUNT] = {
    {"lanes",             "ACLGAN_LANES",             3,  R_CLAMP, 1, 3,       SETTABLE | EMPTY_UNSET, nullptr},
    {"u_batch",           "ACLGAN_U_BATCH",           1,  R_BOOL,  0, 0,       SETTABLE | EMPTY_UNSET, nullptr},
    {"norm_mask",         "ACLGAN_NORM_MASK",         1,  R_BOOL,  0, 0,       SETTABLE | EMPTY_UNSET, nullptr},
    {"mlp_fused",         "ACLGAN_MLP_FUSED",         1,  R_BOOL,  0, 0,       SETTABLE | EMPTY_UNSET, nullptr},
    {"fault_at",          nullptr,                    -1, R_INT,   0, 0,       SETTABLE, nullptr},
    {"enc_reuse",         nullptr,                    1,  R_BOOL,  0, 0,       SETTABLE, nullptr},
    {"glds_tile",         "ACLGAN_GLDS_TILE",         0,  R_CLAMP, 0, INT_MAX, SETTABLE, nullptr},
    {"wino_x3",           "ACLGAN_WINO_X3",           0,  R_BOOL,  0, 0,       SETTABLE, nullptr},
    {"wino_fused",        "ACLGAN_WINO_FUSED",        1,  R_LOW4,  0, 2,       SETTABLE, nullptr},
    {"wino_wgrad_fused",  "ACLGAN_WINO_WGRAD_FUSED",  1,  R_RANGE, 0, 2,       SETTABLE, nullptr},
    {"wino_s2k4",         "ACLGAN_NOWINOS2",          1,  R_NOT,   0, 0,       SETTABLE, nullptr},
    {"dgrad16s_direct",   "ACLGAN_DGRAD16S_DIRECT",   0,  R_BOOL,  0, 0,       SETTABLE, nullptr},
    {"fwd16_patch",       "ACLGAN_FWD16_PATCH",       1,  R_LOW4,  0, 2,       SETTABLE, nullptr},
    {"deterministic",     "ACLGAN_DETERMINISTIC",     0,  R_BOOL,  0, 0,       0, nullptr},
    {"nofast",            "ACLGAN_NOFAST",            0,  R_BOOL,  0, 0,       0, nullptr},
    {"noup5",             "ACLGAN_NOUP5",             0,  R_BOOL,  0, 0,       0, nullptr},
    {"split_nwg",         "ACLGAN_SPLIT_NWG",         256, R_INT,  0, 0,       0, nullptr},
    {"nowgkc",            "ACLGAN_NOWGKC",            0,  R_BOOL,  0, 0,       0, nullptr},
    {"noup5dgrad",        "ACLGAN_NOUP5DGRAD",        0,  R_BOOL,  0, 0,       0, nullptr},
    {"nostatfuse",        "ACLGAN_NOSTATFUSE",        0,  R_BOOL,  0, 0,       0, nullptr},
    {"nokeepv",           "ACLGAN_NOKEEPV",           0,  R_BOOL,  0, 0,       0, nullptr},
    {"nodirect",          "ACLGAN_NODIRECT",          0,  R_BOOL,  0, 0,       0, nullptr},
    {"nowgrad16s",        "ACLGAN_NOWGRAD16S",        0,  R_BOOL,  0, 0,       0, nullptr},
    {"wgrad16s_minpix",   "ACLGAN_WGRAD16S_MINPIX",   64, R_INT,   0, 0,       0, nullptr},
    {"noglds16",          "ACLGAN_NOGLDS16",          0,  R_BOOL,  0, 0,       0, nullptr},
    {"nosmall",           "ACLGAN_NOSMALL",           0,  R_BOOL,  0, 0,       0, nullptr},
    {"nothin",            "ACLGAN_NOTHIN",            0,  R_BOOL,  0, 0,       0, nullptr},
    {"nowino",            "ACLGAN_NOWINO",            0,  R_BOOL,  0, 0,       0, nullptr},
    {"nowinoup5",         "ACLGAN_NOWINOUP5",         0,  R_BOOL,  0, 0,       0, nullptr},
    {"wino_vec",          "ACLGAN_WINO_VEC",          2,  R_ONEOF, VEC_124, 0, 0, nullptr},
    {"wino_vec3",         "ACLGAN_WINO_VEC3",         2,  R_ONEOF, VEC_124, 0, 0, nullptr},
    {"roctx",             "ACLGAN_ROCTX",             0,  R_BOOL,  0, 0,       0, nullptr},
    {"noucache",          "ACLGAN_NOUCACHE",          0,  R_BOOL,  0, 0,       0, nullptr},
    {"act16",             "ACLGAN_ACT16",             1,  R_BOOL,  0, 0,       0, nullptr},
    {"co16",              "ACLGAN_CO16",              1,  R_BOOL,  0, 0,       0, nullptr},
    {"side_stream",       "ACLGAN_SIDE_STREAM",       1,  R_BOOL,  0, 0,       0, nullptr},
    {"keepv_budget_gb",   "ACLGAN_KEEPV_BUDGET_GB",   64, R_INT,   0, 0,       0, parse_real},
};

int normalise(const Switch& s, int v, bool from_env) {
    switch (s.rule) {
    case R_INT: return v;
    case R_BOOL: return v ? 1 : 0;
    case R_NOT: return (v ? 1 : 0) ^ (from_env ? 1 : 0);
    case R_CLAMP: return v < s.lo ? s.lo : v > s.hi ? s.hi : v;
    case R_RANGE: return (v < s.lo || v > s.hi) ? s.dflt : v;
    case R_LOW4: return (v < 0 || (v & 15) < s.lo || (v & 15) > s.hi) ? s.dflt : v;
    case R_ONEOF: return (v >= 0 && v < 31 && ((s.lo >> v) & 1)) ? v : s.dflt;
    }
    return v;
}

std::atomic<double> g_real[SW_COUNT];
std::atomic<long long> g_tuning_epoch{0};

int find(const char* key) {
    for (int i = 0; i < SW_COUNT; ++i)
        if (!strcmp(key, kSwitches[i].key)) return i;
    return -1;
}

}

std::atomic<long long> g_switches[SW_COUNT];

int sw_latch(SwitchId id) {
    const Switch& s = kSwitches[id];
    const char* e = s.env ? getenv(s.env) : nullptr;
    if (e && !*e && (s.flags & EMPTY_UNSET)) e = nullptr;
    int v = s.dflt;
    if (e && s.parse) {
        const double r = s.parse(e);
        g_real[id].store(r, std::memory_order_relaxed);
        v = std::isfinite(r) && std::fabs(r) < 2e9 ? (int)r : 0;
    } else if (e) {
        v = normalise(s, atoi(e), true);
    } else if (s.parse) {
        g_real[id].store(s.dflt, std::memory_order_relaxed);
    }
    long long expected = 0;
    return g_switches[id].compare_exchange_strong(expected, v + SW_BIAS, std::memory_order_release, std::memory_order_acquire) ? v : (int)(expected - SW_BIAS);
}

double sw_real(SwitchId id) {
    if (!g_switches[id].load(std::memory_order_acquire)) sw_latch(id);
    return g_real[id].load(std::memory_order_relaxed);
}

int sw_set(SwitchId id, int v) {
    sw(id);
    return (int)(g_switches[id].exchange(normalise(kSwitches[id], v, false) + SW_BIAS) - SW_BIAS);
}

long long tuning_epoch() { return g_tuning_epoch.load(); }

}

using namespace aclgan;

extern "C" {

int aclgan_set_deterministic(int on) { sw_set(SW_DETERMINISTIC, on); return ACLGAN_OK; }
int aclgan_get_deterministic(void) { return sw(SW_DETERMINISTIC); }

int aclgan_tuning(const char* key, int value, int* previous) {
    ACL_REQUIRE(key, "aclgan_tuning: null key");
    const int i = find(key);
    if (i < 0) { set_error("aclgan_tuning: unknown key '%s'", key); return ACLGAN_EINVAL; }
    if (!(kSwitches[i].flags & SETTABLE)) { set_error("aclgan_tuning: key '%s' is read-only (set %s before the first use instead)", key, kSwitches[i].env); return ACLGAN_EINVAL; }
    const int old = sw_set((SwitchId)i, value);
    ++g_tuning_epoch;
    if (previous) *previous = old;
    return ACLGAN_OK;
}
int aclgan_tuning_get(const char* key, long long* value) {
    ACL_REQUIRE(key && value, "aclgan_tuning_get: null argument");
    if (!strcmp(key, "epoch")) { *value = tuning_epoch(); return ACLGAN_OK; }
    if (!strcmp(key, "enc_reuse_hits")) { *value = g_enc_reuse_hits.load(); return ACLGAN_OK; }
    const int i = find(key);
    if (i < 0) { set_error("aclgan_tuning_get: unknown key '%s'", key); return ACLGAN_EINVAL; }
    *value = sw((SwitchId)i);
    return ACLGAN_OK;
}
int aclgan_set_tuning(const char* key, int value) {
    int old = 0;
    return aclgan_tuning(key, value, &old) == ACLGAN_OK ? old : -1;
}

}
```

Before: 104.2.

## Handle up5 conv borders via clamped Winograd plus dedicated MFMA border-correction kernels

Adds an up5_border mode for the upsample+5x5 conv. The Winograd path now covers the full image using clamp-padding, and small MFMA kernels apply difference-based corrections on the one-pixel output border for forward and weight-gradient. This replaces the earlier ring GEMM pass over the border band. The new switch defaults to 1, which enables only the wgrad border path for 64-aligned channels; the forward border needs level 2. The cost is extra kernel launches and atomic-free but read-modify-write accumulation into y/dw, plus more geometry and workspace logic.

```diff
diff --git a/acl-gan_amd/csrc/common.h b/acl-gan_amd/csrc/common.h
--- a/acl-gan_amd/csrc/common.h
+++ b/acl-gan_amd/csrc/common.h
@@ -87,6 +87,7 @@
 int conv_dgrad_wino_interior(const ConvGeom& g, const float* dy, const float* w, float* dx, int accumulate, void* scratch, hipStream_t st);
 size_t conv_wgrad_wino_scratch_bytes(const ConvGeom& g);
 bool conv_up5_wino_ok(const ConvGeom& g);
+bool conv_up5_border(const ConvGeom& g, int which);
 size_t conv_up5_wino_fwd_scratch_bytes(const ConvGeom& g);
 size_t conv_up5_wino_dgrad_scratch_bytes(const ConvGeom& g);
 size_t conv_up5_wino_wgrad_scratch_bytes(const ConvGeom& g);
@@ -116,7 +117,7 @@
 int wino_fused_filter(const float* w, float* Uf, int Co, int Ci, int flip, hipStream_t st, int nph = 1);
 int wino_fused_launch(int B, int H, int W, int Cin_, int Cout_, const float* in, const float* Uf, const float* bias, float* out, int act, int accumulate,
                       int reflect, float2* stats, hipStream_t st);
-int wino_fused_up5_fwd(int B, int Hi, int Wi, int Cin_, int Cout_, const float* x, const float* Uf, const float* bias, float* y, int Hf, int Wf, int act,
+int wino_fused_up5_fwd(int B, int Hi, int Wi, int Cin_, int Cout_, const float* x, const float* Uf, const float* bias, float* y, int Hf, int Wf, int act, int border,
                        hipStream_t st);
 bool wino_wgrad_fused_ok(const ConvGeom& g);
 size_t wino_wgrad_fused_scratch_bytes(const ConvGeom& g);
diff --git a/acl-gan_amd/csrc/conv_fast.hip b/acl-gan_amd/csrc/conv_fast.hip
--- a/acl-gan_amd/csrc/conv_fast.hip
+++ b/acl-gan_amd/csrc/conv_fast.hip
@@ -808,6 +808,183 @@
 }
 
 
+__device__ __forceinline__ int up5_ct(int j, int W, int w) { return j < 0 ? -1 - j : (j >= W ? w - 1 - (j - W) : j >> 1); }
+__device__ __forceinline__ int up5_re(int i, int H) { return min(max(i, 0), H - 1) >> 1; }
+
+constexpr int UB_NW = 16, UB_U = 4;
+struct Up5BfP { const float* x; const float* w; float* y; int B, h, w_, Ci, Co, H, W, nTW, nTH, tiles; };
+__global__ void __launch_bounds__(UB_NW * 64) up5_border_fwd_kernel(Up5BfP p) {
+    __shared__ float red[UB_NW][32][65];
+    __shared__ long long yoff[32];
+    const int tid = threadIdx.x, lane = tid & 63, wave = __builtin_amdgcn_readfirstlane(tid >> 6), l31 = lane & 31, kh = lane >> 5;
+    int t = blockIdx.x;
+    const int b = t / p.tiles;
+    t -= b * p.tiles;
+    int side, i0;
+    if (t < 2 * p.nTW) { side = t / p.nTW; i0 = (t - side * p.nTW) * 32; }
+    else { t -= 2 * p.nTW; const int s2 = t / p.nTH; side = 2 + s2; i0 = 1 + (t - s2 * p.nTH) * 32; }
+    const int co0 = blockIdx.y * 64;
+    const bool rowt = side < 2;
+    const int idx = i0 + l31;
+    const bool live = rowt ? idx < p.W : idx < p.H - 1;
+    const int r = rowt ? (side ? p.H - 1 : 0) : (live ? idx : 1);
+    const int c = rowt ? (live ? idx : 0) : (side == 2 ? 0 : p.W - 1);
+    if (tid < 32) yoff[tid] = live ? ((long long)(b * p.H + r) * p.W + c) * p.Co : -1ll;
+    const bool has_l = rowt && i0 == 0, has_r = rowt && p.W - 1 >= i0 && p.W - 1 < i0 + 32;
+    const int nact = 5 + (has_l ? 5 : 0) + (has_r ? 5 : 0), nch = p.Ci >> 3, nitems = nact * nch;
+    const bool nok0 = co0 + l31 < p.Co, nok1 = co0 + 32 + l31 < p.Co;
+    const float* wrow0 = p.w + (size_t)min(co0 + l31, p.Co - 1) * 25 * p.Ci + kh * 4;
+    const float* wrow1 = p.w + (size_t)min(co0 + 32 + l31, p.Co - 1) * 25 * p.Ci + kh * 4;
+    f32x16 acc[2];
+#pragma unroll
+    for (int j = 0; j < 2; ++j)
+#pragma unroll
+        for (int e = 0; e < 16; ++e) acc[j][e] = 0.f;
+    for (int it0 = wave * UB_U; it0 < nitems; it0 += UB_NW * UB_U) {
+        f32x4 a[UB_U], a2[UB_U], bw[UB_U], bw1[UB_U];
+        bool onu[UB_U];
+#pragma unroll
+        for (int u = 0; u < UB_U; ++u) {
+            const int item = min(it0 + u, nitems - 1);
+            {
+                const int ta = item / nch, cc = (item - ta * nch) * 8;
+                const int tt = ta < 5 ? ta : ((has_l && ta < 10) ? ta : 10 + ta - (has_l ? 10 : 5));
+                const int gq = tt / 5, k = tt - 5 * gq;
+                int oa, ob, tap;
+                bool on;
+                if (rowt && gq == 0) {
+                    const int j = up5_ct(c + k - 2, p.W, p.w_);
+                    oa = ((b * p.h + (side ? p.h - 2 : 1)) * p.w_ + j) * p.Ci; ob = ((b * p.h + (side ? p.h - 1 : 0)) * p.w_ + j) * p.Ci;
+                    on = live; tap = (side ? 20 : 0) + k;
+                } else {
+                    const bool left = rowt ? gq == 1 : side == 2;
+                    const int i = up5_re(r + k - 2, p.H);
+                    oa = ((b * p.h + i) * p.w_ + (left ? 1 : p.w_ - 2)) * p.Ci; ob = ((b * p.h + i) * p.w_ + (left ? 0 : p.w_ - 1)) * p.Ci;
+                    on = live && (!rowt || c == (left ? 0 : p.W - 1)); tap = 5 * k + (left ? 0 : 4);
+                }
+                a[u] = *reinterpret_cast<const f32x4*>(p.x + oa + kh * 4 + cc); a2[u] = *reinterpret_cast<const f32x4*>(p.x + ob + kh * 4 + cc);
+                bw[u] = *reinterpret_cast<const f32x4*>(wrow0 + (size_t)tap * p.Ci + cc);
+                bw1[u] = *reinterpret_cast<const f32x4*>(wrow1 + (size_t)tap * p.Ci + cc);
+                onu[u] = on && it0 + u < nitems;
+            }
+        }
+#pragma unroll
+        for (int u = 0; u < UB_U; ++u) {
+            const f32x4 z4 = {0.f, 0.f, 0.f, 0.f};
+            a[u] = onu[u] ? a[u] - a2[u] : z4;
+            bw[u] = nok0 ? bw[u] : z4; bw1[u] = nok1 ? bw1[u] : z4;
+        }
+#pragma unroll
+        for (int u = 0; u < UB_U; ++u)
+#pragma unroll
+            for (int e = 0; e < 4; ++e) {
+                acc[0] = __builtin_amdgcn_mfma_f32_32x32x2f32(a[u][e], bw[u][e], acc[0], 0, 0, 0);
+                acc[1] = __builtin_amdgcn_mfma_f32_32x32x2f32(a[u][e], bw1[u][e], acc[1], 0, 0, 0);
+            }
+    }
+#pragma unroll
+    for (int j = 0; j < 2; ++j)
+#pragma unroll
+        for (int e = 0; e < 16; ++e) red[wave][(e & 3) + 8 * (e >> 2) + 4 * kh][j * 32 + l31] = acc[j][e];
+    __syncthreads();
+    const int n = tid & 63;
+#pragma unroll
+    for (int i = 0; i < 2; ++i) {
+        const int m = (tid >> 6) + 16 * i;
+        const long long o = yoff[m];
+        if (o >= 0 && co0 + n < p.Co) {
+            float sum = 0.f;
+#pragma unroll
+            for (int wv = 0; wv < UB_NW; ++wv) sum += red[wv][m][n];
+            p.y[o + co0 + n] += sum;
+        }
+    }
+}
+
+struct Up5BwP { const float* x; const float* dy; float* dw; int B, h, w_, Ci, Co, H, W, tiles_n; };
+__global__ void __launch_bounds__(UB_NW * 64) up5_border_wgrad_kernel(Up5BwP p) {
+    __shared__ float red[UB_NW][32][33];
+    const int tid = threadIdx.x, lane = tid & 63, wave = __builtin_amdgcn_readfirstlane(tid >> 6), l31 = lane & 31, kh = lane >> 5;
+    const int co0 = (blockIdx.x / p.tiles_n) * 32, ci0 = (blockIdx.x % p.tiles_n) * 32;
+    const int tp = blockIdx.y;
+    const int ky = tp < 5 ? 0 : (tp < 10 ? 4 : (tp < 13 ? tp - 9 : tp - 12));
+    const int kx = tp < 5 ? tp : (tp < 10 ? tp - 5 : (tp < 13 ? 0 : 4));
+    f32x16 acc;
+#pragma unroll
+    for (int e = 0; e < 16; ++e) acc[e] = 0.f;
+    for (int pass = 0; pass < 2; ++pass) {
+        if (pass == 0 ? (ky != 0 && ky != 4) : (kx != 0 && kx != 4)) continue;
+        const int L = pass == 0 ? p.W : p.H, nu = (L + 7) >> 3, nunits = p.B * nu;
+        const int sy = pass == 0 ? p.Co : p.W * p.Co, sx = pass == 0 ? p.Ci : p.w_ * p.Ci, shift = pass == 0 ? kx - 2 : ky - 2;
+        const int ry = pass == 0 ? (ky ? p.H - 1 : 0) * p.W * p.Co : (kx ? p.W - 1 : 0) * p.Co;
+        const int ra = pass == 0 ? (ky ? p.h - 2 : 1) * p.w_ * p.Ci : (kx ? p.w_ - 2 : 1) * p.Ci;
+        const int rb = pass == 0 ? (ky ? p.h - 1 : 0) * p.w_ * p.Ci : (kx ? p.w_ - 1 : 0) * p.Ci;
+        const int isy = p.H * p.W * p.Co, isx = p.h * p.w_ * p.Ci;
+        for (int un0 = wave * UB_U; un0 < nunits; un0 += UB_NW * UB_U) {
+            float a[UB_U][4], d[UB_U][4], d2[UB_U][4];
+#pragma unroll
+            for (int u = 0; u < UB_U; ++u) {
+                const int un = min(un0 + u, nunits - 1), b = un / nu, qe = (un - b * nu) * 8;
+                const int imgy = b * isy + ry, imga = b * isx + ra, imgb = b * isx + rb;
+#pragma unroll
+                for (int s = 0; s < 4; ++s) {
+                    int oy[2], oa[2], ob[2];
+#pragma unroll
+                    for (int hh = 0; hh < 2; ++hh) {
+                        const int q = min(qe + 2 * s + hh, L - 1);
+                        const int idx = pass == 0 ? up5_ct(q + shift, p.W, p.w_) : up5_re(q + shift, p.H);
+                        oy[hh] = imgy + q * sy; oa[hh] = imga + idx * sx; ob[hh] = imgb + idx * sx;
+                    }
+                    a[u][s] = p.dy[(kh ? oy[1] : oy[0]) + co0 + l31];
+                    d[u][s] = p.x[(kh ? oa[1] : oa[0]) + ci0 + l31]; d2[u][s] = p.x[(kh ? ob[1] : ob[0]) + ci0 + l31];
+                }
+            }
+#pragma unroll
+            for (int u = 0; u < UB_U; ++u) {
+                const int un = un0 + u, qe = (un % nu) * 8;
+#pragma unroll
+                for (int s = 0; s < 4; ++s) {
+                    const bool ok = un < nunits && qe + 2 * s + kh < L;
+                    a[u][s] = ok ? a[u][s] : 0.f; d[u][s] = ok ? d[u][s] - d2[u][s] : 0.f;
+                }
+            }
+#pragma unroll
+            for (int u = 0; u < UB_U; ++u)
+#pragma unroll
+                for (int s = 0; s < 4; ++s) acc = __builtin_amdgcn_mfma_f32_32x32x2f32(a[u][s], d[u][s], acc, 0, 0, 0);
+        }
+    }
+#pragma unroll
+    for (int e = 0; e < 16; ++e) red[wave][(e & 3) + 8 * (e >> 2) + 4 * kh][l31] = acc[e];
+    __syncthreads();
+    const int n = tid & 31, m = tid >> 5;
+    float sum = 0.f;
+#pragma unroll
+    for (int wv = 0; wv < UB_NW; ++wv) sum += red[wv][m][n];
+    p.dw[((size_t)(co0 + m) * 25 + ky * 5 + kx) * p.Ci + ci0 + n] += sum;
+}
+
+int up5_border_fwd(const ConvGeom& g, const float* x, const float* w, float* y, hipStream_t st) {
+    ACL_REQUIRE((int64_t)g.B * g.Hi * g.Wi * g.Ci < (1ll << 31), "up5_border_fwd: input beyond 2^31 elements");
+    Up5BfP p;
+    p.x = x; p.w = w; p.y = y; p.B = g.B; p.h = g.Hi; p.w_ = g.Wi; p.Ci = g.Ci; p.Co = g.Co; p.H = g.Ho; p.W = g.Wo;
+    p.nTW = cdiv(g.Wo, 32); p.nTH = cdiv(g.Ho - 2, 32); p.tiles = 2 * p.nTW + 2 * p.nTH;
+    hipLaunchKernelGGL(up5_border_fwd_kernel, dim3(g.B * p.tiles, cdiv(g.Co, 64)), dim3(UB_NW * 64), 0, st, p);
+    ACL_CHECK_LAUNCH("up5_border_fwd_kernel");
+    return ACLGAN_OK;
+}
+int up5_border_wgrad(const ConvGeom& g, const float* x, const float* dy, float* dw, hipStream_t st) {
+    ACL_REQUIRE(g.Co % 32 == 0 && g.Ci % 32 == 0, "up5_border_wgrad: channel counts must be multiples of 32");
+    ACL_REQUIRE((int64_t)g.B * g.Ho * g.Wo * g.Co < (1ll << 31) && (int64_t)g.B * g.Hi * g.Wi * g.Ci < (1ll << 31), "up5_border_wgrad: tensor beyond 2^31 elements");
+    Up5BwP p;
+    p.x = x; p.dy = dy; p.dw = dw; p.B = g.B; p.h = g.Hi; p.w_ = g.Wi; p.Ci = g.Ci; p.Co = g.Co; p.H = g.Ho; p.W = g.Wo; p.tiles_n = g.Ci / 32;
+    hipLaunchKernelGGL(up5_border_wgrad_kernel, dim3((g.Co / 32) * p.tiles_n, 16), dim3(UB_NW * 64), 0, st, p);
+    ACL_CHECK_LAUNCH("up5_border_wgrad_kernel");
+    return ACLGAN_OK;
+}
+size_t up5_fwd_ring_part_bytes(const ConvGeom& g) { return conv_up5_border(g, 0) ? 0 : ((fwd_partial_bytes(g, 2, BK) + 255) & ~(size_t)255); }
+bool up5_wgrad_border(const ConvGeom& g) { return conv_up5_border(g, 2) && wgrad_kc_ok(g) && conv_up5_wino_wgrad_scratch_bytes(g) != 0; }
+
 template <int WM, int WN, int TM, int TN>
 int up5_fwd_t(const ConvGeom& g, const float* x, const float* w, const float* bias, float* y, float* wp, hipStream_t st, float* keepV) {
     const int64_t nm = (int64_t)4 * g.Co * 9 * (g.Ci / 4);
@@ -823,10 +1000,11 @@
     p.B = g.B; p.ring = 0; p.phases = 1; p.Hf = g.Ho; p.Wf = g.Wo; p.part = nullptr; p.rows = 0;
     ConvGeom gp = g;
     gp.M = p.M; gp.K = p.K;
-    char* wino_scr = (char*)wp + up5_merged_bytes(g) + ((fwd_partial_bytes(g, 2, BK) + 255) & ~(size_t)255);
+    char* wino_scr = (char*)wp + up5_merged_bytes(g) + up5_fwd_ring_part_bytes(g);
     if (keepV && !conv_up5_wino_ok(g)) { set_error("conv_fwd: this layer does not keep a Winograd input transform"); return ACLGAN_EINVAL; }
     int rc = conv_up5_wino_ok(g) ? conv_up5_wino_fwd_phases(g, x, wp, bias, y, wino_scr, st, keepV, w) : launch_fwd_fast<WM, WN, TM, TN>(gp, p, st);
     if (rc) return rc;
+    if (conv_up5_border(g, 0)) return up5_border_fwd(g, x, w, y, st);
     p.w = w;
     p.Hi = g.Hi; p.Wi = g.Wi; p.Ho = g.Ho; p.Wo = g.Wo; p.k = 5; p.s = 1; p.p = 2; p.up = 1; p.Hu = g.Hu; p.Wu = g.Wu;
     p.M = g.M; p.K = g.K; p.ring = 2; p.phases = 0;
@@ -856,6 +1034,7 @@
     const int64_t ns = (int64_t)g.Co * 25 * (g.Ci / 4);
     hipLaunchKernelGGL(up5_scatter_kernel, dim3((int)std::min<int64_t>(cdiv64(ns, 256), 2048)), dim3(256), 0, st, dwp, dw, g.Co, g.Ci);
     ACL_CHECK_LAUNCH("up5_scatter_kernel");
+    if (up5_wgrad_border(g)) return up5_border_wgrad(g, x, dy, dw, st);
     p.dw = dw;
     p.Hi = g.Hi; p.Wi = g.Wi; p.Ho = g.Ho; p.Wo = g.Wo; p.k = 5; p.s = 1; p.p = 2; p.up = 1; p.Hu = g.Hu; p.Wu = g.Wu;
     p.ring = 2; p.phases = 0; p.Kn = g.K;
@@ -926,7 +1105,7 @@
 size_t conv_fwd_fast_scratch_bytes(const ConvGeom& g) {
     if (sw(SW_NOFAST)) return 0;
     if (conv_wino_ok(g)) return conv_wino_scratch_bytes(g);
-    if (up5_eligible(g)) return up5_merged_bytes(g) + ((fwd_partial_bytes(g, 2, BK) + 255) & ~(size_t)255) + conv_up5_wino_fwd_scratch_bytes(g);
+    if (up5_eligible(g)) return up5_merged_bytes(g) + up5_fwd_ring_part_bytes(g) + conv_up5_wino_fwd_scratch_bytes(g);
     return std::max(fwd_partial_bytes(g, 0, BK), conv_s2k4_wino_scratch_bytes(g));
 }
 
@@ -1075,6 +1254,11 @@
         const double ring_fwd = 2.0 * g.B * ringpix * g.Co * g.K;
         const double band = (double)g.Hp * g.Wp - (double)std::max(0, g.Hp - 12) * std::max(0, g.Wp - 12);
         const double ring_dg = 2.0 * g.B * band * g.Ci * g.Co * 9.0;
+        if (!f16 && conv_up5_border(g, 0) && which == 0)
+            return (wino_fused_ok(g.B, g.Hi, g.Wi, g.Ci, g.Co, g.act, 4, 1) ? fused_flops(g.B, g.Hi, g.Wi, g.Ci, g.Co, 4, 1) : pipe_flops(g.B, g.Hi, g.Wi, g.Ci, g.Co, 4)) +
+                   2.0 * 32.0 * g.Ci * (cdiv(g.Co, 64) * 64.0) * g.B * (10.0 * cdiv(g.Wo, 32) + 20.0 + 10.0 * cdiv(g.Ho - 2, 32));
+        if (!f16 && which == 2 && up5_wgrad_border(g))
+            return pipe_flops(g.B, g.Hi, g.Wi, g.Ci, g.Co, 4) + 2.0 * g.Co * g.Ci * 10.0 * g.B * (cdiv(g.Wo, 8) * 8.0 + cdiv(g.Ho, 8) * 8.0);
         if (!f16 && conv_up5_wino_ok(g)) {
             if (which == 0) return (wino_fused_ok(g.B, g.Hi - 2, g.Wi - 2, g.Ci, g.Co, g.act, 4, 1) ? fused_flops(g.B, g.Hi - 2, g.Wi - 2, g.Ci, g.Co, 4, 1)
                                                                                                      : pipe_flops(g.B, g.Hi - 2, g.Wi - 2, g.Ci, g.Co, 4)) + ring_fwd;
diff --git a/acl-gan_amd/csrc/conv_wino.hip b/acl-gan_amd/csrc/conv_wino.hip
--- a/acl-gan_amd/csrc/conv_wino.hip
+++ b/acl-gan_amd/csrc/conv_wino.hip
@@ -128,7 +128,7 @@
     return ((size_t)(b * v.HS + v.oy0 + v.sy * iy) * v.WS + v.ox0 + v.sx * ix) * C;
 }
 WView ident_view(int H, int W) { WView v = {H, W, 1, 1, 0, 0, H, W}; return v; }
-WView phase_view(int Hv, int Wv, int py, int px, int Hf, int Wf) { WView v = {Hv, Wv, 2, 2, 2 + py, 2 + px, Hf, Wf}; return v; }
+WView phase_view(int Hv, int Wv, int py, int px, int Hf, int Wf, int org = 2) { WView v = {Hv, Wv, 2, 2, org + py, org + px, Hf, Wf}; return v; }
 
 template <int NV>
 __global__ void __launch_bounds__(256) wino_input_kernel(const float* __restrict__ x, float* __restrict__ V, int B, WViews vs, int C, int TY, int TX, int off,
@@ -149,12 +149,12 @@
             F d[6];
             const int ixr = 4 * tx + off + j;
             const bool xin = (unsigned)ixr < (unsigned)v.W;
-            const int ix = reflect ? reflw(ixr, v.W) : (xin ? ixr : 0);
+            const int ix = reflect == 1 ? reflw(ixr, v.W) : (reflect == 2 ? min(max(ixr, 0), v.W - 1) : (xin ? ixr : 0));
 #pragma unroll
             for (int r = 0; r < 6; ++r) {
                 const int iyr = 4 * ty + off + r;
                 const bool yin = (unsigned)iyr < (unsigned)v.H;
-                const int iy = reflect ? reflw(iyr, v.H) : (yin ? iyr : 0);
+                const int iy = reflect == 1 ? reflw(iyr, v.H) : (reflect == 2 ? min(max(iyr, 0), v.H - 1) : (yin ? iyr : 0));
                 const F val = *reinterpret_cast<const F*>(x + vaddr(v, b, iy, ix, C) + c);
                 d[r] = (reflect || (xin && yin)) ? val : (F)(0.f);
             }
@@ -580,23 +580,33 @@
     return !sw(SW_NOWINO) && !sw(SW_NOWINOUP5) && g.up == 1 && g.k == 5 && g.p == 2 && g.s == 1 && g.Hi >= 6 && g.Wi >= 6 && g.Ci % 16 == 0 &&
            g.Co % 16 == 0 && (int64_t)g.Ci * g.Co >= 64 * 64;
 }
+bool conv_up5_border(const ConvGeom& g, int which) {
+    if (!conv_up5_wino_ok(g) || g.act != ACLGAN_ACT_NONE) return false;
+    if (which == 0) return sw(SW_UP5_BORDER) >= 2;
+    return sw(SW_UP5_BORDER) >= 1 && g.Co % 64 == 0 && g.Ci % 64 == 0;
+}
 namespace {
-struct Up5Geo { int Hv, Wv, TY, TX, TYd, TXd; int64_t T, Td; WViews ph; };
-Up5Geo up5_geo(const ConvGeom& g) {
+struct Up5Geo { int border, Hv, Wv, TY, TX, TYd, TXd, off, pad; int64_t T, Td; WViews ph, phd; };
+Up5Geo up5_geo(const ConvGeom& g, int which) {
     Up5Geo q;
-    q.Hv = g.Hi - 2; q.Wv = g.Wi - 2;
+    q.border = conv_up5_border(g, which) ? 1 : 0;
+    q.Hv = g.Hi - (q.border ? 0 : 2); q.Wv = g.Wi - (q.border ? 0 : 2);
+    q.off = q.border ? -1 : 0; q.pad = q.border ? 2 : 0;
     q.TY = cdiv(q.Hv, 4); q.TX = cdiv(q.Wv, 4); q.T = (int64_t)g.B * q.TY * q.TX;
     q.TYd = cdiv(g.Hi, 4); q.TXd = cdiv(g.Wi, 4); q.Td = (int64_t)g.B * q.TYd * q.TXd;
-    for (int p = 0; p < 4; ++p) q.ph.v[p] = phase_view(q.Hv, q.Wv, p >> 1, p & 1, g.Ho, g.Wo);
-    q.ph.nph = 4;
+    for (int p = 0; p < 4; ++p) {
+        q.ph.v[p] = phase_view(q.Hv, q.Wv, p >> 1, p & 1, g.Ho, g.Wo, q.border ? 0 : 2);
+        q.phd.v[p] = phase_view(g.Hi - 2, g.Wi - 2, p >> 1, p & 1, g.Ho, g.Wo);
+    }
+    q.ph.nph = 4; q.phd.nph = 4;
     return q;
 }
 }
 int conv_up5_wino_u_variant(const ConvGeom& g, int dgrad, bool keepV) {
     if (!conv_up5_wino_ok(g)) return -1;
-    const Up5Geo q = up5_geo(g);
+    const Up5Geo q = up5_geo(g, 0);
     if (!dgrad) {
-        if (!keepV && wino_fused_ok(g.B, g.Hi - 2, g.Wi - 2, g.Ci, g.Co, g.act, 4, 1)) return uvar(2, U_FRAG);
+        if (!keepV && wino_fused_ok(g.B, q.Hv, q.Wv, g.Ci, g.Co, g.act, 4, 1)) return uvar(2, U_FRAG);
         return uvar(2, (!keepV && sw(SW_WINO_X3) && gemm_x3_shape_ok((int)q.T, g.Ci, g.Co)) ? U_X3 : U_PIPE);
     }
     if (wino_fused_ok(g.B, g.Hi, g.Wi, g.Co, g.Ci, ACLGAN_ACT_NONE, 1, 4)) return uvar(3, U_FRAG);
@@ -604,25 +614,27 @@
 }
 size_t conv_up5_wino_fwd_scratch_bytes(const ConvGeom& g) {
     if (!conv_up5_wino_ok(g)) return 0;
-    const Up5Geo q = up5_geo(g);
+    const Up5Geo q = up5_geo(g, 0);
     return align256((size_t)144 * g.Co * g.Ci * 6) + align256((size_t)36 * q.T * g.Ci * 6) + align256((size_t)144 * q.T * g.Co * 4) + 256;
 }
 size_t conv_up5_wino_keep_bytes(const ConvGeom& g) {
     if (!conv_up5_wino_ok(g) || g.Co % 64 != 0 || g.Ci % 64 != 0) return 0;
     if (sw(SW_WINO_X3) && gemm_x3_shape_ok(1, g.Ci, g.Co)) return 0;
-    if (wino_fused_ok(g.B, g.Hi - 2, g.Wi - 2, g.Ci, g.Co, g.act, 4, 1)) return 0;
-    return align256((size_t)36 * up5_geo(g).T * g.Ci * sizeof(float));
+    if (conv_up5_border(g, 0) != conv_up5_border(g, 2)) return 0;
+    const Up5Geo q = up5_geo(g, 0);
+    if (wino_fused_ok(g.B, q.Hv, q.Wv, g.Ci, g.Co, g.act, 4, 1)) return 0;
+    return align256((size_t)36 * q.T * g.Ci * sizeof(float));
 }
 int conv_up5_wino_fwd_phases(const ConvGeom& g, const float* x, const float* wp, const float* bias, float* y, void* scratch, hipStream_t st, float* keepV,
                              const float* wkey) {
     if (!conv_up5_wino_ok(g) || !scratch) return ACLGAN_EUNSUPPORTED;
-    const Up5Geo q = up5_geo(g);
+    const Up5Geo q = up5_geo(g, 0);
     char* cur = (char*)scratch;
-    if (!keepV && wino_fused_ok(g.B, g.Hi - 2, g.Wi - 2, g.Ci, g.Co, g.act, 4, 1)) {
+    if (!keepV && wino_fused_ok(g.B, q.Hv, q.Wv, g.Ci, g.Co, g.act, 4, 1)) {
         bool fresh_f = true;
         float* Uf = cached_u((float*)scratch, wkey, uvar(2, U_FRAG), (size_t)144 * g.Co * g.Ci * 4, &fresh_f);
         if (fresh_f) { const int rcf = wino_fused_filter(wp, Uf, g.Co, g.Ci, 0, st, 4); if (rcf) return rcf; }
-        return wino_fused_up5_fwd(g.B, g.Hi, g.Wi, g.Ci, g.Co, x, Uf, bias, y, g.Ho, g.Wo, g.act, st);
+        return wino_fused_up5_fwd(g.B, g.Hi, g.Wi, g.Ci, g.Co, x, Uf, bias, y, g.Ho, g.Wo, g.act, q.border, st);
     }
     const bool x3 = !keepV && sw(SW_WINO_X3) && gemm_x3_shape_ok((int)q.T, g.Ci, g.Co);
     const size_t eb = x3 ? 6 : 4;
@@ -638,7 +650,7 @@
                            (int64_t)g.Co * 9 * g.Ci, (int64_t)36 * g.Co * g.Ci, (int64_t)36 * g.Co * g.Ci);
         ACL_CHECK_LAUNCH("wino_filter_kernel(up5)");
     }
-    int rc = launch_wino_input(x, V, g.B, one_view(ident_view(g.Hi, g.Wi)), 1, g.Ci, q.TY, q.TX, 0, 0, st, vplanes);
+    int rc = launch_wino_input(x, V, g.B, one_view(ident_view(g.Hi, g.Wi)), 1, g.Ci, q.TY, q.TX, q.off, q.pad, st, vplanes);
     if (rc) return rc;
     rc = x3 ? gemm_slices_x3(V, (size_t)vplanes * 2, U, (size_t)uplanes * 2, M, (int)q.T, g.Ci, g.Co, 144, 36, st) : gemm_slices_f32(V, U, M, (int)q.T, g.Ci, g.Co, 144, 36, st);
     if (rc) return rc;
@@ -646,12 +658,12 @@
 }
 size_t conv_up5_wino_dgrad_scratch_bytes(const ConvGeom& g) {
     if (!conv_up5_wino_ok(g)) return 0;
-    const Up5Geo q = up5_geo(g);
+    const Up5Geo q = up5_geo(g, 0);
     return align256((size_t)144 * g.Co * g.Ci * 6) + align256((size_t)144 * q.Td * g.Co * 6) + align256((size_t)144 * q.Td * g.Ci * 4) + 256;
 }
 int conv_up5_wino_dgrad_phases(const ConvGeom& g, const float* dy, const float* wp, float* dx, int accumulate, void* scratch, hipStream_t st, const float* wkey) {
     if (!conv_up5_wino_ok(g) || !scratch) return ACLGAN_EUNSUPPORTED;
-    const Up5Geo q = up5_geo(g);
+    const Up5Geo q = up5_geo(g, 0);
     char* cur = (char*)scratch;
     if (wino_fused_ok(g.B, g.Hi, g.Wi, g.Co, g.Ci, ACLGAN_ACT_NONE, 1, 4)) {
         bool fresh_f = true;
@@ -672,7 +684,7 @@
                            (int64_t)g.Co * 9 * g.Ci, (int64_t)36 * g.Co * g.Ci, (int64_t)36 * g.Co * g.Ci);
         ACL_CHECK_LAUNCH("wino_filter_kernel(up5 dgrad)");
     }
-    int rc = launch_wino_input(dy, V, g.B, q.ph, 4, g.Co, q.TYd, q.TXd, -2, 0, st, vplanes);
+    int rc = launch_wino_input(dy, V, g.B, q.phd, 4, g.Co, q.TYd, q.TXd, -2, 0, st, vplanes);
     if (rc) return rc;
     rc = x3 ? gemm_slices_x3(V, (size_t)vplanes * 2, U, (size_t)uplanes * 2, M, (int)q.Td, g.Co, g.Ci, 144, 0, st) : gemm_slices_f32(V, U, M, (int)q.Td, g.Co, g.Ci, 144, 0, st);
     if (rc) return rc;
@@ -682,13 +694,13 @@
 }
 size_t conv_up5_wino_wgrad_scratch_bytes(const ConvGeom& g) {
     if (!conv_up5_wino_ok(g) || g.Co % 64 != 0 || g.Ci % 64 != 0) return 0;
-    const Up5Geo q = up5_geo(g);
+    const Up5Geo q = up5_geo(g, 2);
     return align256((size_t)36 * q.T * g.Ci * 4) + align256((size_t)144 * q.T * g.Co * 4) + align256((size_t)144 * g.Co * g.Ci * 4) +
            align256(4 * WINO_BPART_BYTES + WINO_L2_BYTES) + gemm_at_b_slices_scratch((int)q.T, g.Co, g.Ci, 144) + 256;
 }
 int conv_up5_wino_wgrad_phases(const ConvGeom& g, const float* x, const float* dy, float* dwp, float* db, void* scratch, hipStream_t st, const float* haveV) {
     if (!conv_up5_wino_ok(g) || g.Co % 64 != 0 || g.Ci % 64 != 0 || !scratch || !wino_bias_ok(g.Co)) return ACLGAN_EUNSUPPORTED;
-    const Up5Geo q = up5_geo(g);
+    const Up5Geo q = up5_geo(g, 2);
     char* cur = (char*)scratch;
     float* V = take(cur, (size_t)36 * q.T * g.Ci * 4);
     float* dM = take(cur, (size_t)144 * q.T * g.Co * 4);
@@ -697,7 +709,7 @@
     void* part = cur;
     int rc0 = ACLGAN_OK;
     if (haveV) V = const_cast<float*>(haveV);
-    else rc0 = launch_wino_input(x, V, g.B, one_view(ident_view(g.Hi, g.Wi)), 1, g.Ci, q.TY, q.TX, 0, 0, st);
+    else rc0 = launch_wino_input(x, V, g.B, one_view(ident_view(g.Hi, g.Wi)), 1, g.Ci, q.TY, q.TX, q.off, q.pad, st);
     if (rc0) return rc0;
     int brows = 0;
     rc0 = launch_wino_outgrad(dy, dM, db ? bpart : (float*)nullptr, g.B, q.ph, 4, g.Co, q.TY, q.TX, st, &brows);
diff --git a/acl-gan_amd/csrc/conv_wino_fused.hip b/acl-gan_amd/csrc/conv_wino_fused.hip
--- a/acl-gan_amd/csrc/conv_wino_fused.hip
+++ b/acl-gan_amd/csrc/conv_wino_fused.hip
@@ -479,15 +479,16 @@
 }
 
 int wino_fused_up5_fwd(int B, int Hi, int Wi, int Cin_, int Cout_, const float* x, const float* Uf, const float* bias, float* y, int Hf, int Wf, int act,
-                       hipStream_t st) {
-    if (!wino_fused_ok(B, Hi - 2, Wi - 2, Cin_, Cout_, act, 4, 1) || Hi < 6 || Wi < 6) return ACLGAN_EUNSUPPORTED;
+                       int border, hipStream_t st) {
+    const int e = border ? 0 : 2;
+    if (!wino_fused_ok(B, Hi - e, Wi - e, Cin_, Cout_, act, 4, 1) || Hi < 6 || Wi < 6) return ACLGAN_EUNSUPPORTED;
     WfP p;
     p.x = x; p.Uf = Uf; p.bias = bias; p.y = y; p.stats = nullptr;
     p.B = B; p.Cin = Cin_; p.Cout = Cout_;
-    p.IH = Hi; p.IW = Wi; p.ivs = 1; p.ivy0 = 0; p.ivx0 = 0; p.IHS = Hi; p.IWS = Wi; p.off = 0; p.reflect = 0;
+    p.IH = Hi; p.IW = Wi; p.ivs = 1; p.ivy0 = 0; p.ivx0 = 0; p.IHS = Hi; p.IWS = Wi; p.off = border ? -1 : 0; p.reflect = border ? 2 : 0;
     p.nkph = 1;
-    for (int i = 0; i < 4; ++i) { p.kph_xoff[i] = 0; p.ovy0[i] = 2 + (i >> 1); p.ovx0[i] = 2 + (i & 1); }
-    p.OH = Hi - 2; p.OW = Wi - 2; p.ovs = 2; p.OHS = Hf; p.OWS = Wf;
+    for (int i = 0; i < 4; ++i) { p.kph_xoff[i] = 0; p.ovy0[i] = e + (i >> 1); p.ovx0[i] = e + (i & 1); }
+    p.OH = Hi - e; p.OW = Wi - e; p.ovs = 2; p.OHS = Hf; p.OWS = Wf;
     p.act = act; p.accumulate = 0;
     return wino_fused_go(p, 4, st);
 }
diff --git a/acl-gan_amd/csrc/switches.h b/acl-gan_amd/csrc/switches.h
--- a/acl-gan_amd/csrc/switches.h
+++ b/acl-gan_amd/csrc/switches.h
@@ -4,7 +4,7 @@
 namespace aclgan {
 
 enum SwitchId {
-    SW_LANES, SW_U_BATCH, SW_NORM_MASK, SW_MLP_FUSED, SW_FAULT_AT, SW_ENC_REUSE,
+    SW_LANES, SW_U_BATCH, SW_NORM_MASK, SW_MLP_FUSED, SW_FAULT_AT, SW_ENC_REUSE, SW_UP5_BORDER,
     SW_GLDS_TILE, SW_WINO_X3, SW_WINO_FUSED, SW_WINO_WGRAD_FUSED, SW_WINO_S2K4, SW_DGRAD16S_DIRECT, SW_FWD16_PATCH,
     SW_DETERMINISTIC,
     SW_NOFAST, SW_NOUP5, SW_SPLIT_NWG,
diff --git a/acl-gan_amd/csrc/switches.hip b/acl-gan_amd/csrc/switches.hip
--- a/acl-gan_amd/csrc/switches.hip
+++ b/acl-gan_amd/csrc/switches.hip
@@ -41,6 +41,7 @@
     {"mlp_fused",         "ACLGAN_MLP_FUSED",         1,  R_BOOL,  0, 0,       SETTABLE | EMPTY_UNSET, nullptr},
     {"fault_at",          nullptr,                    -1, R_INT,   0, 0,       SETTABLE, nullptr},
     {"enc_reuse",         nullptr,                    1,  R_BOOL,  0, 0,       SETTABLE, nullptr},
+    {"up5_border",        nullptr,                    1,  R_CLAMP, 0, 2,       SETTABLE, nullptr},
     {"glds_tile",         "ACLGAN_GLDS_TILE",         0,  R_CLAMP, 0, INT_MAX, SETTABLE, nullptr},
     {"wino_x3",           "ACLGAN_WINO_X3",           0,  R_BOOL,  0, 0,       SETTABLE, nullptr},
     {"wino_fused",        "ACLGAN_WINO_FUSED",        1,  R_LOW4,  0, 2,       SETTABLE, nullptr},
```

Result: no change. 105.2 (median of 6 runs) (+1.0%).
